# naver/must3r

Measured on AMD Instinct MI355X. Metric: views/sec (whole node) MUSt3R_512 20-view 512x384; pointmap max-abs-err vs ref, higher is better.
Workload: dtype fp16 (split weights in the attention-side Linears, plain in the Mlp Linears); 1 GPU; MUSt3R_512 20-view 384x512 scenes, S=28 independent scenes IN FLIGHT per GPU (560 views/step); one at a time: value_single_scene; scenes_in_flight_per_gpu=28, H=384, W=512, parallelism=single GPU

## Files before the change

### include/must3r_hip.h

```cpp
#ifndef MUST3R_HIP_H
#define MUST3R_HIP_H

#include <stdint.h>
#include <stddef.h>

#ifdef __cplusplus
extern "C" {
#endif

#define MUST3R_HIP_ABI_VERSION 21

typedef struct must3r_hip_ctx must3r_hip_ctx;

enum { MUST3R_BF16 = 0, MUST3R_F16 = 1, MUST3R_F16_W2 = 2, MUST3R_F16_WA = 3 };
#define MUST3R_ATTN_FP8 0x100
int must3r_hip_has_fp8_attention(void);

enum { MUST3R_MEM_KV = 0, MUST3R_MEM_NORM_Y = 1, MUST3R_MEM_RAW = 2 };

typedef struct must3r_hip_config {
    int32_t img_size, patch_size;
    int32_t enc_dim, enc_depth, enc_heads;
    int32_t dec_dim, dec_depth, dec_heads;
    int32_t mlp_ratio;
    float rope_freq;
    float rope_f0;
} must3r_hip_config;

int must3r_hip_abi_version(void);
const char* must3r_hip_last_error(void);
int must3r_hip_set_option(const char* name, long long value);

int must3r_hip_create(const must3r_hip_config* cfg, int device, must3r_hip_ctx** out);
void must3r_hip_destroy(must3r_hip_ctx* ctx);

int must3r_hip_load_weight(must3r_hip_ctx* ctx, const char* name, const float* data, int is_device,
                           int ndim, const int64_t* shape);
enum { MUST3R_PART_ENCODER = 1, MUST3R_PART_DECODER = 2 };
int must3r_hip_finalize_weights(must3r_hip_ctx* ctx, int parts);

int must3r_hip_encode(must3r_hip_ctx* ctx, int dtype, const float* img, int n_views, int H, int W,
                      float* out_tokens, int64_t* out_pos, void* stream);

typedef struct must3r_hip_group {
    const float* tokens;
    const int64_t* pos;
    int32_t n_views, n_tokens, H, W;
    float* pointmaps;
    int64_t pointmaps_scene_stride;
} must3r_hip_group;

typedef int (*must3r_hip_cp_exchange_fn)(void* user, int layer, void* slots, size_t slot_bytes, int n_slots, int my_slot, void* stream);
typedef struct must3r_hip_cp {
    int32_t world, rank;
    int32_t n_mem_total;
    int32_t partial16;
    void* slots;
    size_t slot_bytes;
    must3r_hip_cp_exchange_fn exchange;
    void* user;
} must3r_hip_cp;

typedef struct must3r_hip_decode_args {
    int32_t dtype;
    int32_t mem_mode;
    int32_t render;
    int32_t first_call;
    int32_t n_groups;
    const must3r_hip_group* groups;
    int32_t n_mem;
    void* const* mem;
    float* feats;
    int32_t mem_capacity;
    int32_t n_scenes;
    int64_t mem_scene_stride;
    const must3r_hip_cp* cp;
    int32_t causal;
} must3r_hip_decode_args;

size_t must3r_hip_cp_slot_bytes(const must3r_hip_ctx* ctx, int rows);
size_t must3r_hip_cp_slot_bytes16(const must3r_hip_ctx* ctx, int rows);

int must3r_hip_decode(must3r_hip_ctx* ctx, const must3r_hip_decode_args* args, void* stream);

int must3r_hip_postprocess(const float* pointmaps, float* pts3d, float* pts3d_local, float* conf, size_t npix,
                           void* stream);
enum { MUST3R_ACT_NORM_EXP = 0, MUST3R_ACT_LINEAR = 1 };
int must3r_hip_postprocess_act(const float* pointmaps, int activation, float* pts3d, float* pts3d_local, float* conf, size_t npix,
                               void* stream);
int must3r_hip_postprocess_act_grad(const float* pointmaps, int activation, const float* grad_pts3d, const float* grad_pts3d_local,
                                    const float* grad_conf, float* grad_pointmaps, size_t npix, void* stream);

size_t must3r_hip_postprocess_cam_scratch_bytes(int n_views, int H, int W);
int must3r_hip_postprocess_cam(const float* pointmaps, int n_views, int H, int W, float* pts3d, float* pts3d_local,
                               float* conf, float* focal, float* c2w, void* scratch, size_t scratch_bytes, void* stream);
int must3r_hip_postprocess_cam_act(const float* pointmaps, int activation, int n_views, int H, int W, float* pts3d, float* pts3d_local,
                                   float* conf, float* focal, float* c2w, void* scratch, size_t scratch_bytes, void* stream);

int must3r_hip_affine(int is_double, const float* A, const void* sub, const void* B, int b_transposed, const void* bias,
                      const float* resid, float* out, int M, int N, int K, void* stream);
int must3r_hip_row_norm(const float* x, int M, int C, float* out, void* stream);
int must3r_hip_l2_normalize(const float* x, int64_t outer, int L, int64_t inner, float* out, void* stream);
int must3r_hip_layernorm_act_f32(const float* x, const float* gamma, const float* beta, float eps, int M, int C, int gelu,
                                 float* out, void* stream);
int must3r_hip_topk_gather(const float* feat, const float* attn, int n_images, int N, int C, int k, float* out_feat,
                           float* out_attn, int64_t* out_idx, void* stream);
int must3r_hip_weighted_spoc(const float* feat, const float* attn, int n_images, int N, int C, float* out, void* stream);

int must3r_hip_asmk_centroid_sqnorm(const float* centroids, int K, int D, float* out, void* stream);
size_t must3r_hip_asmk_quantize_scratch_bytes(int M, int K, int k);
int must3r_hip_asmk_quantize(const float* feat, int M, const float* centroids, const float* c_sqnorm, int K, int D, int k, int32_t* ids,
                             void* scratch, size_t scratch_bytes, void* stream);
int must3r_hip_asmk_aggregate(const float* feat, const float* centroids, int K, int D, const int32_t* ids, int k_ids, int k_use,
                              const int32_t* offsets_dev, int n_images, int max_rows, int32_t* words, uint32_t* bits, int32_t* counts,
                              void* stream);
int must3r_hip_asmk_scores(const int32_t* words_q, const uint32_t* bits_q, const int32_t* counts_q, const int32_t* offsets_q, int k_q, int n_q,
                           const int32_t* words_d, const uint32_t* bits_d, const int32_t* counts_d, const int32_t* offsets_d, int k_d, int n_d,
                           int D, float alpha, float threshold, int normalize, double* out, void* stream);

int must3r_hip_nn_query(const float* db_xyz, int64_t n_db, const float* q_xyz, int64_t n_q, float* out_dist, void* stream);
int must3r_hip_quadrant_ids(const float* pts_xyz, int64_t n, const float* cam_center_host3, int divider, int32_t* out, void* stream);

size_t must3r_hip_nn_index_bytes(int64_t n, int divider);
size_t must3r_hip_nn_index_scratch_bytes(int64_t n);
int must3r_hip_nn_index_build(const float* xyz, const int32_t* quadrant_ids, int64_t n, int divider, void* index, void* scratch, void* stream);
int must3r_hip_nn_index_query(const void* index, const float* q_xyz, int64_t n_q, const float* cam_center_host3, int divider, float* out_dist,
                              void* stream);

#define MUST3R_EXPORT_MAX_THR 8
#define MUST3R_EXPORT_BLOCK 1024
#define MUST3R_EXPORT_GLB 0
#define MUST3R_EXPORT_PLY 1
typedef struct must3r_hip_export_view {
    const float* conf;
    const float* pts;
    const float* rgb;
    int32_t H, W;
    double M[12];
} must3r_hip_export_view;
size_t must3r_hip_export_scratch_bytes(const must3r_hip_export_view* views_host, int n_views, int n_thr, int mesh);
int must3r_hip_export_count(const must3r_hip_export_view* views_host, int n_views, const float* thr_host, int n_thr, int mesh,
                            void* scratch, size_t scratch_bytes, int64_t* totals_host, void* stream);
int must3r_hip_export_scatter_points(const must3r_hip_export_view* views_host, int n_views, const float* thr_host, int n_thr, int k,
                                     int layout, const void* scratch, void* out_pos, void* out_col, float* minmax, void* stream);
int must3r_hip_export_vertices(const must3r_hip_export_view* views_host, int n_views, int n_thr, void* scratch, float* out_pos,
                               void* out_col, float* minmax, void* stream);
int must3r_hip_export_scatter_faces(const must3r_hip_export_view* views_host, int n_views, const float* thr_host, int n_thr, int k,
                                    const void* scratch, uint32_t* out_faces, void* stream);

#define MUST3R_NORM_AVG_DIS 0
#define MUST3R_NORM_AVG_LOG1P 1
#define MUST3R_NORM_SQRT_DIS 2
#define MUST3R_NORM_MEDIAN_DIS 3
typedef struct must3r_hip_metrics_loss_args {
    int32_t n_scenes, n_views, H, W;
    const float* gt_pts;
    const float* in_camera0;
    const float* w2c;
    const float* pr_pts;
    const float* pr_local;
    const float* conf;
    const uint8_t* valid;
    const uint8_t* sky;
    const float* gt_scale;
    const float* pr_scale;
    const uint8_t* pr_warp;
    int32_t gt_warp, has_dist_clip, loss_in_log;
    float dist_clip, sky_loss_value, alpha;
    int64_t* counts;
    double* sums;
    float* pix_g; float* pix_l; uint8_t* msk_g; uint8_t* msk_l;
} must3r_hip_metrics_loss_args;
size_t must3r_hip_metrics_loss_scratch_bytes(int n_scenes, int n_views, int H, int W);
int must3r_hip_metrics_loss(const must3r_hip_metrics_loss_args* args, void* scratch, size_t scratch_bytes, void* stream);
size_t must3r_hip_metrics_factor_scratch_bytes(int n_scenes, int n_views, int H, int W, int mode);
int must3r_hip_metrics_factor(const float* pts, const float* trf, const uint8_t* valid, int n_scenes, int n_views, int H, int W, int mode,
                              float* factor, float* dist, void* scratch, size_t scratch_bytes, void* stream);

enum { MUST3R_LOSS_W_SCALAR = 0, MUST3R_LOSS_W_MEAN = 1, MUST3R_LOSS_W_CONF = 2, MUST3R_LOSS_W_PIXEL = 3 };
typedef struct must3r_hip_metrics_loss_grad_args {
    const float* w_g;
    const float* w_l;
    int32_t weighting;
    int32_t factor_mode;
    int32_t n_own;
    int32_t reserved;
    const int64_t* counts;
    const uint8_t* own_factor;
    const int64_t* n_valid;
    float* grad_pts;
    float* grad_local;
    float* grad_conf;
} must3r_hip_metrics_loss_grad_args;
size_t must3r_hip_metrics_loss_grad_scratch_bytes(int n_scenes, int n_views, int H, int W);
int must3r_hip_metrics_loss_grad(const must3r_hip_metrics_loss_args* args, const must3r_hip_metrics_loss_grad_args* grad, void* scratch,
                                 size_t scratch_bytes, void* stream);

enum { MUST3R_RESAMPLE_AA_BILINEAR = 0, MUST3R_RESAMPLE_PIL_LANCZOS = 1, MUST3R_RESAMPLE_PIL_BICUBIC = 2, MUST3R_RESAMPLE_NEAREST_EXACT = 3 };
enum { MUST3R_IMG_U8_HWC = 0, MUST3R_IMG_F32_CHW = 1 };

int must3r_hip_resample_coeffs(int mode, int in_size, int out_size, int* ksize, int32_t* bounds, void* weights);

typedef struct must3r_hip_image_desc {
    const void* src;
    int32_t src_format;
    int32_t channels;
    int32_t H, W;
    int64_t row_stride;
    int64_t plane_stride;
    int32_t crop_y, crop_x, crop_h, crop_w;
    int32_t resize_h, resize_w;
    int32_t out_y, out_x, out_h, out_w;
    int64_t out_offset;
} must3r_hip_image_desc;

size_t must3r_hip_image_scratch_bytes(int mode, const must3r_hip_image_desc* descs, int n_images);
int must3r_hip_resample(int mode, const must3r_hip_image_desc* descs, int n_images, float* out, void* scratch, size_t scratch_bytes,
                        void* stream);

enum { MUST3R_EPI_STORE16 = 0, MUST3R_EPI_STORE16_GELU = 1, MUST3R_EPI_QKV_ROPE = 2, MUST3R_EPI_RESID_F32 = 3,
       MUST3R_EPI_F32 = 4, MUST3R_EPI_HEAD = 5 };

int must3r_hip_op_gemm(int dtype, int epi, const void* A, const void* W, const float* bias, void* out,
                       int M, int N, int K, int lda, int ldc,
                       const int64_t* pos, const float* rope_tab, int rope_cols, int rope_npos,
                       const float* bias2, int row_start2, int accumulate,
                       int ntok, int gw, int H, int W_img,
                       int wsplit,
                       void* stream);
int must3r_hip_op_sparse24_pack(const float* w, int rows, int K, void* vals, void* idx, void* stream);
int must3r_hip_op_gemm_sp(int epi, const void* A, const void* W2, const void* Wlo_sp, const void* Widx_sp, const float* bias, void* out,
// ... 365 lines not shown
```

### must3r_amd/_lib.py

```python
import ctypes as C
import os

_HERE = os.path.dirname(os.path.abspath(__file__))
LIB_PATH = os.path.join(_HERE, "libmust3r_hip.so")

BF16, F16, F16_W2, F16_WA = 0, 1, 2, 3
ATTN_FP8 = 0x100
MEM_KV, MEM_NORM_Y, MEM_RAW = 0, 1, 2
PART_ENCODER, PART_DECODER = 1, 2
EPI_STORE16, EPI_STORE16_GELU, EPI_QKV_ROPE, EPI_RESID_F32, EPI_F32, EPI_HEAD = range(6)
ABI_VERSION = 21
ACT_NORM_EXP, ACT_LINEAR = 0, 1
EXPORT_MAX_THR, EXPORT_GLB, EXPORT_PLY = 8, 0, 1
NORM_AVG_DIS, NORM_AVG_LOG1P, NORM_SQRT_DIS, NORM_MEDIAN_DIS = range(4)
LOSS_W_SCALAR, LOSS_W_MEAN, LOSS_W_CONF, LOSS_W_PIXEL = range(4)
RESAMPLE_AA_BILINEAR, RESAMPLE_PIL_LANCZOS, RESAMPLE_PIL_BICUBIC, RESAMPLE_NEAREST_EXACT = range(4)
IMG_U8_HWC, IMG_F32_CHW = 0, 1
LIN_BIAS, LIN_BIAS_RES, LIN_BIAS_GELU = range(3)
TRAIN_LINEAR_F32, TRAIN_LINEAR_BF16 = 0, 1
TRAIN_ATTENTION_F32, TRAIN_ATTENTION_BF16 = 0, 1

class Config(C.Structure):
    _fields_ = [("img_size", C.c_int32), ("patch_size", C.c_int32),
                ("enc_dim", C.c_int32), ("enc_depth", C.c_int32), ("enc_heads", C.c_int32),
                ("dec_dim", C.c_int32), ("dec_depth", C.c_int32), ("dec_heads", C.c_int32),
                ("mlp_ratio", C.c_int32), ("rope_freq", C.c_float), ("rope_f0", C.c_float)]


class Group(C.Structure):
    _fields_ = [("tokens", C.c_void_p), ("pos", C.c_void_p),
                ("n_views", C.c_int32), ("n_tokens", C.c_int32), ("H", C.c_int32), ("W", C.c_int32),
                ("pointmaps", C.c_void_p), ("pointmaps_scene_stride", C.c_int64)]


CpExchangeFn = C.CFUNCTYPE(C.c_int, C.c_void_p, C.c_int, C.c_void_p, C.c_size_t, C.c_int, C.c_int, C.c_void_p)


class Cp(C.Structure):
    _fields_ = [("world", C.c_int32), ("rank", C.c_int32), ("n_mem_total", C.c_int32), ("partial16", C.c_int32),
                ("slots", C.c_void_p), ("slot_bytes", C.c_size_t), ("exchange", CpExchangeFn), ("user", C.c_void_p)]


class DecodeArgs(C.Structure):
    _fields_ = [("dtype", C.c_int32), ("mem_mode", C.c_int32), ("render", C.c_int32), ("first_call", C.c_int32),
                ("n_groups", C.c_int32), ("groups", C.POINTER(Group)), ("n_mem", C.c_int32),
                ("mem", C.POINTER(C.c_void_p)), ("feats", C.c_void_p),
                ("mem_capacity", C.c_int32), ("n_scenes", C.c_int32), ("mem_scene_stride", C.c_int64),
                ("cp", C.POINTER(Cp)), ("causal", C.c_int32)]


class ImageDesc(C.Structure):
    _fields_ = [("src", C.c_void_p), ("src_format", C.c_int32), ("channels", C.c_int32), ("H", C.c_int32), ("W", C.c_int32),
                ("row_stride", C.c_int64), ("plane_stride", C.c_int64),
                ("crop_y", C.c_int32), ("crop_x", C.c_int32), ("crop_h", C.c_int32), ("crop_w", C.c_int32),
                ("resize_h", C.c_int32), ("resize_w", C.c_int32),
                ("out_y", C.c_int32), ("out_x", C.c_int32), ("out_h", C.c_int32), ("out_w", C.c_int32), ("out_offset", C.c_int64)]


class AttnOp(C.Structure):
    _fields_ = [("dtype", C.c_int32), ("Q", C.c_void_p), ("K", C.c_void_p), ("V", C.c_void_p), ("O", C.c_void_p),
                ("ldq", C.c_int32), ("ldk", C.c_int32), ("ldv", C.c_int32), ("ldo", C.c_int32), ("heads", C.c_int32),
                ("views_dev", C.c_void_p), ("n_views", C.c_int32), ("view0_inline", C.c_int32), ("view0", C.c_int32 * 6),
                ("max_nq", C.c_int32), ("max_nk", C.c_int32), ("q_prescaled", C.c_int32),
                ("nsplit", C.c_int32), ("scratch", C.c_void_p), ("total_q_rows", C.c_int32), ("dense_rows", C.c_int32),
                ("stage", C.c_int32), ("slot_o", C.c_void_p), ("slot_ml", C.c_void_p), ("p16", C.c_int32), ("nslots", C.c_int32),
                ("stride_o", C.c_int64), ("stride_ml", C.c_int64), ("picked", C.POINTER(C.c_char_p))]


class LnOp(C.Structure):
    _fields_ = [("dtype", C.c_int32), ("x", C.c_void_p), ("x16", C.c_void_p), ("add", C.c_void_p), ("w", C.c_void_p), ("b", C.c_void_p),
                ("out16", C.c_void_p), ("out16_lo", C.c_void_p), ("out16_dup", C.c_void_p), ("ld16", C.c_int32),
                ("out32", C.c_void_p), ("copy32", C.c_void_p), ("raw16", C.c_void_p), ("M", C.c_int32), ("C", C.c_int32), ("eps", C.c_float),
                ("rows_per_group", C.c_int32), ("add_groups", C.c_int32), ("picked", C.POINTER(C.c_char_p)), ("mean_out", C.c_void_p)]


class GemmOp(C.Structure):
    _fields_ = [("dtype", C.c_int32), ("epi", C.c_int32), ("A", C.c_void_p), ("W", C.c_void_p), ("bias", C.c_void_p), ("out", C.c_void_p),
                ("M", C.c_int32), ("N", C.c_int32), ("K", C.c_int32), ("lda", C.c_int32), ("ldc", C.c_int32), ("wsplit", C.c_int32),
                ("Wlo_sp", C.c_void_p), ("Widx_sp", C.c_void_p), ("wsp_rows", C.c_int32), ("out_scale", C.c_float), ("scale_cols", C.c_int32),
                ("batch", C.c_int32), ("strideA", C.c_int64), ("strideW", C.c_int64), ("strideB", C.c_int64), ("out_table", C.c_void_p), ("wdiv", C.c_int32),
                ("pos", C.c_void_p), ("rope_tab", C.c_void_p), ("rope_cols", C.c_int32), ("rope_npos", C.c_int32),
                ("bias2", C.c_void_p), ("row_start2", C.c_int32), ("row_period2", C.c_int32), ("accumulate", C.c_int32),
                ("ntok", C.c_int32), ("gw", C.c_int32), ("H", C.c_int32), ("Wimg", C.c_int32), ("head_views", C.c_int32), ("head_scene_skip", C.c_int64),
                ("picked", C.POINTER(C.c_char_p))]


class LnFoldOp(C.Structure):
    _fields_ = [("dtype", C.c_int32), ("epi", C.c_int32), ("A", C.c_void_p), ("W", C.c_void_p), ("bias", C.c_void_p), ("out", C.c_void_p),
                ("M", C.c_int32), ("N", C.c_int32), ("K", C.c_int32), ("lda", C.c_int32), ("ldc", C.c_int32), ("wsplit", C.c_int32),
                ("x16_out", C.c_void_p), ("copy32_out", C.c_void_p), ("stats_out", C.c_void_p),
                ("ln_stats", C.c_void_p), ("ln_s", C.c_void_p), ("ln_eps", C.c_float), ("ln_shift", C.c_void_p), ("ln_shift_init", C.c_int32),
                ("pos", C.c_void_p), ("rope_tab", C.c_void_p), ("rope_cols", C.c_int32), ("rope_npos", C.c_int32),
                ("out_scale", C.c_float), ("scale_cols", C.c_int32), ("bias2", C.c_void_p), ("row_start2", C.c_int32),
                ("picked", C.POINTER(C.c_char_p))]


class ExportView(C.Structure):
    _fields_ = [("conf", C.c_void_p), ("pts", C.c_void_p), ("rgb", C.c_void_p), ("H", C.c_int32), ("W", C.c_int32), ("M", C.c_double * 12)]


class MetricsLossArgs(C.Structure):
    _fields_ = [("n_scenes", C.c_int32), ("n_views", C.c_int32), ("H", C.c_int32), ("W", C.c_int32),
                ("gt_pts", C.c_void_p), ("in_camera0", C.c_void_p), ("w2c", C.c_void_p), ("pr_pts", C.c_void_p), ("pr_local", C.c_void_p),
                ("conf", C.c_void_p), ("valid", C.c_void_p), ("sky", C.c_void_p), ("gt_scale", C.c_void_p), ("pr_scale", C.c_void_p),
                ("pr_warp", C.c_void_p), ("gt_warp", C.c_int32), ("has_dist_clip", C.c_int32), ("loss_in_log", C.c_int32),
                ("dist_clip", C.c_float), ("sky_loss_value", C.c_float), ("alpha", C.c_float),
                ("counts", C.c_void_p), ("sums", C.c_void_p),
                ("pix_g", C.c_void_p), ("pix_l", C.c_void_p), ("msk_g", C.c_void_p), ("msk_l", C.c_void_p)]


class MetricsLossGradArgs(C.Structure):
    _fields_ = [("w_g", C.c_void_p), ("w_l", C.c_void_p), ("weighting", C.c_int32), ("factor_mode", C.c_int32), ("n_own", C.c_int32),
                ("reserved", C.c_int32), ("counts", C.c_void_p), ("own_factor", C.c_void_p), ("n_valid", C.c_void_p),
                ("grad_pts", C.c_void_p), ("grad_local", C.c_void_p), ("grad_conf", C.c_void_p)]


class HeadGradArgs(C.Structure):
    _fields_ = [("x", C.c_void_p), ("gamma", C.c_void_p), ("beta", C.c_void_p), ("W", C.c_void_p), ("G", C.c_void_p),
                ("n_views", C.c_int32), ("H", C.c_int32), ("Wimg", C.c_int32), ("D", C.c_int32), ("eps", C.c_float), ("reserved", C.c_int32),
                ("dx", C.c_void_p), ("dgamma", C.c_void_p), ("dbeta", C.c_void_p), ("dW", C.c_void_p), ("db", C.c_void_p)]


class HeadForwardArArgs(C.Structure):
    _fields_ = [("x", C.c_void_p), ("gamma", C.c_void_p), ("beta", C.c_void_p), ("W", C.c_void_p), ("b", C.c_void_p),
                ("dtype", C.c_int32), ("n_views", C.c_int32), ("H", C.c_int32), ("Wimg", C.c_int32), ("D", C.c_int32), ("eps", C.c_float),
                ("pointmaps", C.c_void_p), ("transposed", C.c_void_p), ("stream", C.c_void_p)]


class HeadGradArArgs(C.Structure):
    _fields_ = [("g", HeadGradArgs), ("transposed", C.c_void_p), ("stream", C.c_void_p)]


class AttnTrainArgs(C.Structure):
    _fields_ = [("q", C.c_void_p), ("k", C.c_void_p), ("v", C.c_void_p), ("dO", C.c_void_p),
                ("ldq", C.c_int32), ("ldk", C.c_int32), ("ldv", C.c_int32), ("lddo", C.c_int32), ("heads", C.c_int32), ("n_views", C.c_int32),
                ("views", C.c_void_p), ("O", C.c_void_p), ("lse", C.c_void_p), ("dQ", C.c_void_p), ("dK", C.c_void_p), ("dV", C.c_void_p),
                ("ldo", C.c_int32), ("lddq", C.c_int32), ("lddk", C.c_int32), ("lddv", C.c_int32)]


class AttnMaskedArgs(C.Structure):
    _fields_ = [("core", AttnTrainArgs), ("mask_bits", C.c_void_p), ("view_mask", C.c_void_p), ("mask_rows", C.c_int32), ("mask_ld", C.c_int32),
                ("stream", C.c_void_p)]


class MlpSublayerArgs(C.Structure):
    _fields_ = [("x", C.c_void_p), ("gamma", C.c_void_p), ("beta", C.c_void_p), ("W1", C.c_void_p), ("b1", C.c_void_p), ("W2", C.c_void_p), ("b2", C.c_void_p),
                ("dy", C.c_void_p), ("M", C.c_int32), ("D", C.c_int32), ("hidden", C.c_int32), ("eps", C.c_float), ("out", C.c_void_p),
                ("dx", C.c_void_p), ("dgamma", C.c_void_p), ("dbeta", C.c_void_p), ("dW1", C.c_void_p), ("db1", C.c_void_p), ("dW2", C.c_void_p),
                ("db2", C.c_void_p)]


class AttnSublayerArgs(C.Structure):
    _fields_ = [("x", C.c_void_p), ("gamma", C.c_void_p), ("beta", C.c_void_p), ("Wqkv", C.c_void_p), ("bqkv", C.c_void_p), ("Wproj", C.c_void_p),
                ("bproj", C.c_void_p), ("dy", C.c_void_p), ("pos", C.c_void_p), ("rope_tab", C.c_void_p), ("views", C.c_void_p),
                ("M", C.c_int32), ("D", C.c_int32), ("n_views", C.c_int32), ("rope_npos", C.c_int32), ("eps", C.c_float), ("reserved", C.c_int32),
                ("out", C.c_void_p), ("dx", C.c_void_p), ("dgamma", C.c_void_p), ("dbeta", C.c_void_p), ("dWqkv", C.c_void_p), ("dbqkv", C.c_void_p),
                ("dWproj", C.c_void_p), ("dbproj", C.c_void_p)]


class CrossSublayerArgs(C.Structure):
    _fields_ = [("x", C.c_void_p), ("mem", C.c_void_p), ("gamma", C.c_void_p), ("beta", C.c_void_p), ("Wq", C.c_void_p), ("bq", C.c_void_p),
                ("Wk", C.c_void_p), ("bk", C.c_void_p), ("Wv", C.c_void_p), ("bv", C.c_void_p), ("Wproj", C.c_void_p), ("bproj", C.c_void_p),
                ("dy", C.c_void_p), ("views", C.c_void_p), ("out", C.c_void_p),
                ("dx", C.c_void_p), ("dmem", C.c_void_p), ("dgamma", C.c_void_p), ("dbeta", C.c_void_p), ("dWq", C.c_void_p), ("dbq", C.c_void_p),
                ("dWk", C.c_void_p), ("dbk", C.c_void_p), ("dWv", C.c_void_p), ("dbv", C.c_void_p), ("dWproj", C.c_void_p), ("dbproj", C.c_void_p),
                ("M", C.c_int32), ("Rm", C.c_int32), ("D", C.c_int32), ("n_views", C.c_int32), ("ldmem", C.c_int32), ("lddmem", C.c_int32),
                ("eps", C.c_float), ("reserved", C.c_int32), ("stream", C.c_void_p)]


class CrossSublayerMaskedArgs(C.Structure):
    _fields_ = [("core", CrossSublayerArgs), ("mask_bits", C.c_void_p), ("view_mask", C.c_void_p), ("mask_rows", C.c_int32), ("mask_ld", C.c_int32)]


FEEDBACK_MAX_LAYERS = 32


class FeedbackPrepareArgs(C.Structure):
    _fields_ = [(n, C.c_void_p * FEEDBACK_MAX_LAYERS) for n in ("x", "gamma", "beta", "dy", "y", "dx", "dgamma", "dbeta")] + [
        ("offset", C.c_void_p), ("doffset", C.c_void_p), ("L", C.c_int32), ("R", C.c_int32), ("D", C.c_int32), ("add_layers", C.c_int32),
        ("eps", C.c_float), ("reserved", C.c_int32), ("stream", C.c_void_p)]


OPTIM_CHUNK = 32768


class OptimTensor(C.Structure):
    _fields_ = [("p", C.c_void_p), ("g", C.c_void_p), ("m", C.c_void_p), ("v", C.c_void_p), ("step", C.c_void_p), ("n", C.c_int64),
                ("group", C.c_int32), ("reserved", C.c_int32)]


class OptimGroup(C.Structure):
    _fields_ = [("lr", C.c_double), ("weight_decay", C.c_double), ("beta1", C.c_double), ("beta2", C.c_double), ("eps", C.c_double)]


class OptimControl(C.Structure):
    _fields_ = [("norm", C.c_float), ("coef", C.c_float), ("found_inf", C.c_int32), ("reserved", C.c_int32)]


class OptimArgs(C.Structure):
    _fields_ = [("tensors", C.POINTER(OptimTensor)), ("groups", C.POINTER(OptimGroup)), ("n_tensors", C.c_int32), ("n_groups", C.c_int32),
                ("control", C.c_void_p), ("scale", C.c_void_p), ("growth_tracker", C.c_void_p),
                ("max_norm", C.c_float), ("growth_factor", C.c_float), ("backoff_factor", C.c_float), ("growth_interval", C.c_int32),
                ("stream", C.c_void_p)]


class PatchRowsArgs(C.Structure):
    _fields_ = [("img", C.c_void_p), ("transposed", C.c_void_p), ("rows", C.c_void_p), ("pos", C.c_void_p),
                ("V", C.c_int32), ("H", C.c_int32), ("W", C.c_int32), ("reserved", C.c_int32), ("stream", C.c_void_p)]


GT_VIEW_BLOCKS = 32


class GtArgs(C.Structure):
    _fields_ = [("depth", C.c_void_p), ("depth_scale", C.c_void_p), ("K", C.c_void_p), ("c2w", C.c_void_p), ("transposed", C.c_void_p),
                ("pts3d", C.c_void_p), ("valid", C.c_void_p), ("sky", C.c_void_p), ("n_valid", C.c_void_p),
                ("scratch", C.c_void_p), ("scratch_bytes", C.c_size_t),
                ("V", C.c_int32), ("Hs", C.c_int32), ("Ws", C.c_int32), ("depth_u16", C.c_int32), ("stream", C.c_void_p)]


AUG_BRIGHTNESS, AUG_CONTRAST, AUG_SATURATION, AUG_HUE = range(4)
AUG_TILE = 64


class AugmentColorView(C.Structure):
    _fields_ = [("src_offset", C.c_int64), ("h", C.c_int32), ("w", C.c_int32), ("portrait", C.c_int32), ("order", C.c_int32 * 4),
                ("apply", C.c_int32 * 4), ("factor", C.c_float * 4), ("reserved", C.c_int32)]


class AugmentColorArgs(C.Structure):
    _fields_ = [("src", C.c_void_p), ("src_elems", C.c_int64), ("views", C.POINTER(AugmentColorView)), ("out", C.c_void_p),
                ("scratch", C.c_void_p), ("scratch_bytes", C.c_size_t),
                ("V", C.c_int32), ("Hs", C.c_int32), ("Ws", C.c_int32), ("reserved", C.c_int32), ("stream", C.c_void_p)]


class AugmentDepthView(C.Structure):
    _fields_ = [("src", C.c_void_p), ("row_stride", C.c_int64), ("H", C.c_int32), ("W", C.c_int32),
                ("crop_x", C.c_int32), ("crop_y", C.c_int32), ("crop_w", C.c_int32), ("crop_h", C.c_int32),
                ("resize_w", C.c_int32), ("resize_h", C.c_int32),
                ("win_x", C.c_int32), ("win_y", C.c_int32), ("out_w", C.c_int32), ("out_h", C.c_int32), ("portrait", C.c_int32), ("reserved", C.c_int32)]


class AugmentDepthArgs(C.Structure):
    _fields_ = [("views", C.POINTER(AugmentDepthView)), ("out", C.c_void_p), ("scratch", C.c_void_p), ("scratch_bytes", C.c_size_t),
                ("V", C.c_int32), ("Hs", C.c_int32), ("Ws", C.c_int32), ("depth_u16", C.c_int32), ("stream", C.c_void_p)]


class ProfRecord(C.Structure):
    _fields_ = [("name", C.c_char * 32), ("ms", C.c_double), ("flops", C.c_double), ("calls", C.c_int64)]


vp, i32, i64, fp, sz, cstr, P = C.c_void_p, C.c_int, C.c_int64, C.c_float, C.c_size_t, C.c_char_p, C.POINTER
PROTOTYPES = {
    "must3r_hip_last_error": (cstr, []),
    "must3r_hip_has_fp8_attention": (i32, []),
    "must3r_hip_abi_version": (i32, []),
    "must3r_hip_set_option": (i32, [cstr, i64]),
    "must3r_hip_create": (i32, [P(Config), i32, P(vp)]),
    "must3r_hip_destroy": (None, [vp]),
    "must3r_hip_load_weight": (i32, [vp, cstr, vp, i32, i32, P(i64)]),
    "must3r_hip_finalize_weights": (i32, [vp, i32]),
    "must3r_hip_encode": (i32, [vp, i32, vp, i32, i32, i32, vp, vp, vp]),
    "must3r_hip_cp_slot_bytes": (sz, [vp, i32]),
    "must3r_hip_cp_slot_bytes16": (sz, [vp, i32]),
    "must3r_hip_decode": (i32, [vp, P(DecodeArgs), vp]),
    "must3r_hip_postprocess": (i32, [vp, vp, vp, vp, sz, vp]),
    "must3r_hip_postprocess_act": (i32, [vp, i32, vp, vp, vp, sz, vp]),
    "must3r_hip_postprocess_act_grad": (i32, [vp, i32, vp, vp, vp, vp, sz, vp]),
    "must3r_hip_postprocess_cam_scratch_bytes": (sz, [i32, i32, i32]),
    "must3r_hip_postprocess_cam": (i32, [vp, i32, i32, i32, vp, vp, vp, vp, vp, vp, sz, vp]),
    "must3r_hip_postprocess_cam_act": (i32, [vp, i32, i32, i32, i32, vp, vp, vp, vp, vp, vp, sz, vp]),
    "must3r_hip_affine": (i32, [i32, vp, vp, vp, i32, vp, vp, vp, i32, i32, i32, vp]),
    "must3r_hip_row_norm": (i32, [vp, i32, i32, vp, vp]),
    "must3r_hip_l2_normalize": (i32, [vp, i64, i32, i64, vp, vp]),
    "must3r_hip_layernorm_act_f32": (i32, [vp, vp, vp, fp, i32, i32, i32, vp, vp]),
    "must3r_hip_topk_gather": (i32, [vp, vp, i32, i32, i32, i32, vp, vp, vp, vp]),
    "must3r_hip_weighted_spoc": (i32, [vp, vp, i32, i32, i32, vp, vp]),
    "must3r_hip_asmk_quantize_scratch_bytes": (sz, [i32, i32, i32]),
    "must3r_hip_asmk_centroid_sqnorm": (i32, [vp, i32, i32, vp, vp]),
    "must3r_hip_asmk_quantize": (i32, [vp, i32, vp, vp, i32, i32, i32, vp, vp, sz, vp]),
    "must3r_hip_asmk_aggregate": (i32, [vp, vp, i32, i32, vp, i32, i32, vp, i32, i32, vp, vp, vp, vp]),
    "must3r_hip_asmk_scores": (i32, [vp, vp, vp, vp, i32, i32, vp, vp, vp, vp, i32, i32, i32, fp, fp, i32, vp, vp]),
    "must3r_hip_nn_query": (i32, [vp, i64, vp, i64, vp, vp]),
    "must3r_hip_quadrant_ids": (i32, [vp, i64, P(fp), i32, vp, vp]),
    "must3r_hip_nn_index_bytes": (sz, [i64, i32]),
    "must3r_hip_nn_index_scratch_bytes": (sz, [i64]),
    "must3r_hip_nn_index_build": (i32, [vp, vp, i64, i32, vp, vp, vp]),
    "must3r_hip_nn_index_query": (i32, [vp, vp, i64, P(fp), i32, vp, vp]),
    "must3r_hip_export_scratch_bytes": (sz, [P(ExportView), i32, i32, i32]),
    "must3r_hip_export_count": (i32, [P(ExportView), i32, P(fp), i32, i32, vp, sz, P(i64), vp]),
    "must3r_hip_export_scatter_points": (i32, [P(ExportView), i32, P(fp), i32, i32, i32, vp, vp, vp, vp, vp]),
    "must3r_hip_export_vertices": (i32, [P(ExportView), i32, i32, vp, vp, vp, vp, vp]),
    "must3r_hip_export_scatter_faces": (i32, [P(ExportView), i32, P(fp), i32, i32, vp, vp, vp]),
    "must3r_hip_metrics_loss_scratch_bytes": (sz, [i32, i32, i32, i32]),
    "must3r_hip_metrics_loss": (i32, [P(MetricsLossArgs), vp, sz, vp]),
    "must3r_hip_metrics_factor_scratch_bytes": (sz, [i32, i32, i32, i32, i32]),
    "must3r_hip_metrics_factor": (i32, [vp, vp, vp, i32, i32, i32, i32, i32, vp, vp, vp, sz, vp]),
    "must3r_hip_metrics_loss_grad_scratch_bytes": (sz, [i32, i32, i32, i32]),
    "must3r_hip_metrics_loss_grad": (i32, [P(MetricsLossArgs), P(MetricsLossGradArgs), vp, sz, vp]),
    "must3r_hip_resample_coeffs": (i32, [i32, i32, i32, P(i32), vp, vp]),
    "must3r_hip_image_scratch_bytes": (sz, [i32, P(ImageDesc), i32]),
    "must3r_hip_resample": (i32, [i32, P(ImageDesc), i32, vp, vp, sz, vp]),
    "must3r_hip_op_gemm": (i32, [i32, i32, vp, vp, vp, vp, i32, i32, i32, i32, i32, vp, vp, i32, i32, vp, i32, i32, i32, i32, i32, i32, i32, vp]),
    "must3r_hip_op_sparse24_pack": (i32, [vp, i32, i32, vp, vp, vp]),
    "must3r_hip_op_gemm_sp": (i32, [i32, vp, vp, vp, vp, vp, vp, i32, i32, i32, i32, i32, vp, vp, i32, i32, vp]),
    "must3r_hip_op_gemm_lnfold": (i32, [i32, i32, vp, vp, vp, vp, i32, i32, i32, i32, i32, vp, vp, vp, vp, vp, fp, vp, i32, vp, vp, i32, i32, fp, i32, vp]),
    "must3r_hip_op_gemm_lnfold_ex": (i32, [P(LnFoldOp), vp]),
    "must3r_hip_op_gemm_fold256": (i32, [i32, i32, vp, vp, vp, vp, vp, vp, i32, i32, i32, i32, i32, vp, vp, vp, vp, vp, fp, vp, vp, vp, i32, i32, fp, i32, vp]),
    "must3r_hip_op_gemm_ex": (i32, [P(GemmOp), vp]),
    "must3r_hip_rope_table": (i32, [fp, fp, i32, vp]),
    "must3r_hip_attention_scratch_bytes": (sz, [i32, i32, i32]),
    "must3r_hip_op_attention": (i32, [i32, vp, vp, vp, vp, i32, i32, i32, i32, i32, vp, i32, i32, i32, vp, i32, vp]),
    "must3r_hip_op_attention_ex": (i32, [P(AttnOp), vp]),
    "must3r_hip_op_layernorm": (i32, [i32, vp, vp, vp, vp, vp, vp, vp, vp, i32, i32, fp, vp]),
    "must3r_hip_op_layernorm_ex": (i32, [P(LnOp), vp]),
    "must3r_hip_op_im2col": (i32, [i32, vp, vp, i32, i32, i32, vp]),
    "must3r_hip_op_cast": (i32, [i32, vp, vp, vp, sz, vp]),
    "must3r_hip_head_grad_splits": (i32, [i32]),
    "must3r_hip_head_forward_scratch_bytes": (sz, [i32, i32, i32, i32]),
    "must3r_hip_head_forward": (i32, [i32, vp, vp, vp, vp, vp, i32, i32, i32, i32, fp, vp, vp, sz, vp]),
    "must3r_hip_op_head_linear": (i32, [i32, vp, vp, vp, i32, i32, i32, i32, vp, vp, sz, vp]),
    "must3r_hip_head_grad_scratch_bytes": (sz, [i32, i32, i32, i32]),
    "must3r_hip_head_grad": (i32, [P(HeadGradArgs), vp, sz, vp]),
    "must3r_hip_head_forward_many_ar_scratch_bytes": (sz, [i32, i32, i32, i32]),
    "must3r_hip_head_forward_many_ar": (i32, [P(HeadForwardArArgs), vp, sz]),
    "must3r_hip_head_grad_many_ar_scratch_bytes": (sz, [i32, i32, i32, i32]),
    "must3r_hip_head_grad_many_ar": (i32, [P(HeadGradArArgs), vp, sz]),
    "must3r_hip_op_linear_dgrad_f32": (i32, [vp, i32, vp, vp, i32, i32, i32, vp]),
    "must3r_hip_op_linear_wgrad_scratch_bytes": (sz, [i32, i32, i32]),
    "must3r_hip_op_linear_wgrad_f32": (i32, [vp, i32, vp, i32, vp, vp, i32, i32, i32, vp, sz, vp]),
    "must3r_hip_op_layernorm_grad_scratch_bytes": (sz, [i32, i32]),
    "must3r_hip_op_layernorm_grad": (i32, [vp, vp, vp, vp, vp, vp, i32, i32, fp, vp, sz, vp]),
    "must3r_hip_attn_train_scratch_bytes": (sz, [i32, i32, i32, i32]),
    "must3r_hip_attn_train_groups": (i32, [vp, i32]),
    "must3r_hip_attn_forward_f32": (i32, [P(AttnTrainArgs), vp, sz, vp]),
    "must3r_hip_attn_grad": (i32, [P(AttnTrainArgs), vp, sz, vp]),
    "must3r_hip_attn_masked_scratch_bytes": (sz, [i32, i32, i32, i32]),
    "must3r_hip_attn_masked_forward": (i32, [P(AttnMaskedArgs), vp, sz]),
    "must3r_hip_attn_masked_grad": (i32, [P(AttnMaskedArgs), vp, sz]),
    "must3r_hip_op_linear_f32": (i32, [i32, vp, i32, vp, vp, vp, i32, vp, i32, vp, i32, i32, i32, i32, vp]),
    "must3r_hip_op_layernorm_f32": (i32, [vp, vp, vp, vp, i32, i32, fp, vp]),
    "must3r_hip_op_gelu_f32": (i32, [vp, vp, vp, C.c_longlong, vp]),
    "must3r_hip_op_gelu_grad_f32": (i32, [vp, i32, vp, i32, vp, i32, i32, i32, vp]),
    "must3r_hip_op_rope_f32": (i32, [vp, i32, vp, vp, i32, i32, i32, i32, vp]),
    "must3r_hip_op_layernorm_grad_add": (i32, [vp, vp, vp, vp, vp, vp, vp, i32, i32, fp, vp, sz, vp]),
    "must3r_hip_mlp_sublayer_scratch_bytes": (sz, [i32, i32, i32]),
    "must3r_hip_mlp_sublayer_forward": (i32, [P(MlpSublayerArgs), vp, sz, vp]),
    "must3r_hip_mlp_sublayer_grad": (i32, [P(MlpSublayerArgs), vp, sz, vp]),
    "must3r_hip_attn_sublayer_scratch_bytes": (sz, [i32, i32, i32]),
    "must3r_hip_attn_sublayer_forward": (i32, [P(AttnSublayerArgs), vp, sz, vp]),
    "must3r_hip_attn_sublayer_grad": (i32, [P(AttnSublayerArgs), vp, sz, vp]),
    "must3r_hip_cross_sublayer_scratch_bytes": (sz, [i32, i32, i32, i32, i32]),
    "must3r_hip_cross_sublayer_forward": (i32, [P(CrossSublayerArgs), vp, sz]),
    "must3r_hip_cross_sublayer_grad": (i32, [P(CrossSublayerArgs), vp, sz]),
    "must3r_hip_cross_sublayer_masked_scratch_bytes": (sz, [i32, i32, i32, i32, i32]),
    "must3r_hip_cross_sublayer_masked_forward": (i32, [P(CrossSublayerMaskedArgs), vp, sz]),
    "must3r_hip_cross_sublayer_masked_grad": (i32, [P(CrossSublayerMaskedArgs), vp, sz]),
    "must3r_hip_feedback_prepare_scratch_bytes": (sz, [i32, i32, i32]),
    "must3r_hip_feedback_prepare_forward": (i32, [P(FeedbackPrepareArgs), vp, sz]),
    "must3r_hip_feedback_prepare_grad": (i32, [P(FeedbackPrepareArgs), vp, sz]),
    "must3r_hip_optim_scratch_bytes": (sz, [i64, i64]),
    "must3r_hip_optim_norm": (i32, [P(OptimArgs), vp, sz]),
    "must3r_hip_optim_adamw": (i32, [P(OptimArgs), vp, sz]),
    "must3r_hip_train_linear_mode": (i32, [i32]),
    "must3r_hip_train_attention_mode": (i32, [i32]),
    "must3r_hip_patch_rows": (i32, [P(PatchRowsArgs)]),
    "must3r_hip_gt_from_depth": (i32, [P(GtArgs)]),
    "must3r_hip_augment_color_scratch_bytes": (sz, [i32, i32, i32]),
    "must3r_hip_augment_color": (i32, [P(AugmentColorArgs)]),
    "must3r_hip_augment_depth_scratch_bytes": (sz, [i32]),
    "must3r_hip_augment_depth": (i32, [P(AugmentDepthArgs)]),
    "must3r_hip_debug_tr_probe": (i32, [vp, vp]),
    "must3r_hip_set_profiling": (i32, [vp, i32]),
    "must3r_hip_get_profile": (i32, [vp, P(ProfRecord), i32, i32]),
}
EXPORTS = tuple(PROTOTYPES)


class HipError(RuntimeError):
    pass


_lib = None


def load():
    global _lib
    if _lib is not None:
        return _lib
    if not os.path.exists(LIB_PATH):
        raise ImportError(
            f"{LIB_PATH} not found: build it with `python -c 'import __graft_entry__ as g; g.build()'` "
            "(make -C must3r_amd/csrc). must3r_amd has no CPU fallback.")
    lib = C.CDLL(LIB_PATH)
    for name, (restype, argtypes) in PROTOTYPES.items():
        fn = getattr(lib, name)
        fn.restype, fn.argtypes = restype, argtypes
    if lib.must3r_hip_abi_version() != ABI_VERSION:
        raise ImportError(f"{LIB_PATH}: ABI version {lib.must3r_hip_abi_version()} != {ABI_VERSION}; rebuild")
    _lib = lib
    return lib


def stream_ptr(device):
    import torch
    return torch.cuda.current_stream(device).cuda_stream


def check(rc):
    if rc != 0:
        raise HipError(load().must3r_hip_last_error().decode("utf-8", "replace"))


def has_fp8_attention():
    return bool(load().must3r_hip_has_fp8_attention())
# ... 52 lines not shown
```

### must3r_amd/csrc/kernels.hpp

```cpp
#pragma once
#include <hip/hip_runtime.h>
#include <stdint.h>

struct must3r_hip_ctx;

namespace m3r {

enum DType { DT_BF16 = 0, DT_F16 = 1 };

enum Epi {
    EPI_STORE16 = 0,
    EPI_STORE16_GELU,
    EPI_QKV_ROPE,
    EPI_RESID_F32,
    EPI_F32,
    EPI_HEAD,
    EPI_COUNT
};

#ifdef M3R_ATTN_FP8
constexpr bool kAttnFp8Built = true;
#else
constexpr bool kAttnFp8Built = false;
#endif

struct GemmArgs {
    const void* A;
    const void* W;
    const float* bias;
    void* out;
    int M, N, K, lda, ldc;
    int wsplit;
    const void* Wlo_sp;
    const void* Widx_sp;
    int wsp_rows;
    float out_scale;
    int scale_cols;
    int batch;
    long long strideA, strideW, strideB;
    void* const* out_table;
    int wdiv;
    const int64_t* pos;
    const float* rope_tab;
    int rope_cols;
    int rope_npos;
    const float* bias2;
    int row_start2;
    int row_period2;
    int accumulate;
    int ntok, gw, H, Wimg;
    int head_views;
    long long head_scene_skip;
    void* x16_out;
    float* copy32_out;
    float* stats_out;
    const float* ln_stats;
    const float* ln_s;
    float ln_eps;
    float* ln_shift;
    int ln_shift_init;
    int fold256;
    int gm;
#ifdef GEMM_TRACE
    int trace_block;
#endif
};

int launch_gemm(DType dt, Epi epi, const GemmArgs& a, hipStream_t s, const char** err);
const char* gemm_last_kernel();
bool gemm_fold256_shape_ok(int M, int N, int K, bool split);

struct AttnView {
    int q_row0;
    int nq;
    int kv_row0;
    int nk;
    int skip_lo;
    int skip_hi;
};

struct AttnArgs {
    const void* Q; const void* K; const void* V; void* O;
    int ldq, ldk, ldv, ldo;
    int heads;
    const AttnView* views;
    int nviews;
    int view0_inline;
    AttnView view0;
    int max_nq;
    float scale;
    int q_prescaled;
    int nsplit;
    float* part_o;
    float* part_ml;
    int total_q_rows;
    int dense_rows;
    int part16;
    int fp8;
    int max_nk;
    long long part_stride_o, part_stride_ml;
};
int launch_attention_partial_merge(DType dt, const AttnArgs& a, float* out_o, float* out_ml, int p16, hipStream_t s, const char** err);
int launch_attention_partial_empty(float* out_o, float* out_ml, int rows, int heads, int p16, hipStream_t s, const char** err);
int launch_attention_partial_final(DType dt, const AttnArgs& a, const float* slots_o, const float* slots_ml, long long stride_o, long long stride_ml, int nslots,
                                   int p16, hipStream_t s, const char** err);
size_t attention_split_scratch_bytes(int nsplit, int total_q_rows, int heads);
int attention_pick_split(int nviews, int heads, int max_nq, int max_nk);
int launch_attention(DType dt, const AttnArgs& a, hipStream_t s, const char** err);
bool attention_is_small(int nviews, int heads, int max_nq, int nsplit);
int launch_attention_phase(DType dt, const AttnArgs& a, int phase, hipStream_t s, const char** err);
const char* attention_last_kernel();

struct LnArgs {
    const float* x;
    const void* x16;
    void* raw16;
    const float* add;
    const float* w; const float* b;
    void* out16;
    void* out16_lo;
    void* out16_dup;
    int ld16;
    float* out32;
    float* copy32;
    float* mean_out;
    int M, C;
    float eps;
    int rows_per_group;
    int add_groups;
};
int launch_layernorm(DType dt, const LnArgs& a, hipStream_t s, const char** err);
const char* layernorm_last_kernel();

int launch_im2col(DType dt, const float* img, void* out16, int V, int H, int W, hipStream_t s, const char** err);
int launch_cast(DType dt, const float* in, void* out16, void* out16_lo, size_t n, hipStream_t s, const char** err);
int launch_quant8(DType dt, const void* in16, int ld_in, void* out8, int ld_out, void* const* out_table, int rows_per_group,
                  size_t rows, int cols, int tail_cols, hipStream_t s, const char** err);
int launch_fill_pos(int64_t* pos, int V, int gh, int gw, hipStream_t s, const char** err);
int launch_split16(DType dt, const float* in, void* hi, void* lo, size_t n, hipStream_t s, const char** err);
int launch_sparse24_pack(const float* w, int rows, int K, void* vals, void* idx, hipStream_t s, const char** err);

int head_layernorm(must3r_hip_ctx* c, DType dt, const float* x, const float* gamma, const float* beta, void* hcat, float* y32, int R, int D, float eps,
                   hipStream_t s);
int head_linear(must3r_hip_ctx* c, DType dt, const void* hcat, const void* wcat, const float* bias_ps, float* pointmaps, int rows, int D, int OUT, int ntok,
                int gw, int H, int Wimg, int head_views, long long head_scene_skip, hipStream_t s);

int launch_dgrad_seg_f32(const float* dZ, int ldz, const float* W0, const float* W1, int O0, float* out, int ldo, int M, int O, int K, hipStream_t s);

struct LinArgs;
bool train_linear_bf16();
int launch_linear_bf16(const char* who, int epi, const LinArgs& p, hipStream_t s);
int launch_dgrad_bf16(const char* who, const float* dZ, int ldz, const float* W0, const float* W1, int O0, float* out, int ldo, int M, int O, int K, hipStream_t s);
int launch_wgrad_parts_bf16(const float* dZ, int ldz, const float* A, int lda, int M, int O, int K, int rows_per_split, int S, int want_dw, float* part,
                            float* pdb, hipStream_t s);

int launch_tr_probe(short* out, hipStream_t s);

}
```

### must3r_amd/csrc/misc.hip

```cpp
#include "abi.hpp"
#include "common.hpp"
#include "kernels.hpp"
#include "options.hpp"
#include <cstring>
#include <cstdio>
#include <cstdlib>

namespace m3r {
namespace {
struct OptRow { const char* name; long long def, lo, hi; };
const OptRow kOpts[OPT_COUNT] = {
    {"PERSIST", 0, 0, 1}, {"GEMM256", 1, 0, 2}, {"G256K", 1, 0, 2}, {"G256P", 1, 0, 1}, {"G256P_SPLIT", 1, 0, 2}, {"SPARSE_256", 1, 0, 1},
    {"SPARSE_LO", 1, 0, 1}, {"BK128", 1, 0, 1}, {"LN_ROWS", 1, 0, 1}, {"LNFOLD", 1, 0, 2}, {"ENC_CHUNK_ROWS", 32768, 256, 1 << 22}, {"ATTN_LZ", 1, 0, 2},
    {"LNFOLD256", 0, 0, 1}, {"G256_GM", 4, 1, 64}, {"NN_LEAF_LOG2", 5, 4, 6}, {"NN_QUERY_LANES_LOG2", 3, 0, 4},
};
long long g_opt_val[OPT_COUNT];
bool g_opt_init[OPT_COUNT];
}

int opt(Opt o) {
    if (!g_opt_init[o]) {
        const OptRow& r = kOpts[o];
        long long v = r.def;
        char env[48];
        snprintf(env, sizeof(env), "M3R_%s", r.name);
        if (const char* e = getenv(env)) {
            char* end = nullptr;
            const long long x = strtoll(e, &end, 10);
            if (end == e || *end != 0 || x < r.lo || x > r.hi)
                fprintf(stderr, "libmust3r_hip: %s=%s ignored (an integer in [%lld, %lld] is expected); using %lld\n", env, e, r.lo, r.hi, r.def);
            else v = x;
        }
        g_opt_val[o] = v;
        g_opt_init[o] = true;
    }
    return (int)g_opt_val[o];
}

int opt_set(const char* name, long long value, const char** err) {
    static thread_local char msg[128];
    for (int o = 0; o < OPT_COUNT; ++o) {
        if (name == nullptr || strcmp(name, kOpts[o].name) != 0) continue;
        if (value < kOpts[o].lo || value > kOpts[o].hi) {
            snprintf(msg, sizeof(msg), "set_option: %s = %lld is outside [%lld, %lld]", name, value, kOpts[o].lo, kOpts[o].hi);
            *err = msg;
            return 1;
        }
        g_opt_val[o] = value;
        g_opt_init[o] = true;
        return 0;
    }
    snprintf(msg, sizeof(msg), "set_option: unknown option '%s'", name ? name : "(null)");
    *err = msg;
    return 1;
}


template <class T, bool MEAN = false>
__global__ void __launch_bounds__(256) ln_kernel(const LnArgs p) {
    typedef typename Vec<T>::v4 v4;
    const int lane = threadIdx.x & 63;
    const int row = blockIdx.x * 4 + (threadIdx.x >> 6);
    if (row >= p.M) return;
    const float* wp = p.w;
    const float* bp = p.b;
    const float* addp = p.add ? p.add + (size_t)row * p.C : nullptr;
    if (p.rows_per_group > 0) {
        const int g = row / p.rows_per_group;
        wp += (size_t)g * p.C;
        bp += (size_t)g * p.C;
        addp = (p.add && g < p.add_groups) ? p.add + (size_t)(row - g * p.rows_per_group) * p.C : nullptr;
    }
    f32x4 v[4];
    float s = 0.f;
#pragma unroll
    for (int i = 0; i < 4; ++i) {
        const int c = (i * 64 + lane) * 4;
        v[i] = f32x4{0.f, 0.f, 0.f, 0.f};
        if (c < p.C) {
            if (p.x) v[i] = *reinterpret_cast<const f32x4*>(p.x + (size_t)row * p.C + c);
            else v[i] = __builtin_convertvector(*reinterpret_cast<const v4*>(reinterpret_cast<const T*>(p.x16) + (size_t)row * p.C + c), f32x4);
            if (addp) v[i] += *reinterpret_cast<const f32x4*>(addp + c);
            if (p.copy32) *reinterpret_cast<f32x4*>(p.copy32 + (size_t)row * p.C + c) = v[i];
            if (p.raw16) *reinterpret_cast<v4*>(reinterpret_cast<T*>(p.raw16) + (size_t)row * p.C + c) = cvt4_sat<T>(v[i]);
            s += v[i][0] + v[i][1] + v[i][2] + v[i][3];
        }
    }
    const float mean = wave_sum_dpp(s) / (float)p.C;
    if constexpr (MEAN) {
        if (lane == 0) p.mean_out[row] = mean;
    }
    float q = 0.f;
#pragma unroll
    for (int i = 0; i < 4; ++i) {
        const int c = (i * 64 + lane) * 4;
        if (c < p.C) {
            v[i] -= mean;
            q += v[i][0] * v[i][0] + v[i][1] * v[i][1] + v[i][2] * v[i][2] + v[i][3] * v[i][3];
        }
    }
    const float rstd = rsqrtf(wave_sum_dpp(q) / (float)p.C + p.eps);
#pragma unroll
    for (int i = 0; i < 4; ++i) {
        const int c = (i * 64 + lane) * 4;
        if (c < p.C) {
            const f32x4 w = *reinterpret_cast<const f32x4*>(wp + c);
            const f32x4 b = *reinterpret_cast<const f32x4*>(bp + c);
            const f32x4 y = v[i] * rstd * w + b;
            if (p.out32) *reinterpret_cast<f32x4*>(p.out32 + (size_t)row * p.C + c) = y;
            if (p.out16) {
                const size_t ld = p.ld16 ? (size_t)p.ld16 : (size_t)p.C;
                const v4 h = cvt4<T>(y);
                *reinterpret_cast<v4*>(reinterpret_cast<T*>(p.out16) + row * ld + c) = h;
                if (p.out16_dup) *reinterpret_cast<v4*>(reinterpret_cast<T*>(p.out16_dup) + row * ld + c) = h;
                if (p.out16_lo) {
                    const f32x4 hf = __builtin_convertvector(h, f32x4);
                    *reinterpret_cast<v4*>(reinterpret_cast<T*>(p.out16_lo) + row * ld + c) = cvt4<T>(y - hf);
                }
            }
        }
    }
}

template <class T, int NV>
__global__ void __launch_bounds__(256) ln_rows_kernel(const LnArgs p) {
    typedef typename Vec<T>::v4 v4;
    const int lane = threadIdx.x & 63;
    const int nwaves = gridDim.x * 4;
    int row = blockIdx.x * 4 + (threadIdx.x >> 6);
    if (row >= p.M) return;
    const bool grouped = p.rows_per_group > 0;
    bool act[NV];
    f32x4 w[NV], b[NV];
#pragma unroll
    for (int i = 0; i < NV; ++i) {
        act[i] = (i * 64 + lane) * 4 < p.C;
        w[i] = b[i] = f32x4{0.f, 0.f, 0.f, 0.f};
        if (act[i] && !grouped) {
            w[i] = *reinterpret_cast<const f32x4*>(p.w + (i * 64 + lane) * 4);
            b[i] = *reinterpret_cast<const f32x4*>(p.b + (i * 64 + lane) * 4);
        }
    }
    auto load = [&](int r, f32x4 (&v)[NV]) {
#pragma unroll
        for (int i = 0; i < NV; ++i) {
            const int c = (i * 64 + lane) * 4;
            v[i] = f32x4{0.f, 0.f, 0.f, 0.f};
            if (act[i]) {
                if (p.x) v[i] = *reinterpret_cast<const f32x4*>(p.x + (size_t)r * p.C + c);
                else v[i] = __builtin_convertvector(*reinterpret_cast<const v4*>(reinterpret_cast<const T*>(p.x16) + (size_t)r * p.C + c), f32x4);
            }
        }
    };
    f32x4 v[NV], nx[NV];
    load(row, v);
    for (; row < p.M; row += nwaves) {
        const int nr = row + nwaves;
        if (nr < p.M) load(nr, nx);
        const float* addp = p.add ? p.add + (size_t)row * p.C : nullptr;
        if (grouped) {
            const int g = row / p.rows_per_group;
            addp = (p.add && g < p.add_groups) ? p.add + (size_t)(row - g * p.rows_per_group) * p.C : nullptr;
#pragma unroll
            for (int i = 0; i < NV; ++i)
                if (act[i]) {
                    w[i] = *reinterpret_cast<const f32x4*>(p.w + (size_t)g * p.C + (i * 64 + lane) * 4);
                    b[i] = *reinterpret_cast<const f32x4*>(p.b + (size_t)g * p.C + (i * 64 + lane) * 4);
                }
        }
        float s = 0.f;
#pragma unroll
        for (int i = 0; i < NV; ++i) {
            const int c = (i * 64 + lane) * 4;
            if (act[i]) {
                if (addp) v[i] += *reinterpret_cast<const f32x4*>(addp + c);
                if (p.copy32) *reinterpret_cast<f32x4*>(p.copy32 + (size_t)row * p.C + c) = v[i];
                if (p.raw16) *reinterpret_cast<v4*>(reinterpret_cast<T*>(p.raw16) + (size_t)row * p.C + c) = cvt4_sat<T>(v[i]);
                s += v[i][0] + v[i][1] + v[i][2] + v[i][3];
            }
        }
        const float mean = wave_sum_dpp(s) / (float)p.C;
        float q = 0.f;
#pragma unroll
        for (int i = 0; i < NV; ++i)
            if (act[i]) {
                v[i] -= mean;
                q += v[i][0] * v[i][0] + v[i][1] * v[i][1] + v[i][2] * v[i][2] + v[i][3] * v[i][3];
            }
        const float rstd = rsqrtf(wave_sum_dpp(q) / (float)p.C + p.eps);
#pragma unroll
        for (int i = 0; i < NV; ++i) {
            const int c = (i * 64 + lane) * 4;
            if (act[i]) {
                const f32x4 y = v[i] * rstd * w[i] + b[i];
                if (p.out32) *reinterpret_cast<f32x4*>(p.out32 + (size_t)row * p.C + c) = y;
                if (p.out16) {
                    const size_t ld = p.ld16 ? (size_t)p.ld16 : (size_t)p.C;
                    const v4 h = cvt4<T>(y);
                    *reinterpret_cast<v4*>(reinterpret_cast<T*>(p.out16) + row * ld + c) = h;
                    if (p.out16_dup) *reinterpret_cast<v4*>(reinterpret_cast<T*>(p.out16_dup) + row * ld + c) = h;
                    if (p.out16_lo) {
                        const f32x4 hf = __builtin_convertvector(h, f32x4);
                        *reinterpret_cast<v4*>(reinterpret_cast<T*>(p.out16_lo) + row * ld + c) = cvt4<T>(y - hf);
                    }
                }
            }
        }
#pragma unroll
        for (int i = 0; i < NV; ++i) v[i] = nx[i];
    }
}

static int ln_rows_mode() { return opt(OPT_LN_ROWS); }
static thread_local const char* g_ln_pick = "";
const char* layernorm_last_kernel() { return g_ln_pick; }
template <class T>
static void launch_ln_t(const LnArgs& a, hipStream_t s) {
    const int grid_one = (a.M + 3) / 4;
    if (a.mean_out != nullptr) {
        g_ln_pick = "ln";
        hipLaunchKernelGGL((ln_kernel<T, true>), dim3(grid_one), dim3(256), 0, s, a);
        return;
    }
    if (ln_rows_mode() == 0 || a.M < 65536) {
        g_ln_pick = "ln";
        hipLaunchKernelGGL(ln_kernel<T>, dim3(grid_one), dim3(256), 0, s, a);
        return;
    }
    const int grid = 256 * 8;
    g_ln_pick = a.C <= 768 ? "ln_rows/3" : "ln_rows/4";
    if (a.C <= 768) hipLaunchKernelGGL((ln_rows_kernel<T, 3>), dim3(grid), dim3(256), 0, s, a);
    else hipLaunchKernelGGL((ln_rows_kernel<T, 4>), dim3(grid), dim3(256), 0, s, a);
}

int launch_layernorm(DType dt, const LnArgs& a, hipStream_t s, const char** err) {
    if (a.M <= 0) return 0;
    if (a.C > 1024 || a.C % 4) { *err = "layernorm: C must be <= 1024 and a multiple of 4"; return 1; }
    if (dt == DT_BF16) launch_ln_t<bf16_t>(a, s);
    else launch_ln_t<f16_t>(a, s);
    if (hipGetLastError() != hipSuccess) { *err = "layernorm: launch failed"; return 1; }
    return 0;
}

template <class T>
__global__ void im2col_kernel(const float* __restrict__ img, T* __restrict__ out, int V, int H, int W) {
    typedef typename Vec<T>::v8 v8;
    const int gh = H / 16, gw = W / 16;
    const size_t total = (size_t)V * gh * gw * 96;
    for (size_t idx = (size_t)blockIdx.x * blockDim.x + threadIdx.x; idx < total; idx += (size_t)gridDim.x * blockDim.x) {
        const int ch = (int)(idx % 96);
        const size_t tok = idx / 96;
        const int t = (int)(tok % (gh * gw));
        const int v = (int)(tok / (gh * gw));
        const int gy = t / gw, gx = t - gy * gw;
        const int c = ch / 32, rem = ch - c * 32;
        const int i = rem >> 1, j0 = (rem & 1) * 8;
        const float* src = img + (((size_t)v * 3 + c) * H + gy * 16 + i) * W + gx * 16 + j0;
        const f32x4 a = *reinterpret_cast<const f32x4*>(src);
        const f32x4 b = *reinterpret_cast<const f32x4*>(src + 4);
        const f32x8 f = __builtin_shufflevector(a, b, 0, 1, 2, 3, 4, 5, 6, 7);
        *reinterpret_cast<v8*>(out + tok * 768 + ch * 8) = cvt8<T>(f);
    }
}

int launch_im2col(DType dt, const float* img, void* out16, int V, int H, int W, hipStream_t s, const char** err) {
    if (H % 16 || W % 16) { *err = "im2col: H and W must be multiples of 16"; return 1; }
    const size_t total = (size_t)V * (H / 16) * (W / 16) * 96;
    if (!total) return 0;
    const int grid = (int)((total + 255) / 256 < 4096 ? (total + 255) / 256 : 4096);
    if (dt == DT_BF16) hipLaunchKernelGGL(im2col_kernel<bf16_t>, dim3(grid), dim3(256), 0, s, img, (bf16_t*)out16, V, H, W);
    else hipLaunchKernelGGL(im2col_kernel<f16_t>, dim3(grid), dim3(256), 0, s, img, (f16_t*)out16, V, H, W);
    if (hipGetLastError() != hipSuccess) { *err = "im2col: launch failed"; return 1; }
    return 0;
}

template <class T>
__global__ void cast_kernel(const float* __restrict__ in, T* __restrict__ hi, T* __restrict__ lo, size_t n4) {
    typedef typename Vec<T>::v4 v4;
    for (size_t i = (size_t)blockIdx.x * blockDim.x + threadIdx.x; i < n4; i += (size_t)gridDim.x * blockDim.x) {
        const f32x4 x = reinterpret_cast<const f32x4*>(in)[i];
        const v4 h = cvt4<T>(x);
        reinterpret_cast<v4*>(hi)[i] = h;
        if (lo) reinterpret_cast<v4*>(lo)[i] = cvt4<T>(x - __builtin_convertvector(h, f32x4));
    }
}

int launch_split16(DType dt, const float* in, void* hi, void* lo, size_t n, hipStream_t s, const char** err) {
    if (n % 4) { *err = "cast: element count must be a multiple of 4"; return 1; }
    if (!n) return 0;
    const size_t n4 = n / 4;
    const int grid = (int)((n4 + 255) / 256 < 8192 ? (n4 + 255) / 256 : 8192);
    if (dt == DT_BF16) hipLaunchKernelGGL(cast_kernel<bf16_t>, dim3(grid), dim3(256), 0, s, in, (bf16_t*)hi, (bf16_t*)lo, n4);
    else hipLaunchKernelGGL(cast_kernel<f16_t>, dim3(grid), dim3(256), 0, s, in, (f16_t*)hi, (f16_t*)lo, n4);
    if (hipGetLastError() != hipSuccess) { *err = "cast: launch failed"; return 1; }
    return 0;
}

int launch_cast(DType dt, const float* in, void* out16, void* out16_lo, size_t n, hipStream_t s, const char** err) {
    return launch_split16(dt, in, out16, out16_lo, n, s, err);
}

__global__ void sparse24_pack_kernel(const float* __restrict__ w, int rows, int K, f16_t* __restrict__ vals, unsigned short* __restrict__ idx) {
    const size_t total = (size_t)(K / 64) * rows * 4;
    for (size_t u = (size_t)blockIdx.x * blockDim.x + threadIdx.x; u < total; u += (size_t)gridDim.x * blockDim.x) {
        const int g = (int)(u & 3);
        const size_t tn = u >> 2;
        const int n = (int)(tn % rows), t = (int)(tn / rows);
        const float* src = w + (size_t)n * K + t * 64 + g * 16;
        unsigned bits = 0;
        f16_t out[8];
#pragma unroll
        for (int q = 0; q < 4; ++q) {
            float lo[4], mag[4];
#pragma unroll
            for (int e = 0; e < 4; ++e) {
                const float x = src[q * 4 + e];
                const f16_t hi = (f16_t)x;
                lo[e] = (float)(f16_t)(x - (float)hi);
                mag[e] = fabsf(lo[e]);
            }
            int p0 = 0;
#pragma unroll
            for (int e = 1; e < 4; ++e) if (mag[e] > mag[p0]) p0 = e;
            int p1 = p0 == 0 ? 1 : 0;
#pragma unroll
            for (int e = 0; e < 4; ++e) if (e != p0 && mag[e] > mag[p1]) p1 = e;
            const int a = p0 < p1 ? p0 : p1, b = p0 < p1 ? p1 : p0;
            out[q * 2] = (f16_t)lo[a];
            out[q * 2 + 1] = (f16_t)lo[b];
            bits |= (unsigned)(a | (b << 2)) << (4 * q);
        }
        f16_t* dv = vals + ((size_t)t * rows + n) * 32 + g * 8;
#pragma unroll
        for (int e = 0; e < 8; ++e) dv[e] = out[e];
        idx[(((size_t)t * (rows / 32) + n / 32) * 64 + (n % 16) + 16 * g) * 2 + ((n % 32) / 16)] = (unsigned short)bits;
    }
}

int launch_sparse24_pack(const float* w, int rows, int K, void* vals, void* idx, hipStream_t s, const char** err) {
    if (rows <= 0 || K <= 0 || rows % 32 || K % 64) { *err = "sparse24_pack: rows % 32 and K % 64 must be 0"; return 1; }
    const size_t total = (size_t)(K / 64) * rows * 4;
    const int grid = (int)((total + 255) / 256 < 8192 ? (total + 255) / 256 : 8192);
    hipLaunchKernelGGL(sparse24_pack_kernel, dim3(grid), dim3(256), 0, s, w, rows, K, (f16_t*)vals, (unsigned short*)idx);
    if (hipGetLastError() != hipSuccess) { *err = "sparse24_pack: launch failed"; return 1; }
    return 0;
}

#ifdef M3R_ATTN_FP8
template <class T>
__global__ void quant8_kernel(const T* __restrict__ in, int ld_in, unsigned char* __restrict__ out, int ld_out, void* const* out_table,
                              int rows_per_group, size_t rows, int cols, int tail_cols) {
    typedef typename Vec<T>::v8 v8;
    const int cpr = (cols + tail_cols) / 8;
    const size_t total = rows * (size_t)cpr;
    for (size_t idx = (size_t)blockIdx.x * blockDim.x + threadIdx.x; idx < total; idx += (size_t)gridDim.x * blockDim.x) {
        const size_t r = idx / cpr;
        const int c = (int)(idx - r * cpr) * 8;
        const v8 raw = *reinterpret_cast<const v8*>(in + r * ld_in + c);
        unsigned char* dst = out;
        size_t rr = r;
        if (out_table) {
            const size_t g = r / rows_per_group;
            dst = reinterpret_cast<unsigned char*>(out_table[g]);
            rr = r - g * rows_per_group;
        }
        if (c >= cols) {
            *reinterpret_cast<v8*>(dst + rr * ld_out + cols + (size_t)(c - cols) * 2) = raw;
            continue;
        }
        const f32x8 x = __builtin_convertvector(raw, f32x8);
        float y[8];
#pragma unroll
        for (int e = 0; e < 8; ++e) y[e] = __builtin_amdgcn_fmed3f(x[e], -448.0f, 448.0f);
        int lo = 0, hi = 0;
        lo = __builtin_amdgcn_cvt_pk_fp8_f32(y[0], y[1], lo, false);
        lo = __builtin_amdgcn_cvt_pk_fp8_f32(y[2], y[3], lo, true);
        hi = __builtin_amdgcn_cvt_pk_fp8_f32(y[4], y[5], hi, false);
        hi = __builtin_amdgcn_cvt_pk_fp8_f32(y[6], y[7], hi, true);
        *reinterpret_cast<u32x2*>(dst + rr * ld_out + c) = u32x2{(unsigned)lo, (unsigned)hi};
    }
}

int launch_quant8(DType dt, const void* in16, int ld_in, void* out8, int ld_out, void* const* out_table, int rows_per_group,
                  size_t rows, int cols, int tail_cols, hipStream_t s, const char** err) {
    if (!rows || !(cols + tail_cols)) return 0;
    if (cols % 16 || tail_cols % 8 || ld_in % 8 || ld_out % 16) { *err = "quant8: cols % 16, tail_cols % 8, ld_in % 8, ld_out % 16"; return 1; }
    const size_t total = rows * (size_t)((cols + tail_cols) / 8);
    const int grid = (int)((total + 255) / 256 < 8192 ? (total + 255) / 256 : 8192);
    if (dt == DT_BF16) hipLaunchKernelGGL(quant8_kernel<bf16_t>, dim3(grid), dim3(256), 0, s, (const bf16_t*)in16, ld_in, (unsigned char*)out8, ld_out, out_table, rows_per_group, rows, cols, tail_cols);
    else hipLaunchKernelGGL(quant8_kernel<f16_t>, dim3(grid), dim3(256), 0, s, (const f16_t*)in16, ld_in, (unsigned char*)out8, ld_out, out_table, rows_per_group, rows, cols, tail_cols);
    if (hipGetLastError() != hipSuccess) { *err = "quant8: launch failed"; return 1; }
    return 0;
}
#endif

__global__ void fill_pos_kernel(int64_t* pos, int V, int gh, int gw) {
    const size_t total = (size_t)V * gh * gw;
    for (size_t i = (size_t)blockIdx.x * blockDim.x + threadIdx.x; i < total; i += (size_t)gridDim.x * blockDim.x) {
        const int t = (int)(i % (gh * gw));
        pos[i * 2 + 0] = t / gw;
        pos[i * 2 + 1] = t % gw;
    }
}

int launch_fill_pos(int64_t* pos, int V, int gh, int gw, hipStream_t s, const char** err) {
    const size_t total = (size_t)V * gh * gw;
    if (!total) return 0;
    const int grid = (int)((total + 255) / 256 < 2048 ? (total + 255) / 256 : 2048);
    hipLaunchKernelGGL(fill_pos_kernel, dim3(grid), dim3(256), 0, s, pos, V, gh, gw);
    if (hipGetLastError() != hipSuccess) { *err = "fill_pos: launch failed"; return 1; }
    return 0;
}

__device__ __forceinline__ void norm_exp3(const float* v, float* o) {
    const float d = sqrtf(v[0] * v[0] + v[1] * v[1] + v[2] * v[2]);
    const float sc = expm1f(d) / fmaxf(d, 1e-8f);
    o[0] = v[0] * sc;
    o[1] = v[1] * sc;
    o[2] = v[2] * sc;
}

template <bool LINEAR>
__global__ void postprocess_kernel(const float* __restrict__ pm, float* __restrict__ p3, float* __restrict__ pl,
                                   float* __restrict__ cf, size_t npix) {
    for (size_t i = (size_t)blockIdx.x * blockDim.x + threadIdx.x; i < npix; i += (size_t)gridDim.x * blockDim.x) {
        float v[7];
#pragma unroll
        for (int k = 0; k < 7; ++k) v[k] = pm[i * 7 + k];
        float a[3], b[3];
        if constexpr (LINEAR) {
#pragma unroll
            for (int k = 0; k < 3; ++k) { a[k] = v[k]; b[k] = v[3 + k]; }
        } else {
            norm_exp3(v, a);
            norm_exp3(v + 3, b);
        }
#pragma unroll
        for (int k = 0; k < 3; ++k) {
            p3[i * 3 + k] = a[k];
            pl[i * 3 + k] = b[k];
        }
        cf[i] = 1.0f + expf(v[6]);
    }
}

__device__ __forceinline__ void norm_exp3_grad(const float* v, const float* g, float* o) {
    const float d = sqrtf(v[0] * v[0] + v[1] * v[1] + v[2] * v[2]);
    if (d == 0.f) { o[0] = o[1] = o[2] = 0.f; return; }
    const float c = fmaxf(d, 1e-8f);
    const float h = expm1f(d) / c;
    const float b = d >= 1e-8f ? expf(d) - h : expf(d) * d / c;
    const float s = (v[0] * g[0] + v[1] * g[1] + v[2] * g[2]) / d * b;
    o[0] = h * g[0] + s * (v[0] / d);
    o[1] = h * g[1] + s * (v[1] / d);
// ... 82 lines not shown
```

### must3r_amd/csrc/model.hip

```cpp
#include <hip/hip_runtime.h>
#include <cmath>
#include <cstdarg>
#include <cstdio>
#include <cstring>
#include <map>
#include <string>
#include <vector>

#include "abi.hpp"
#include "kernels.hpp"
#include "options.hpp"

using namespace m3r;

static thread_local char g_err[512] = "";
int m3r::fail(const char* fmt, ...) {
    va_list ap;
    va_start(ap, fmt);
    vsnprintf(g_err, sizeof(g_err), fmt, ap);
    va_end(ap);
    return 1;
}
#define HIP_OK(expr)                                                                              \
    do {                                                                                          \
// ... 623 lines not shown
struct Fold {
    uint16_t* x16 = nullptr;
    float* stats = nullptr;
    float* shift = nullptr;
    bool f256 = false;
    bool fresh = true;
    bool on() const { return x16 != nullptr; }
    void in(GemmArgs& g, const Param* s, const Param* c) {
        g.A = x16; g.ln_stats = stats; g.ln_s = s->d; g.bias = c->d; g.ln_eps = 1e-6f;
        g.ln_shift = shift; g.ln_shift_init = (fresh && !f256) ? 1 : 0; g.fold256 = f256 ? 1 : 0;
        fresh = false;
    }
    void out(GemmArgs& g, float* copy32) const { g.x16_out = x16; g.stats_out = stats; g.copy32_out = copy32; g.ln_shift = shift; g.fold256 = f256 ? 1 : 0; }
};

struct BlockRows {
    int R, C, heads, F;
    float* x; uint16_t *h16, *qkv, *a16, *g16;
    uint8_t* q8;
    const int64_t* pos;
};
struct SelfViews { const AttnView* dev; int n, max_n; double flops; const AttnView* inline0; };

static int self_attention_sublayer(must3r_hip_ctx* c, DType dt, const std::vector<Param*>& LP, const BlockRows& b, const SelfViews& v, Fold& fold, bool fold_n1,
                                   float* copy32, float* mean_out, hipStream_t s) {
    const int R = b.R, C = b.C;
    const bool a8 = kAttnFp8Built && c->attn8 != 0;
    const void* w;
    if (!fold_n1) {
        LnArgs la = lnargs(b.x, nullptr, LP[LF_N1W]->d, LP[LF_N1B]->d, b.h16, nullptr, nullptr, copy32, R, C, 1e-6f);
        if (mean_out) { la.mean_out = mean_out; fold.fresh = false; }
        M3R_OK(layernorm_a(c, dt, la, s));
    }
    M3R_OK(w16p(c, *LP[fold_n1 ? LF_QKVLN_W : LF_QKVW], dt, &w, s));
    GemmArgs ga = gargs(b.h16, w, LP[LF_QKVB]->d, b.qkv, R, 3 * C, C, C, 3 * C);
    if (fold_n1) fold.in(ga, LP[LF_QKVLN_S], LP[LF_QKVLN_C]);
    ga.pos = b.pos; ga.rope_tab = c->rope_tab; ga.rope_cols = 2 * C; ga.rope_npos = c->rope_npos;
    ga.out_scale = kQScale; ga.scale_cols = C;
    M3R_OK(gemm(c, dt, EPI_QKV_ROPE, ga, s));
    AttnArgs aa;
    memset(&aa, 0, sizeof(aa));
    aa.Q = b.qkv; aa.K = b.qkv + C; aa.V = b.qkv + 2 * C; aa.O = b.a16;
    aa.ldq = aa.ldk = aa.ldv = 3 * C; aa.ldo = C; aa.heads = b.heads;
    aa.views = v.dev; aa.nviews = v.n; aa.max_nq = v.max_n; aa.scale = 0.125f; aa.q_prescaled = 1;
    if (v.inline0) { aa.view0_inline = 1; aa.view0 = *v.inline0; }
    if (a8 && !attention_is_small(v.n, b.heads, v.max_n, 1)) {
        M3R_OK(quant8(c, dt, b.qkv, 3 * C, b.q8, 2 * C, nullptr, 0, (size_t)R, 2 * C, 0, s));
        aa.Q = b.q8; aa.K = b.q8 + C; aa.ldq = aa.ldk = 2 * C; aa.fp8 = 1;
    }
    aa.max_nk = v.max_n;
    M3R_OK(attention(c, dt, aa, v.flops, PC_ATTN_SA, s));
    M3R_OK(w16p(c, *LP[LF_PROJW], dt, &w, s));
    GemmArgs gp = gargs(b.a16, w, LP[LF_PROJB]->d, b.x, R, C, C, C, C);
    if (fold.on()) fold.out(gp, nullptr);
    return gemm(c, dt, EPI_RESID_F32, gp, s);
}

static int mlp_sublayer(must3r_hip_ctx* c, DType dt, const std::vector<Param*>& LP, int norm_w, const BlockRows& b, Fold& fold, bool leave_rows, float* copy32,
                        hipStream_t s) {
    const int R = b.R, C = b.C, F = b.F;
    const bool folded = fold.on();
    const void* w;
    int ws;
    if (!folded) M3R_OK(layernorm_a(c, dt, lnargs(b.x, nullptr, LP[norm_w]->d, LP[norm_w + 1]->d, b.h16, nullptr, nullptr, nullptr, R, C, 1e-6f), s));
    M3R_OK(wmlp(c, *LP[folded ? LF_FC1LN_W : LF_FC1W], dt, &w, &ws, s));
    GemmArgs g1 = gargs(b.h16, w, LP[LF_FC1B]->d, b.g16, R, F, C, C, F);
    if (folded) fold.in(g1, LP[LF_FC1LN_S], LP[LF_FC1LN_C]);
    M3R_OK(gemm(c, dt, EPI_STORE16_GELU, g1, s, ws));
    M3R_OK(wmlp(c, *LP[LF_FC2W], dt, &w, &ws, s));
    GemmArgs g2 = gargs(b.g16, w, LP[LF_FC2B]->d, b.x, R, C, F, F, C);
    if (leave_rows) fold.out(g2, copy32);
    return gemm(c, dt, EPI_RESID_F32, g2, s, ws);
}

static int encode_chunk(must3r_hip_ctx* c, DType dt, const float* img, int V, int H, int W, float* out_tokens,
                        int64_t* out_pos, hipStream_t s) {
    const must3r_hip_config& g = c->cfg;
    const int C = g.enc_dim, gh = H / 16, gw = W / 16, N = gh * gw, R = V * N, F = g.mlp_ratio * C;
    const char* err = "";
    const bool a8 = kAttnFp8Built && c->attn8 != 0;
    if (c->enc_tab.empty()) build_layer_tables(c, false);
    const bool f256 = opt(OPT_LNFOLD256) != 0 && dt == DT_F16 && c->wsplit == 2 && c->mlp_plain && !a8 && (C == 768 || C == 1024) &&
                      c->enc_tab[0][LF_QKVLN_W] && c->enc_tab[0][LF_FC1LN_W] &&
                      gemm_fold256_shape_ok(R, 3 * C, C, true) && gemm_fold256_shape_ok(R, C, C, true) &&
                      gemm_fold256_shape_ok(R, F, C, false) && gemm_fold256_shape_ok(R, C, F, false);
    Workspace ws; uint16_t* P16;
    BlockRows b{R, C, g.enc_heads, F, nullptr, nullptr, nullptr, nullptr, nullptr, nullptr, out_pos};
    Fold fold; fold.f256 = f256;
    ws.want(P16, (size_t)R * 768);
    ws.want(b.x, (size_t)R * C);
    ws.want(b.h16, (size_t)R * C);
    ws.want(b.qkv, (size_t)R * 3 * C);
    ws.want(b.a16, (size_t)R * C);
    ws.want(b.g16, (size_t)R * F);
    ws.want(b.q8, a8 ? (size_t)R * 2 * C : 0);
    ws.want(fold.x16, f256 ? (size_t)R * C : 0);
    ws.want(fold.stats, f256 ? (size_t)R * (C / 64) * 2 : 0);
    ws.want(fold.shift, f256 ? (size_t)R : 0);
    M3R_OK(ws.commit(c, s));
    if (f256) HIP_OK(hipMemsetAsync(fold.shift, 0, (size_t)R * sizeof(float), s));

    {
        ProfScope ps(c, s, PC_MISC, 0.0);
        if (launch_fill_pos(out_pos, V, gh, gw, s, &err)) return fail("%s", err);
        if (launch_im2col(dt, img, P16, V, H, W, s, &err)) return fail("%s", err);
    }
    std::vector<AttnView> views(V);
    for (int v = 0; v < V; ++v) views[v] = AttnView{v * N, N, v * N, N, 0, 0};
    void* views_dev = nullptr;
    M3R_OK(upload_table(c, views.data(), sizeof(AttnView) * V, &views_dev, s));
    const SelfViews sv{reinterpret_cast<const AttnView*>(views_dev), V, N, 4.0 * V * (double)N * N * C, nullptr};

    const void* w;
    M3R_OK(w16(c, "encoder.patch_embed.proj.weight", dt, &w, s));
    M3R_OK(gemm(c, dt, EPI_F32, gargs(P16, w, p32(c, "encoder.patch_embed.proj.bias"), b.x, R, C, 768, 768, C), s));
    for (int l = 0; l < g.enc_depth; ++l) {
        const std::vector<Param*>& LP = c->enc_tab[l];
        M3R_OK(self_attention_sublayer(c, dt, LP, b, sv, fold, f256 && l > 0, nullptr, nullptr, s));
        M3R_OK(mlp_sublayer(c, dt, LP, LF_N2W, b, fold, f256 && l + 1 < g.enc_depth, nullptr, s));
    }
    return layernorm_a(c, dt, lnargs(b.x, nullptr, p32(c, "encoder.norm_enc.weight"), p32(c, "encoder.norm_enc.bias"), nullptr, nullptr,
                     out_tokens, nullptr, R, C, 1e-6f), s);
}

extern "C" int must3r_hip_encode(must3r_hip_ctx* c, int dtype, const float* img, int n_views, int H, int W,
                                 float* out_tokens, int64_t* out_pos, void* stream) {
    if (!c || !img || !out_tokens || !out_pos) return fail("encode: null argument");
    if (!c->fin_enc) return fail("encode: encoder weights not finalized");
    if ((dtype & MUST3R_ATTN_FP8) && !kAttnFp8Built) return fail("encode: MUST3R_ATTN_FP8 is an experiment build (make EXTRA=-DM3R_ATTN_FP8): measured outside the 1e-3 target for +0.4 %%");
    if (!set_mode(c, dtype)) return fail("encode: bad dtype %d", dtype & ~MUST3R_ATTN_FP8);
    if (n_views <= 0) return 0;
    if (H <= 0 || W <= 0 || H % 16 || W % 16) return fail("encode: H=%d W=%d must be positive multiples of 16", H, W);
    if (H / 16 > c->rope_npos || W / 16 > c->rope_npos) return fail("encode: image too large for the RoPE table");
    DeviceGuard dev_guard(c->device);
    hipStream_t s = reinterpret_cast<hipStream_t>(stream);
    const int N = (H / 16) * (W / 16);
    const int chunk_rows = opt(OPT_ENC_CHUNK_ROWS);
    int per = chunk_rows / N;
    if (per < 1) per = 1;
    {
        const int nch = (n_views + per - 1) / per;
        per = (n_views + nch - 1) / nch;
    }
    for (int v0 = 0; v0 < n_views; v0 += per) {
        const int nv = (n_views - v0 < per) ? n_views - v0 : per;
        M3R_OK(encode_chunk(c, c->dt, img +(size_t)v0 * 3 * H * W, nv, H, W, out_tokens + (size_t)v0 * N * c->cfg.enc_dim,
                            out_pos + (size_t)v0 * N * 2, s));
    }
    return 0;
}

struct Decode {
    must3r_hip_ctx* c; const must3r_hip_decode_args* A; void* stream; hipStream_t s; DType dt; bool a8;
    int C, D, Hh, F, L, Nm, mode;
    int S, Rs, R, total_views, max_n; long long mem_stride; std::vector<int> grow0; bool one_block;
    bool update, use_mask, lone_view, need_pre_kv, lnf, lnf_all, f256;
    const must3r_hip_cp* cp;
    int max_nk_ca, ca_split, memD; size_t split_bytes, memRB, kvs_rows1, kvs_rows, kv16_rows;
    BlockRows b; Fold fold;
    uint16_t *t16, *hcat, *q16, *yall, *kvs, *ytmp, *kv16; float *newmem, *off32; char* split_ws; uint8_t* kvs8;
    std::vector<AttnView> tab; SelfViews sv; const AttnView* ca_views; double ca_flops; void* const* kvout;
};

static void decode_plan(Decode& d) {
    must3r_hip_ctx* c = d.c; const must3r_hip_decode_args* A = d.A;
    const must3r_hip_config& g = c->cfg;
    d.dt = c->dt;
    d.a8 = kAttnFp8Built && c->attn8 != 0;
    d.C = g.enc_dim; d.D = g.dec_dim; d.Hh = g.dec_heads; d.F = g.mlp_ratio * g.dec_dim; d.L = g.dec_depth; d.Nm = A->n_mem; d.mode = A->mem_mode;
    const int D = d.D, F = d.F, Nm = d.Nm;
    const int S = d.S = A->n_scenes > 1 ? A->n_scenes : 1;
    d.mem_stride = S > 1 ? A->mem_scene_stride : 0;
    int Rs = 0, views_s = 0;
    d.max_n = 0;
    d.grow0.resize(A->n_groups);
    for (int gi = 0; gi < A->n_groups; ++gi) {
        const must3r_hip_group& G = A->groups[gi];
        d.grow0[gi] = Rs;
        Rs += G.n_views * G.n_tokens;
        views_s += G.n_views;
        if (G.n_tokens > d.max_n) d.max_n = G.n_tokens;
    }
    const int R = S * Rs;
    d.Rs = Rs; d.R = R; d.total_views = S * views_s;
    d.one_block = A->n_groups == 1;
    const bool update = d.update = !A->render;
    d.cp = A->cp;
    const int Nm_global = d.cp ? d.cp->n_mem_total : Nm;
    d.use_mask = update && (Nm_global > 0 || views_s > 1);
    d.lone_view = update && views_s == 1 && Nm_global > 0;
    d.need_pre_kv = update && !d.lone_view;
    d.lnf = opt(OPT_LNFOLD) != 0 && update && !d.need_pre_kv && c->wsplit == 2 && d.dt == DT_F16 && !d.a8 && !A->feats && A->n_groups == 1 &&
            S == 1 && D == 768 && F % 96 == 0;
    d.f256 = !d.lnf && opt(OPT_LNFOLD256) != 0 && c->wsplit == 2 && c->mlp_plain && d.dt == DT_F16 && !d.a8 && !A->feats && !A->cp && (D == 768 || D == 1024) &&
             gemm_fold256_shape_ok(R, 3 * D, D, true) && gemm_fold256_shape_ok(R, D, D, true) &&
             gemm_fold256_shape_ok(R, F, D, false) && gemm_fold256_shape_ok(R, D, F, false);
    d.lnf_all = d.lnf && opt(OPT_LNFOLD) == 2;
    d.max_nk_ca = A->render ? Nm : Nm + (d.lone_view ? 0 : Rs);
    d.ca_split = attention_pick_split(d.total_views, d.Hh, d.max_n, d.max_nk_ca);
    if (d.cp) d.ca_split = Nm > 0 ? (d.ca_split > 2 ? d.ca_split : 2) : 0;
    d.split_bytes = attention_split_scratch_bytes(d.ca_split, R, d.Hh);
    d.memD = d.mode == MUST3R_MEM_KV ? 2 * D : D;
    d.memRB = (d.a8 && d.mode == MUST3R_MEM_KV) ? (size_t)3 * D : (size_t)d.memD * 2;
    d.kvs_rows1 = d.mode == MUST3R_MEM_KV ? 0 : (size_t)d.max_nk_ca;
    d.kvs_rows = d.kvs_rows1 * S;
    d.kv16_rows = (d.a8 && d.mode == MUST3R_MEM_KV && update) ? (size_t)d.L * R : 0;
}

static int decode_workspace(Decode& d) {
    const size_t R = d.R, D = d.D, L = d.L;
    const bool update = d.update, lnF = d.lnf || d.f256, a8 = d.a8;
    d.b = BlockRows{d.R, d.D, d.Hh, d.F, nullptr, nullptr, nullptr, nullptr, nullptr, nullptr, d.A->groups[0].pos};
    d.fold.f256 = d.f256;
    Workspace ws;
    ws.want(d.t16, R * d.C);
    ws.want(d.b.x, R * D);
    ws.want(d.b.h16, R * D);
    ws.want(d.hcat, R * 3 * D);
    ws.want(d.b.qkv, R * 3 * D);
    ws.want(d.q16, R * D);
    ws.want(d.b.a16, R * D);
    ws.want(d.b.g16, R * d.F);
    ws.want(d.newmem, update ? L * R * D : 0);
    ws.want(d.off32, update ? R * D : 0);
    ws.want(d.yall, update ? L * R * D : 0);
    ws.want(d.fold.x16, lnF ? R * D : 0);
    ws.want(d.fold.stats, lnF ? R * (D / 16) * 2 : 0);
    ws.want(d.fold.shift, lnF ? R : 0);
    ws.want(d.split_ws, d.split_bytes);
    ws.want(d.kvs, d.kvs_rows * 2 * D);
    ws.want(d.ytmp, d.mode == MUST3R_MEM_RAW ? d.kvs_rows * D : 0);
    ws.want(d.b.q8, a8 ? R * 2 * D : 0);
    ws.want(d.kv16, d.kv16_rows * 2 * D);
    ws.want(d.kvs8, a8 ? d.kvs_rows * D : 0);
    M3R_OK(ws.commit(d.c, d.s));
    if (d.f256) HIP_OK(hipMemsetAsync(d.fold.shift, 0, R * sizeof(float), d.s));
    return 0;
}

static int decode_tables(Decode& d) {
    const must3r_hip_decode_args* A = d.A;
    const int S = d.S, Rs = d.Rs, Nm = d.Nm, D = d.D, L = d.L, total_views = d.total_views;
    d.tab.resize(2 * (size_t)total_views);
    double sa_flops = 0;
    d.ca_flops = 0;
    const long long kv_stride = d.mode == MUST3R_MEM_KV ? d.mem_stride : (long long)d.kvs_rows1;
    int vi = 0;
    for (int b = 0; b < S; ++b)
        for (int gi = 0; gi < A->n_groups; ++gi) {
            const must3r_hip_group& G = A->groups[gi];
            for (int j = 0; j < G.n_views; ++j, ++vi) {
                const int rl = d.grow0[gi] + j * G.n_tokens, n = G.n_tokens;
                const int r0 = b * Rs + rl;
                d.tab[vi] = AttnView{r0, n, r0, n, 0, 0};
                AttnView cv{r0, n, (int)(b * kv_stride), Nm, 0, 0};
                if (d.update) {
                    if (d.lone_view) { cv.nk = Nm; }
                    else if (d.use_mask && A->causal) {
                        if (Nm == 0 && j == 0) { cv.nk = 2 * n; cv.skip_lo = 0; cv.skip_hi = n; }
                        else { cv.nk = Nm + rl; }
                    }
                    else if (d.use_mask) { cv.nk = Nm + Rs; cv.skip_lo = Nm + rl; cv.skip_hi = Nm + rl + n; }
                    else { cv.nk = Nm + Rs; }
                }
                d.tab[total_views + vi] = cv;
                sa_flops += 4.0 * n * (double)n * D;
                d.ca_flops += 4.0 * n * (double)(cv.nk - (cv.skip_hi - cv.skip_lo)) * D;
            }
        }
    void* tab_dev = nullptr;
    M3R_OK(upload_table(d.c, d.tab.data(), sizeof(AttnView) * d.tab.size(), &tab_dev, d.s));
    const AttnView* sa_views = reinterpret_cast<const AttnView*>(tab_dev);
    d.ca_views = sa_views + total_views;
    d.sv = SelfViews{sa_views, total_views, d.max_n, sa_flops, total_views == 1 ? &d.tab[0] : nullptr};

    void* kvout_dev = nullptr;
    if (d.update && d.mode == MUST3R_MEM_KV) {
        std::vector<void*> outs(2 * (size_t)L * S);
        for (int l = 0; l < L; ++l)
            for (int b = 0; b < S; ++b) {
                void* memrow = reinterpret_cast<char*>(A->mem[l]) + ((size_t)b * d.mem_stride + Nm) * d.memRB;
                outs[(size_t)l * S + b] = d.a8 ? static_cast<void*>(d.kv16 + ((size_t)l * S + b) * Rs * 2 * D) : memrow;
                outs[(size_t)L * S + (size_t)l * S + b] = memrow;
            }
        M3R_OK(upload_table(d.c, outs.data(), sizeof(void*) * outs.size(), &kvout_dev, d.s));
    }
    d.kvout = reinterpret_cast<void* const*>(kvout_dev);
    return 0;
}

static int decode_embed(Decode& d) {
    must3r_hip_ctx* c = d.c; const must3r_hip_decode_args* A = d.A; hipStream_t s = d.s;
    const int S = d.S, Rs = d.Rs, C = d.C, D = d.D;
    const char* err = "";
    for (int b = 0; b < (d.one_block ? 1 : S); ++b)
        for (int gi = 0; gi < A->n_groups; ++gi) {
            const must3r_hip_group& G = A->groups[gi];
            const size_t rg = (size_t)G.n_views * G.n_tokens;
            ProfScope ps(c, s, PC_MISC, 0.0);
            if (launch_cast(d.dt, G.tokens + (size_t)b * rg * C, d.t16 + ((size_t)b * Rs + d.grow0[gi]) * C, nullptr, (d.one_block ? S : 1) * rg * C, s, &err))
                return fail("%s", err);
        }
    const void* w;
    M3R_OK(w16(c, "decoder.feat_embed_enc_to_dec.weight", d.dt, &w, s));
    GemmArgs ga = gargs(d.t16, w, p32(c, "decoder.feat_embed_enc_to_dec.bias"), d.b.x, d.R, D, C, C, D);
    ga.bias2 = p32(c, "decoder.image2_embed");
    ga.row_start2 = A->first_call ? A->groups[0].n_tokens : 0;
    ga.row_period2 = S > 1 ? Rs : 0;
    if (d.lnf_all) { ga.x16_out = d.fold.x16; ga.stats_out = d.fold.stats; ga.copy32_out = d.newmem; }
    M3R_OK(gemm(c, d.dt, EPI_F32, ga, s));
    if (!d.one_block) {
        int64_t* pos_ws = reinterpret_cast<int64_t*>(d.t16);
        for (int b = 0; b < S; ++b)
            for (int gi = 0; gi < A->n_groups; ++gi) {
                const must3r_hip_group& G = A->groups[gi];
                const size_t rg = (size_t)G.n_views * G.n_tokens;
                HIP_OK(hipMemcpyAsync(pos_ws + ((size_t)b * Rs + d.grow0[gi]) * 2, G.pos + (size_t)b * rg * 2, rg * 16, hipMemcpyDeviceToDevice, s));
            }
        d.b.pos = pos_ws;
    }
    return 0;
}

static int kv_project(Decode& d, int l, const float* src, const float* add, float* copy) {
    must3r_hip_ctx* c = d.c; const must3r_hip_decode_args* A = d.A; hipStream_t s = d.s;
    const int S = d.S, Rs = d.Rs, R = d.R, D = d.D, Nm = d.Nm;
    const std::vector<Param*>& LP = c->dec_tab[l];
    if (d.mode != MUST3R_MEM_KV) {
        for (int b = 0; b < S; ++b) {
            uint16_t* dst = reinterpret_cast<uint16_t*>(A->mem[l]) + ((size_t)b * d.mem_stride + Nm) * d.memD;
            const size_t o = (size_t)b * Rs * D;
            LnArgs la = lnargs(src + o, add ? add + o : nullptr, LP[LF_NYW]->d, LP[LF_NYB]->d, nullptr, nullptr, nullptr, copy ? copy + o : nullptr, Rs, D, 1e-6f);
            if (d.mode == MUST3R_MEM_NORM_Y) la.out16 = dst; else la.raw16 = dst;
            M3R_OK(layernorm_a(c, d.dt, la, s));
        }
        return 0;
    }
    M3R_OK(layernorm_a(c, d.dt, lnargs(src, add, LP[LF_NYW]->d, LP[LF_NYB]->d, d.b.h16, nullptr, nullptr, copy, R, D, 1e-6f), s));
    const void* wk;
    M3R_OK(w16p(c, *LP[LF_PKVW], d.dt, &wk, s));
    GemmArgs gk = gargs(d.b.h16, wk, LP[LF_PKVB]->d, nullptr, Rs, 2 * D, D, D, 2 * D);
    gk.batch = S; gk.strideA = (long long)Rs * D; gk.out_table = d.kvout + (size_t)l * S;
    if (S == 1) { gk.batch = 0; gk.out_table = nullptr; gk.out = d.a8 ? static_cast<void*>(d.kv16) : reinterpret_cast<char*>(A->mem[l]) + (size_t)Nm * d.memRB; }
    M3R_OK(gemm(c, d.dt, EPI_STORE16, gk, s));
    if (!d.a8) return 0;
    return quant8(c, d.dt, d.kv16 + (size_t)l * S * Rs * 2 * D * (S > 1 ? 1 : 0), 2 * D, S == 1 ? reinterpret_cast<char*>(A->mem[l]) + (size_t)Nm * d.memRB : nullptr,
                  3 * D, S > 1 ? d.kvout + (size_t)d.L * S + (size_t)l * S : nullptr, Rs, (size_t)R, D, D, s);
}
static int kv_source(Decode& d, int l, const void** kptr) {
    must3r_hip_ctx* c = d.c; hipStream_t s = d.s;
    const int D = d.D, rows = (int)d.kvs_rows1;
    if (d.mode == MUST3R_MEM_KV) { *kptr = d.A->mem[l]; return 0; }
    const std::vector<Param*>& LP = c->dec_tab[l];
    const void* wk;
    M3R_OK(w16p(c, *LP[LF_PKVW], d.dt, &wk, s));
    for (int b = 0; b < d.S; ++b) {
        const uint16_t* src = reinterpret_cast<const uint16_t*>(d.A->mem[l]) + (size_t)b * d.mem_stride * D;
        if (d.mode == MUST3R_MEM_RAW) {
            LnArgs la = lnargs(nullptr, nullptr, LP[LF_NYW]->d, LP[LF_NYB]->d, d.ytmp, nullptr, nullptr, nullptr, rows, D, 1e-6f);
            la.x16 = src;
            M3R_OK(layernorm_a(c, d.dt, la, s));
            src = d.ytmp;
        }
        M3R_OK(gemm(c, d.dt, EPI_STORE16, gargs(src, wk, LP[LF_PKVB]->d, d.kvs + (size_t)b * rows * 2 * D, rows, 2 * D, D, D, 2 * D), s));
    }
    *kptr = d.kvs;
    if (d.a8) M3R_OK(quant8(c, d.dt, d.kvs, 2 * D, d.kvs8, D, nullptr, 0, (size_t)d.kvs_rows, D, 0, s));
    return 0;
}

static int cross_attention_cp(Decode& d, int l, AttnArgs& aa) {
    must3r_hip_ctx* c = d.c; hipStream_t s = d.s; const must3r_hip_cp* cp = d.cp;
    const int R = d.R, p16 = cp->partial16 ? 1 : 0;
    const char* err = "";
    char* const slot0 = reinterpret_cast<char*>(cp->slots);
    const size_t o_bytes = (size_t)R * d.D * (p16 ? 2 : 4);
    float* const my_o = reinterpret_cast<float*>(slot0 + (size_t)cp->rank * cp->slot_bytes);
    float* const my_ml = reinterpret_cast<float*>(slot0 + (size_t)cp->rank * cp->slot_bytes + o_bytes);
    if (d.Nm > 0) {
        {
            ProfScope ps(c, s, PC_ATTN_CA, d.ca_flops);
            if (launch_attention_phase(d.dt, aa, 1, s, &err)) return fail("%s", err);
            ps.kernel(attention_last_kernel(), "/cross");
        }
        ProfScope ps(c, s, PC_ATTN_COMBINE, 0.0);
        aa.total_q_rows = R;
        if (launch_attention_partial_merge(d.dt, aa, my_o, my_ml, p16, s, &err)) return fail("%s", err);
    } else {
        ProfScope ps(c, s, PC_ATTN_COMBINE, 0.0);
        if (launch_attention_partial_empty(my_o, my_ml, R, d.Hh, p16, s, &err)) return fail("%s", err);
    }
    if (cp->exchange(cp->user, l, cp->slots, cp->slot_bytes, cp->world, cp->rank, d.stream))
        return fail("decode: the context-parallel exchange of layer %d failed", l);
    ProfScope ps(c, s, PC_ATTN_COMBINE, 0.0);
    aa.total_q_rows = R;
    if (launch_attention_partial_final(d.dt, aa, reinterpret_cast<const float*>(slot0), reinterpret_cast<const float*>(slot0 + o_bytes),
                                       (long long)(cp->slot_bytes / (p16 ? 2 : 4)), (long long)(cp->slot_bytes / 4), cp->world, p16, s, &err)) return fail("%s", err);
    return 0;
}

static int cross_attention_sublayer(Decode& d, int l) {
    must3r_hip_ctx* c = d.c; hipStream_t s = d.s; const DType dt = d.dt;
    const BlockRows& b = d.b;
    const std::vector<Param*>& LP = c->dec_tab[l];
    const int R = d.R, D = d.D;
    const bool folded = d.fold.on();
    const void* w;
    if (!folded) M3R_OK(layernorm_a(c, dt, lnargs(b.x, nullptr, LP[LF_N2W]->d, LP[LF_N2B]->d, b.h16, nullptr, nullptr, nullptr, R, D, 1e-6f), s));
    M3R_OK(w16p(c, *LP[folded ? LF_PQLN_W : LF_PQW], dt, &w, s));
    GemmArgs gq = gargs(b.h16, w, LP[LF_PQB]->d, d.q16, R, D, D, D, D);
    if (folded) d.fold.in(gq, LP[LF_PQLN_S], LP[LF_PQLN_C]);
    gq.out_scale = kQScale; gq.scale_cols = D;
    M3R_OK(gemm(c, dt, EPI_STORE16, gq, s));
    const void* mk = nullptr;
    M3R_OK(kv_source(d, l, &mk));
    AttnArgs aa;
    memset(&aa, 0, sizeof(aa));
    aa.Q = d.q16; aa.K = mk; aa.V = reinterpret_cast<const uint16_t*>(mk) + D; aa.O = b.a16;
    aa.ldq = D; aa.ldk = aa.ldv = 2 * D; aa.ldo = D; aa.heads = d.Hh;
    if (d.a8) {
        M3R_OK(quant8(c, dt, d.q16, D, b.q8, D, nullptr, 0, (size_t)R, D, 0, s));
        aa.Q = b.q8; aa.fp8 = 1;
        if (d.mode == MUST3R_MEM_KV) { aa.ldk = 3 * D; aa.ldv = 3 * D / 2; aa.V = reinterpret_cast<const char*>(mk) + D; }
        else { aa.K = d.kvs8; aa.ldk = D; }
    }
    aa.max_nk = d.max_nk_ca;
    aa.views = d.ca_views; aa.nviews = d.total_views; aa.max_nq = d.max_n; aa.scale = 0.125f; aa.q_prescaled = 1;
    if (d.total_views == 1) { aa.view0_inline = 1; aa.view0 = d.tab[d.total_views]; }
    if (d.ca_split > 1) {
        aa.nsplit = d.ca_split; aa.total_q_rows = R; aa.dense_rows = 1;
        aa.part_o = reinterpret_cast<float*>(d.split_ws);
        aa.part_ml = aa.part_o + (size_t)d.ca_split * R * D;
    }
    if (d.cp) M3R_OK(cross_attention_cp(d, l, aa));
    else M3R_OK(attention(c, dt, aa, d.ca_flops, PC_ATTN_CA, s));
    M3R_OK(w16p(c, *LP[LF_CPW], dt, &w, s));
    GemmArgs gp = gargs(b.a16, w, LP[LF_CPB]->d, b.x, R, D, D, D, D);
    if (folded) d.fold.out(gp, nullptr);
    return gemm(c, dt, EPI_RESID_F32, gp, s);
}

static int decode_head(Decode& d) {
    must3r_hip_ctx* c = d.c; const must3r_hip_decode_args* A = d.A;
    const int S = d.S, R = d.R, D = d.D, OUT = c->cfg.patch_size * c->cfg.patch_size * 7;
    M3R_OK(head_layernorm(c, d.dt, d.b.x, p32(c, "decoder.norm_dec.weight"), p32(c, "decoder.norm_dec.bias"), d.hcat,
                          A->feats ? A->feats + (size_t)(d.L - 1) * R * D : nullptr, R, D, 1e-6f, d.s));
    const void* wcat;
    M3R_OK(w3(c, "decoder.head_dec.proj_ps.weight", d.dt, &wcat, d.s));
    for (int b = 0; b < (d.one_block ? 1 : S); ++b)
        for (int gi = 0; gi < A->n_groups; ++gi) {
            const must3r_hip_group& G = A->groups[gi];
            const int rg = G.n_views * G.n_tokens;
            const int Rg = d.one_block ? S * rg : rg;
            const size_t scene_elems = (size_t)G.n_views * G.H * G.W * 7;
            const size_t scene_stride = G.pointmaps_scene_stride > 0 ? (size_t)G.pointmaps_scene_stride : scene_elems;
            const bool skip = d.one_block && scene_stride != scene_elems;
            M3R_OK(head_linear(c, d.dt, d.hcat + ((size_t)b * d.Rs + d.grow0[gi]) * 3 * D, wcat, p32(c, "decoder.head_dec.proj_ps.bias"),
                               G.pointmaps + (size_t)b * scene_stride, Rg, D, OUT, G.n_tokens, G.W / 16, G.H, G.W, skip ? G.n_views : 0,
                               skip ? (long long)(scene_stride - scene_elems) : 0, d.s));
        }
    return 0;
}

static int decode_feedback_memory(Decode& d) {
    must3r_hip_ctx* c = d.c; hipStream_t s = d.s; const DType dt = d.dt;
    const int S = d.S, Rs = d.Rs, R = d.R, D = d.D, L = d.L;
    uint16_t* const h16 = d.b.h16;
    const void* w;
    const bool fb_mlp = is_loaded(c, "decoder.feedback_layer.fc1.weight");
    const bool fb_lin = !fb_mlp && is_loaded(c, "decoder.feedback_layer.weight");
    float* const off32 = (fb_mlp || fb_lin) ? d.off32 : nullptr;
    if (fb_mlp || fb_lin)
        M3R_OK(layernorm_a(c, dt, lnargs(d.newmem + (size_t)(L - 1) * R * D, nullptr, p32(c, "decoder.feedback_norm.weight"),
                         p32(c, "decoder.feedback_norm.bias"), h16, nullptr, nullptr, nullptr, R, D, 1e-5f), s));
    if (fb_mlp) {
        int ws_fb;
        M3R_OK(wmlp(c, c->params.at("decoder.feedback_layer.fc1.weight"), dt, &w, &ws_fb, s));
        M3R_OK(gemm(c, dt, EPI_STORE16_GELU, gargs(h16, w, p32(c, "decoder.feedback_layer.fc1.bias"), d.b.g16, R, 4 * D, D, D, 4 * D), s, ws_fb));
        M3R_OK(wmlp(c, c->params.at("decoder.feedback_layer.fc2.weight"), dt, &w, &ws_fb, s));
        M3R_OK(gemm(c, dt, EPI_F32, gargs(d.b.g16, w, p32(c, "decoder.feedback_layer.fc2.bias"), off32, R, D, 4 * D, 4 * D, D), s, ws_fb));
    } else if (fb_lin) {
        M3R_OK(w16(c, "decoder.feedback_layer.weight", dt, &w, s));
        M3R_OK(gemm(c, dt, EPI_F32, gargs(h16, w, p32(c, "decoder.feedback_layer.bias"), off32, R, D, D, D, D), s));
    }
    if (d.mode != MUST3R_MEM_KV) {
        for (int l = 0; l < L; ++l)
            M3R_OK(kv_project(d, l, d.newmem + (size_t)l * R * D, l < L - 1 ? off32 : nullptr, nullptr));
        return 0;
    }
    LnArgs la = lnargs(d.newmem, off32, p32(c, "decoder.norm_y_all.weight"), p32(c, "decoder.norm_y_all.bias"), d.yall, nullptr,
                       nullptr, nullptr, L * R, D, 1e-6f);
    la.rows_per_group = R; la.add_groups = L - 1;
    M3R_OK(layernorm_a(c, dt, la, s));
    const void* wk;
    M3R_OK(w16(c, "decoder.projkv_all.weight", dt, &wk, s));
    GemmArgs gk = gargs(d.yall, wk, p32(c, "decoder.projkv_all.bias"), nullptr, Rs, 2 * D, D, D, 2 * D);
    gk.batch = L * S; gk.wdiv = S; gk.strideA = (long long)Rs * D; gk.strideW = (long long)2 * D * D * (c->wsplit == 2 ? 2 : 1);
    gk.strideB = 2 * D; gk.out_table = d.kvout;
    M3R_OK(gemm(c, dt, EPI_STORE16, gk, s));
    if (d.a8) M3R_OK(quant8(c, dt, d.kv16, 2 * D, nullptr, 3 * D, d.kvout + (size_t)L * S, Rs, (size_t)L * R, D, D, s));
    return 0;
}

static int decode_impl(must3r_hip_ctx* c, const must3r_hip_decode_args* A, void* stream) {
    DeviceGuard dev_guard(c->device);
    if (c->dec_tab.empty()) build_layer_tables(c, true);
    Decode d; d.c = c; d.A = A; d.stream = stream; d.s = reinterpret_cast<hipStream_t>(stream);
    decode_plan(d);
    M3R_OK(decode_workspace(d));
    M3R_OK(decode_tables(d));
    M3R_OK(decode_embed(d));
    const size_t RD = (size_t)d.R * d.D;
    for (int l = 0; l < d.L; ++l) {
        const std::vector<Param*>& LP = c->dec_tab[l];
        if (d.need_pre_kv) M3R_OK(kv_project(d, l, d.b.x, nullptr, nullptr));
        const bool fq = d.lnf_all || (d.fold.on() && l > 0);
        M3R_OK(self_attention_sublayer(c, d.dt, LP, d.b, d.sv, d.fold, fq, d.update ? d.newmem + l * RD : nullptr, d.lnf ? d.fold.shift : nullptr, d.s));
        M3R_OK(cross_attention_sublayer(d, l));
        M3R_OK(mlp_sublayer(c, d.dt, LP, LF_N3W, d.b, d.fold, d.fold.on() && l + 1 < d.L, d.update ? d.newmem + (l + 1) * RD : nullptr, d.s));
        if (A->feats && l < d.L - 1)
            HIP_OK(hipMemcpyAsync(A->feats + l * RD, d.b.x, RD * sizeof(float), hipMemcpyDeviceToDevice, d.s));
    }
    M3R_OK(decode_head(d));
    return d.update ? decode_feedback_memory(d) : 0;
}

extern "C" int must3r_hip_has_fp8_attention(void) { return kAttnFp8Built ? 1 : 0; }

static size_t cp_slot_bytes(const must3r_hip_ctx* c, int rows, int partial16) {
    return align_up((size_t)rows * ((size_t)c->cfg.dec_dim * (partial16 ? 2 : 4) + 2 * (size_t)c->cfg.dec_heads * sizeof(float)), 256);
}
extern "C" size_t must3r_hip_cp_slot_bytes(const must3r_hip_ctx* c, int rows) {
    if (!c || rows <= 0) return 0;
    return cp_slot_bytes(c, rows, 0);
}
extern "C" size_t must3r_hip_cp_slot_bytes16(const must3r_hip_ctx* c, int rows) {
    if (!c || rows <= 0) return 0;
    return cp_slot_bytes(c, rows, 1);
}

extern "C" int must3r_hip_decode(must3r_hip_ctx* c, const must3r_hip_decode_args* A, void* stream) {
    if (!c || !A || !A->groups || !A->mem) return fail("decode: null argument");
    if (!c->fin_dec) return fail("decode: decoder weights not finalized");
    if (!set_mode(c, A->dtype)) return fail("decode: bad dtype %d", A->dtype);
    if ((A->dtype & MUST3R_ATTN_FP8) && !kAttnFp8Built) return fail("decode: MUST3R_ATTN_FP8 is an experiment build (make EXTRA=-DM3R_ATTN_FP8): measured outside the 1e-3 target for +0.4 %%");
    if (A->mem_mode != MUST3R_MEM_KV && A->mem_mode != MUST3R_MEM_NORM_Y && A->mem_mode != MUST3R_MEM_RAW)
        return fail("decode: bad mem_mode %d", A->mem_mode);
    if (A->n_groups <= 0) return fail("decode: no input group");
    if (A->n_mem < 0) return fail("decode: negative n_mem");
    if (A->render && (A->first_call || A->n_mem <= 0)) return fail("decode: render needs a memory (decoder.py:278)");
    if (A->first_call && A->n_mem != 0) return fail("decode: first_call with a non-empty memory");
    if (A->n_scenes < 0) return fail("decode: negative n_scenes");
    const int S = A->n_scenes > 1 ? A->n_scenes : 1;
    if (A->causal != 0 && A->causal != 1) return fail("decode: causal must be 0 or 1");
    if (A->causal && (A->n_groups != 1 || A->cp)) return fail("decode: the causal forward takes ONE group of views (CausalMUSt3R has no list dispatch) and no context parallelism");
    if (A->cp) {
        const must3r_hip_cp& P = *A->cp;
        if (P.world < 1 || P.rank < 0 || P.rank >= P.world) return fail("decode: context parallel: bad rank %d of %d", P.rank, P.world);
        if (A->render || A->first_call || S != 1 || A->n_groups != 1 || A->groups[0].n_views != 1)
            return fail("decode: context parallel is for memory-update calls of ONE view on ONE scene against an existing memory");
        if (A->mem_mode != MUST3R_MEM_KV || (A->dtype & MUST3R_ATTN_FP8)) return fail("decode: context parallel needs memory_mode 'kv' and 16-bit attention operands");
        if (P.n_mem_total <= 0 || A->n_mem > P.n_mem_total) return fail("decode: context parallel: n_mem_total %d with %d local rows", P.n_mem_total, A->n_mem);
        if (P.partial16 != 0 && P.partial16 != 1) return fail("decode: context parallel: partial16 must be 0 or 1");
        if (!P.exchange || !P.slots || (reinterpret_cast<uintptr_t>(P.slots) & 15) || (P.slot_bytes & 15) ||
            P.slot_bytes < cp_slot_bytes(c, A->groups[0].n_tokens, P.partial16))
            return fail("decode: context parallel: slots must be 16-byte aligned, world x slot_bytes with slot_bytes >= %zu, and an exchange function given",
                        cp_slot_bytes(c, A->groups[0].n_tokens, P.partial16));
    }
    long long Rs = 0, views_s = 0;
    for (int gi = 0; gi < A->n_groups; ++gi) {
        const must3r_hip_group& G = A->groups[gi];
        if (!G.tokens || !G.pos || !G.pointmaps) return fail("decode: null buffer in group %d", gi);
        if (G.n_views <= 0 || G.n_tokens <= 0) return fail("decode: empty group %d", gi);
        if (G.pointmaps_scene_stride != 0 && G.pointmaps_scene_stride < (long long)G.n_views * G.H * G.W * 7)
            return fail("decode: group %d: pointmaps_scene_stride %lld is smaller than one scene's pointmaps", gi, (long long)G.pointmaps_scene_stride);
        if (G.pointmaps_scene_stride % 4 != 0 || (reinterpret_cast<uintptr_t>(G.pointmaps) & 15) != 0)
            return fail("decode: group %d: pointmaps must be 16-byte aligned and pointmaps_scene_stride (%lld) a multiple of 4 floats", gi, (long long)G.pointmaps_scene_stride);
        if (G.H % 16 || G.W % 16 || (G.H / 16) * (G.W / 16) != G.n_tokens)
            return fail("decode: group %d: %dx%d does not give %d tokens", gi, G.H, G.W, G.n_tokens);
        if (G.H / 16 > c->rope_npos || G.W / 16 > c->rope_npos) return fail("decode: group %d: image too large for the RoPE table", gi);
        Rs += (long long)G.n_views * G.n_tokens;
        views_s += G.n_views;
    }
    for (int l = 0; l < c->cfg.dec_depth; ++l)
        if (!A->mem[l]) return fail("decode: null memory buffer for layer %d", l);
    const long long rows_needed = (long long)A->n_mem + (A->render ? 0 : Rs);
    if (A->mem_capacity <= 0) return fail("decode: mem_capacity must be given (rows each scene's memory buffer can hold)");
    if (rows_needed > A->mem_capacity)
        return fail("decode: memory buffers hold %d rows, this call needs %lld (n_mem %d + %lld new)", A->mem_capacity, rows_needed, A->n_mem,
                    A->render ? 0LL : Rs);
    if (S > 1 && A->mem_scene_stride < A->mem_capacity)
        return fail("decode: mem_scene_stride %lld < mem_capacity %d", (long long)A->mem_scene_stride, A->mem_capacity);
    if ((S - 1) * (S > 1 ? (long long)A->mem_scene_stride : 0) + rows_needed > 0x7fffffffLL || (long long)S * Rs > (1LL << 24))
        return fail("decode: call too large (row indices are 32-bit)");
    {
        const long long memD = A->mem_mode == MUST3R_MEM_KV ? 2LL * c->cfg.dec_dim : 1LL * c->cfg.dec_dim;
        if (rows_needed * 2LL * c->cfg.dec_dim * 2 >= 0x7fffffffLL || rows_needed * memD * 2 >= 0x7fffffffLL)
            return fail("decode: a scene memory of %lld rows exceeds the 2 GiB the attention staging can address per layer", rows_needed);
    }
    const long long max_views = (long long)(must3r_hip_ctx::kSlotBytes / (2 * sizeof(AttnView)));
    if (!A->render && A->mem_mode == MUST3R_MEM_KV && (size_t)2 * c->cfg.dec_depth * S * sizeof(void*) > must3r_hip_ctx::kSlotBytes)
        return fail("decode: %d scenes in one memory update (limit %zu at decoder depth %d)", S,
                    must3r_hip_ctx::kSlotBytes / (2 * sizeof(void*) * c->cfg.dec_depth), c->cfg.dec_depth);
    if (S * views_s <= max_views) return decode_impl(c, A, stream);
    if (!A->render) return fail("decode: %lld views in one memory update (limit %lld)", S * views_s, max_views);
    if (A->feats) return fail("decode: return_feats with %lld rendered views in one call (limit %lld)", S * views_s, max_views);
    must3r_hip_decode_args sub = *A;
    if (S > 1) {
        const int per = views_s <= max_views ? (int)(max_views / views_s) : 1;
        std::vector<must3r_hip_group> gs(A->n_groups);
        std::vector<void*> mems(c->cfg.dec_depth);
        const long long memRB = ((A->dtype & MUST3R_ATTN_FP8) && A->mem_mode == MUST3R_MEM_KV) ? 3LL * c->cfg.dec_dim
                                : (A->mem_mode == MUST3R_MEM_KV ? 4LL : 2LL) * c->cfg.dec_dim;
        for (int b0 = 0; b0 < S; b0 += per) {
            const int nb = S - b0 < per ? S - b0 : per;
            for (int gi = 0; gi < A->n_groups; ++gi) {
                gs[gi] = A->groups[gi];
                const size_t rg = (size_t)gs[gi].n_views * gs[gi].n_tokens;
                gs[gi].tokens += (size_t)b0 * rg * c->cfg.enc_dim;
                gs[gi].pos += (size_t)b0 * rg * 2;
                gs[gi].pointmaps += (size_t)b0 * (gs[gi].pointmaps_scene_stride > 0 ? (size_t)gs[gi].pointmaps_scene_stride
                                                                                       : (size_t)gs[gi].n_views * gs[gi].H * gs[gi].W * 7);
            }
            for (int l = 0; l < c->cfg.dec_depth; ++l)
                mems[l] = reinterpret_cast<char*>(A->mem[l]) + (size_t)b0 * A->mem_scene_stride * memRB;
            sub.groups = gs.data(); sub.mem = mems.data(); sub.n_scenes = nb;
            M3R_OK(must3r_hip_decode(c, &sub, stream));
        }
        return 0;
    }
    for (int gi = 0; gi < A->n_groups; ++gi) {
        const must3r_hip_group& G = A->groups[gi];
        for (long long v0 = 0; v0 < G.n_views; v0 += max_views) {
            must3r_hip_group g1 = G;
            g1.n_views = (int)(G.n_views - v0 < max_views ? G.n_views - v0 : max_views);
            g1.tokens += (size_t)v0 * G.n_tokens * c->cfg.enc_dim;
            g1.pos += (size_t)v0 * G.n_tokens * 2;
            g1.pointmaps += (size_t)v0 * G.H * G.W * 7;
            sub.groups = &g1; sub.n_groups = 1;
            M3R_OK(decode_impl(c, &sub, stream));
        }
    }
    return 0;
}

extern "C" int must3r_hip_op_gemm(int dtype, int epi, const void* A, const void* W, const float* bias, void* out, int M, int N,
                                  int K, int lda, int ldc, const int64_t* pos, const float* rope_tab, int rope_cols,
                                  int rope_npos, const float* bias2, int row_start2, int accumulate, int ntok, int gw, int H,
                                  int W_img, int wsplit, void* stream) {
    if (dtype != MUST3R_BF16 && dtype != MUST3R_F16) return fail("op_gemm: bad dtype");
    if (epi < 0 || epi >= EPI_COUNT) return fail("op_gemm: bad epilogue");
    GemmArgs a = gargs(A, W, bias, out, M, N, K, lda, ldc);
    a.pos = pos; a.rope_tab = rope_tab; a.rope_cols = rope_cols; a.rope_npos = rope_npos;
    a.bias2 = bias2; a.row_start2 = row_start2; a.accumulate = accumulate;
    a.ntok = ntok; a.gw = gw; a.H = H; a.Wimg = W_img; a.wsplit = wsplit;
    const char* err = "";
    if (launch_gemm((DType)dtype, (Epi)epi, a, reinterpret_cast<hipStream_t>(stream), &err)) return fail("%s", err);
    return 0;
}

extern "C" int must3r_hip_op_sparse24_pack(const float* w, int rows, int K, void* vals, void* idx, void* stream) {
    const char* err = "";
    if (launch_sparse24_pack(w, rows, K, vals, idx, reinterpret_cast<hipStream_t>(stream), &err)) return fail("%s", err);
    return 0;
}
extern "C" int must3r_hip_op_gemm_fold256(int epi, int wsplit, const void* A, const void* W, const void* Wlo_sp, const void* Widx_sp, const float* bias, void* out,
                                          int M, int N, int K, int lda, int ldc, void* x16_out, float* copy32_out, float* stats_out, const float* ln_stats,
                                          const float* ln_s, float ln_eps, float* ln_shift, const int64_t* pos, const float* rope_tab, int rope_cols, int rope_npos,
                                          float out_scale, int scale_cols, void* stream) {
    if (epi < 0 || epi >= EPI_COUNT) return fail("op_gemm_fold256: bad epilogue");
    GemmArgs a = gargs(A, W, bias, out, M, N, K, lda, ldc);
    a.wsplit = wsplit == 2 ? 2 : 0; a.Wlo_sp = Wlo_sp; a.Widx_sp = Widx_sp; a.wsp_rows = N;
    a.x16_out = x16_out; a.copy32_out = copy32_out; a.stats_out = stats_out;
    a.ln_stats = ln_stats; a.ln_s = ln_s; a.ln_eps = ln_eps; a.ln_shift = ln_shift; a.fold256 = 1;
    a.pos = pos; a.rope_tab = rope_tab; a.rope_cols = rope_cols; a.rope_npos = rope_npos;
    a.out_scale = out_scale; a.scale_cols = scale_cols;
    const char* err = "";
    if (launch_gemm(DT_F16, (Epi)epi, a, reinterpret_cast<hipStream_t>(stream), &err)) return fail("%s", err);
    return 0;
}
extern "C" int must3r_hip_op_gemm_sp(int epi, const void* A, const void* W2, const void* Wlo_sp, const void* Widx_sp, const float* bias, void* out, int M,
                                     int N, int K, int lda, int ldc, const int64_t* pos, const float* rope_tab, int rope_cols, int rope_npos, void* stream) {
    if (epi < 0 || epi >= EPI_COUNT) return fail("op_gemm_sp: bad epilogue");
    GemmArgs a = gargs(A, W2, bias, out, M, N, K, lda, ldc);
    a.wsplit = 2; a.Wlo_sp = Wlo_sp; a.Widx_sp = Widx_sp; a.wsp_rows = N;
    a.pos = pos; a.rope_tab = rope_tab; a.rope_cols = rope_cols; a.rope_npos = rope_npos;
    const char* err = "";
    if (launch_gemm(DT_F16, (Epi)epi, a, reinterpret_cast<hipStream_t>(stream), &err)) return fail("%s", err);
    return 0;
}

extern "C" int must3r_hip_op_gemm_lnfold(int dtype, int epi, const void* A, const void* W2, const float* bias, void* out, int M, int N, int K,
                                         int lda, int ldc, void* x16_out, float* copy32_out, float* stats_out, const float* ln_stats,
                                         const float* ln_s, float ln_eps, float* ln_shift, int ln_shift_init, const int64_t* pos,
                                         const float* rope_tab, int rope_cols, int rope_npos, float out_scale, int scale_cols, void* stream) {
    if (dtype != MUST3R_F16) return fail("op_gemm_lnfold: fp16 operands with split weights only");
    if (epi < 0 || epi >= EPI_COUNT) return fail("op_gemm_lnfold: bad epilogue");
    GemmArgs a = gargs(A, W2, bias, out, M, N, K, lda, ldc);
    a.wsplit = 2;
    a.x16_out = x16_out; a.copy32_out = copy32_out; a.stats_out = stats_out;
    a.ln_stats = ln_stats; a.ln_s = ln_s; a.ln_eps = ln_eps; a.ln_shift = ln_shift; a.ln_shift_init = ln_shift_init;
    a.pos = pos; a.rope_tab = rope_tab; a.rope_cols = rope_cols; a.rope_npos = rope_npos;
    a.out_scale = out_scale; a.scale_cols = scale_cols;
    const char* err = "";
    if (launch_gemm(DT_F16, (Epi)epi, a, reinterpret_cast<hipStream_t>(stream), &err)) return fail("%s", err);
    return 0;
}

extern "C" int must3r_hip_op_gemm_lnfold_ex(const must3r_hip_lnfold_op* d, void* stream) {
    if (!d) return fail("op_gemm_lnfold_ex: null descriptor");
    if (d->dtype != MUST3R_F16) return fail("op_gemm_lnfold_ex: the fold is built for fp16 operands (dtype)");
    if (d->epi < 0 || d->epi >= EPI_COUNT) return fail("op_gemm_lnfold_ex: bad epilogue");
    if (d->wsplit != 0 && d->wsplit != 2) return fail("op_gemm_lnfold_ex: wsplit = %d (0: plain weights, 2: split weights)", d->wsplit);
    if (!d->A || !d->W || !d->out) return fail("op_gemm_lnfold_ex: A, W and out are needed");
    if (d->M < 0 || d->N <= 0 || d->K <= 0) return fail("op_gemm_lnfold_ex: M >= 0, N > 0 and K > 0 are needed");
    const bool cons = d->ln_stats != nullptr, prod = d->x16_out || d->copy32_out || d->stats_out;
    if (cons && prod) return fail("op_gemm_lnfold_ex: ln_stats (consumer) and x16_out / copy32_out / stats_out (producer) exclude each other");
    if (cons) {
        if (d->epi != EPI_STORE16 && d->epi != EPI_STORE16_GELU && d->epi != EPI_QKV_ROPE) return fail("op_gemm_lnfold_ex: a consumer has a 16-bit-store epilogue");
        if (!d->ln_s || !d->bias || !d->ln_shift) return fail("op_gemm_lnfold_ex: a consumer needs ln_s, bias and ln_shift");
        if (d->K != 768) return fail("op_gemm_lnfold_ex: a consumer reads 48 fragment sums per row (K = 768), not K = %d", d->K);
    }
    if (prod) {
        if (d->epi != EPI_RESID_F32 && d->epi != EPI_F32) return fail("op_gemm_lnfold_ex: producer outputs belong to the RESID_F32 / F32 epilogues");
        if (d->stats_out && !d->x16_out) return fail("op_gemm_lnfold_ex: stats_out comes with x16_out");
        if (d->stats_out && d->N != 768) return fail("op_gemm_lnfold_ex: stats_out needs N = 768, not N = %d", d->N);
        if (d->ldc != d->N) return fail("op_gemm_lnfold_ex: producer outputs are addressed with out's stride: ldc = %d must equal N = %d", d->ldc, d->N);
    }
    if (d->bias2 && d->epi != EPI_F32) return fail("op_gemm_lnfold_ex: bias2 belongs to EPI_F32");
    if (d->row_start2 < 0) return fail("op_gemm_lnfold_ex: row_start2 must not be negative");
    if (d->out_scale != 0.f && d->epi != EPI_STORE16 && d->epi != EPI_QKV_ROPE) return fail("op_gemm_lnfold_ex: out_scale belongs to the STORE16 / QKV_ROPE epilogues");
    if (d->out_scale != 0.f && (d->scale_cols < 0 || d->scale_cols % 64 != 0)) return fail("op_gemm_lnfold_ex: scale_cols = %d must be a multiple of 64", d->scale_cols);
    GemmArgs a = gargs(d->A, d->W, d->bias, d->out, d->M, d->N, d->K, d->lda, d->ldc);
    a.wsplit = d->wsplit;
    a.x16_out = d->x16_out; a.copy32_out = d->copy32_out; a.stats_out = d->stats_out;
    a.ln_stats = d->ln_stats; a.ln_s = d->ln_s; a.ln_eps = d->ln_eps; a.ln_shift = d->ln_shift; a.ln_shift_init = d->ln_shift_init;
    a.pos = d->pos; a.rope_tab = d->rope_tab; a.rope_cols = d->rope_cols; a.rope_npos = d->rope_npos;
    a.out_scale = d->out_scale; a.scale_cols = d->scale_cols;
    a.bias2 = d->bias2; a.row_start2 = d->row_start2;
    const char* err = "";
    if (launch_gemm(DT_F16, (Epi)d->epi, a, reinterpret_cast<hipStream_t>(stream), &err)) return fail("%s", err);
    if (d->picked && d->M > 0) *d->picked = gemm_last_kernel();
    return 0;
}

extern "C" int must3r_hip_op_gemm_ex(const must3r_hip_gemm_op* d, void* stream) {
    if (!d) return fail("op_gemm_ex: null descriptor");
    if (d->dtype != MUST3R_BF16 && d->dtype != MUST3R_F16) return fail("op_gemm_ex: bad dtype");
    if (d->epi < 0 || d->epi >= EPI_COUNT) return fail("op_gemm_ex: bad epilogue");
    if (!d->A || !d->W) return fail("op_gemm_ex: A and W are needed");
    if (d->M < 0 || d->N <= 0 || d->K <= 0) return fail("op_gemm_ex: M >= 0, N > 0 and K > 0 are needed");
    if (d->batch < 0 || d->wdiv < 0 || d->strideA < 0 || d->strideW < 0 || d->strideB < 0) return fail("op_gemm_ex: batch, wdiv and the strides must not be negative");
    if (d->batch > 1 && !d->out_table) return fail("op_gemm_ex: batch = %d needs out_table", d->batch);
    if (d->batch <= 1 && !d->out) return fail("op_gemm_ex: out is needed");
    if (d->wdiv > 1 && (d->batch <= 1 || d->batch % d->wdiv != 0)) return fail("op_gemm_ex: wdiv = %d must divide batch = %d", d->wdiv, d->batch);
    if (d->out_scale != 0.f && d->epi != EPI_STORE16 && d->epi != EPI_QKV_ROPE) return fail("op_gemm_ex: out_scale belongs to the STORE16 / QKV_ROPE epilogues");
    if (d->out_scale != 0.f && (d->scale_cols < 0 || d->scale_cols % 64 != 0)) return fail("op_gemm_ex: scale_cols = %d must be a multiple of 64", d->scale_cols);
    if (d->row_start2 < 0 || d->row_period2 < 0) return fail("op_gemm_ex: row_start2 and row_period2 must not be negative");
    if (d->row_period2 > 0 && !d->bias2) return fail("op_gemm_ex: row_period2 = %d needs bias2", d->row_period2);
    if ((d->head_views != 0 || d->head_scene_skip != 0) && d->epi != EPI_HEAD) return fail("op_gemm_ex: head_views / head_scene_skip belong to EPI_HEAD");
    if (d->head_views < 0 || d->head_scene_skip < 0) return fail("op_gemm_ex: head_views and head_scene_skip must not be negative");
    if (d->head_scene_skip % 4 != 0) return fail("op_gemm_ex: head_scene_skip = %lld must be a multiple of 4 floats", (long long)d->head_scene_skip);
    if ((d->Wlo_sp != nullptr) != (d->Widx_sp != nullptr)) return fail("op_gemm_ex: Wlo_sp and Widx_sp come together");
    if (d->Wlo_sp) {
        if (d->wsplit != 2 || d->dtype != MUST3R_F16) return fail("op_gemm_ex: the sparse low part belongs to fp16 split weights (wsplit = 2)");
        const long long ngroups = d->batch > 1 ? (d->wdiv > 1 ? d->batch / d->wdiv : d->batch) : 1;
        const long long need = (ngroups - 1) * (d->strideW / (2 * (long long)d->K)) + d->N;
        if (d->wsp_rows < need || d->wsp_rows % 32 != 0)
            return fail("op_gemm_ex: wsp_rows = %d, but the %lld weight groups index %lld rows of the packed low part (a multiple of 32)", d->wsp_rows, ngroups, need);
    }
    GemmArgs a = gargs(d->A, d->W, d->bias, d->out, d->M, d->N, d->K, d->lda, d->ldc);
    a.wsplit = d->wsplit == 2 ? 2 : 0; a.Wlo_sp = d->Wlo_sp; a.Widx_sp = d->Widx_sp; a.wsp_rows = d->wsp_rows;
    a.out_scale = d->out_scale; a.scale_cols = d->scale_cols;
    a.batch = d->batch; a.strideA = d->strideA; a.strideW = d->strideW; a.strideB = d->strideB; a.out_table = d->out_table; a.wdiv = d->wdiv;
    a.pos = d->pos; a.rope_tab = d->rope_tab; a.rope_cols = d->rope_cols; a.rope_npos = d->rope_npos;
    a.bias2 = d->bias2; a.row_start2 = d->row_start2; a.row_period2 = d->row_period2; a.accumulate = d->accumulate;
    a.ntok = d->ntok; a.gw = d->gw; a.H = d->H; a.Wimg = d->Wimg; a.head_views = d->head_views; a.head_scene_skip = d->head_scene_skip;
    const char* err = "";
    if (launch_gemm((DType)d->dtype, (Epi)d->epi, a, reinterpret_cast<hipStream_t>(stream), &err)) return fail("%s", err);
    if (d->picked && d->M > 0) *d->picked = gemm_last_kernel();
    return 0;
}

extern "C" size_t must3r_hip_attention_scratch_bytes(int nsplit, int total_q_rows, int heads) {
    return attention_split_scratch_bytes(nsplit, total_q_rows, heads);
}

extern "C" int must3r_hip_op_attention(int dtype, const void* Q, const void* K, const void* V, void* O, int ldq, int ldk, int ldv,
                                       int ldo, int heads, const int32_t* views_dev, int n_views, int max_nq, int nsplit,
                                       void* scratch, int total_q_rows, void* stream) {
    const int fp8 = (dtype & MUST3R_ATTN_FP8) ? 1 : 0;
    if (fp8 && !kAttnFp8Built) return fail("op_attention: MUST3R_ATTN_FP8 is an experiment build (make EXTRA=-DM3R_ATTN_FP8)");
    dtype &= ~MUST3R_ATTN_FP8;
    if (dtype != MUST3R_BF16 && dtype != MUST3R_F16) return fail("op_attention: bad dtype");
    AttnArgs a;
    memset(&a, 0, sizeof(a));
    a.fp8 = fp8;
    a.Q = Q; a.K = K; a.V = V; a.O = O; a.ldq = ldq; a.ldk = ldk; a.ldv = ldv; a.ldo = ldo; a.heads = heads;
// ... 121 lines not shown
```

### must3r_amd/csrc/options.hpp

```cpp
#pragma once

namespace m3r {

enum Opt {
    OPT_PERSIST = 0,
    OPT_GEMM256,
    OPT_G256K,
    OPT_G256P,
    OPT_G256P_SPLIT,
    OPT_SPARSE_256,
    OPT_SPARSE_LO,
    OPT_BK128,
    OPT_LN_ROWS,
    OPT_LNFOLD,
    OPT_ENC_CHUNK_ROWS,
    OPT_ATTN_LZ,
    OPT_LNFOLD256,
    OPT_G256_GM,
    OPT_NN_LEAF_LOG2,
    OPT_NN_QUERY_LANES_LOG2,
    OPT_COUNT
};

int opt(Opt o);
int opt_set(const char* name, long long value, const char** err);

}
```

### must3r_amd/engine.py

```python
import torch

from . import _lib
from .model import ActivationType


@torch.no_grad()
def postprocess(pointmaps, pointmaps_activation=ActivationType.NORM_EXP, compute_cam=False):
    if isinstance(pointmaps_activation, str):
        pointmaps_activation = ActivationType(pointmaps_activation)
    if pointmaps_activation not in (ActivationType.NORM_EXP, ActivationType.LINEAR):
        raise ValueError(f"Unknown activation: {pointmaps_activation}")
    if pointmaps.shape[-1] != 7:
        raise NotImplementedError("fused postprocess handles the 7-channel (pts3d, pts3d_local, conf) layout of the released models")
    act = _lib.ACT_LINEAR if pointmaps_activation == ActivationType.LINEAR else _lib.ACT_NORM_EXP
    if not pointmaps.is_cuda:
        raise RuntimeError("must3r_amd.postprocess: input is on CPU; the HIP path has no CPU fallback")
    pm = pointmaps.float().contiguous()
    lead = pm.shape[:-1]
    npix = pm.numel() // 7
    p3 = torch.empty((*lead, 3), dtype=torch.float32, device=pm.device)
    pl = torch.empty((*lead, 3), dtype=torch.float32, device=pm.device)
    cf = torch.empty(lead, dtype=torch.float32, device=pm.device)
    lib = _lib.load()
    stream = _lib.stream_ptr(pm.device)
    out = {"pts3d": p3, "pts3d_local": pl, "conf": cf}
    if not compute_cam:
        with torch.cuda.device(pm.device):
            _lib.check(lib.must3r_hip_postprocess_act(pm.data_ptr(), act, p3.data_ptr(), pl.data_ptr(), cf.data_ptr(), npix, stream))
        return out
    if pm.dim() < 3:
        raise ValueError("compute_cam needs pointmaps of shape [..., H, W, 7]")
    batch_dims = tuple(pm.shape[:-3])
    H, W = int(pm.shape[-3]), int(pm.shape[-2])
    n = npix // (H * W) if H * W else 0
    focal = torch.empty(batch_dims, dtype=torch.float32, device=pm.device)
    c2w = torch.empty((*batch_dims, 4, 4), dtype=torch.float32, device=pm.device)
    if n:
        with torch.cuda.device(pm.device):
            nbytes = lib.must3r_hip_postprocess_cam_scratch_bytes(n, H, W)
            scratch = torch.empty(nbytes, dtype=torch.uint8, device=pm.device)
            _lib.check(lib.must3r_hip_postprocess_cam_act(pm.data_ptr(), act, n, H, W, p3.data_ptr(), pl.data_ptr(), cf.data_ptr(),
                                                      focal.data_ptr(), c2w.data_ptr(), scratch.data_ptr(), nbytes, stream))
    out["focal"] = focal
    out["c2w"] = c2w
    return out


def demo_mem_batches(n_views, init_num_images=2, batch_num_views=1):
    if n_views <= init_num_images:
        return [n_views]
    rest = n_views - init_num_images
    out = [init_num_images] + [batch_num_views] * (rest // batch_num_views)
    if rest % batch_num_views:
        out.append(rest % batch_num_views)
    return out


@torch.no_grad()
def run_scene(encoder, decoder, imgs, true_shape, mem_batches=None, render_bs=None, activate=True, encoder_tokens=None):
    V = imgs.shape[0]
    if mem_batches is None:
        mem_batches = demo_mem_batches(V)
    true_shape = true_shape.cpu() if true_shape.is_cuda else true_shape
    x, pos = encoder_tokens if encoder_tokens is not None else encoder(imgs, true_shape)
    mem = None
    upd = []
    i = 0
    if imgs.is_cuda and hasattr(decoder, "reserve_memory_tokens"):
        decoder.reserve_memory_tokens = sum(mem_batches) * ((imgs.shape[-2] // 16) * (imgs.shape[-1] // 16))
    for nb in mem_batches:
        mem, pm = decoder(x[i:i + nb].unsqueeze(0), pos[i:i + nb].unsqueeze(0), true_shape[i:i + nb].unsqueeze(0), mem)
        upd.append(pm[0])
        i += nb
    ren = []
    bs = render_bs or V
    for v0 in range(0, V, bs):
        _, pm = decoder(x[v0:v0 + bs].unsqueeze(0), pos[v0:v0 + bs].unsqueeze(0), true_shape[v0:v0 + bs].unsqueeze(0), mem,
                        render=True)
        ren.append(pm[0])
    out = {"update": torch.cat(upd, dim=0), "render": torch.cat(ren, dim=0), "mem": mem, "x": x, "pos": pos}
    if activate:
        out.update(postprocess(out["render"]))
    return out


@torch.no_grad()
def run_scenes(encoder, decoder, imgs, true_shape, mem_batches=None, activate=True, encoder_tokens=None):
    S, V = int(imgs.shape[0]), int(imgs.shape[1])
    if mem_batches is None:
        mem_batches = demo_mem_batches(V)
    true_shape = true_shape.cpu() if true_shape.is_cuda else true_shape
    if encoder_tokens is not None:
        x, pos = encoder_tokens
    else:
        x, pos = encoder(imgs.reshape(S * V, *imgs.shape[2:]), true_shape.repeat(S, 1))
    x = x.view(S, V, *x.shape[1:])
    pos = pos.view(S, V, *pos.shape[1:])
    ts = true_shape.unsqueeze(0).expand(S, -1, -1)
    if hasattr(decoder, "reserve_memory_tokens"):
        decoder.reserve_memory_tokens = sum(mem_batches) * ((imgs.shape[-2] // 16) * (imgs.shape[-1] // 16))
    strided = bool(getattr(decoder, "_ctx", "x") != "x") and imgs.is_cuda
    H, W = int(imgs.shape[-2]), int(imgs.shape[-1])
    upd_all = torch.empty((S, sum(mem_batches), H, W, 7), dtype=torch.float32, device=imgs.device) if strided else None
    mem, upd, i = None, [], 0
    for nb in mem_batches:
        if strided:
            mem, pm = decoder(x[:, i:i + nb], pos[:, i:i + nb], ts[:, i:i + nb], mem, pointmaps_out=upd_all[:, i:i + nb])
        else:
            mem, pm = decoder(x[:, i:i + nb], pos[:, i:i + nb], ts[:, i:i + nb], mem)
            upd.append(pm)
        i += nb
    _, ren = decoder(x, pos, ts, mem, render=True)
    out = {"update": upd_all if strided else torch.cat(upd, dim=1), "render": ren, "mem": mem, "x": x, "pos": pos}
    if activate:
        out.update(postprocess(out["render"]))
    return out


@torch.no_grad()
def run_scene_mixed(encoder, decoder, img_groups, mem_batches=None, activate=True):
    dev = img_groups[0].device
    enc = []
    for g in img_groups:
        n, _, H, W = g.shape
        ts = torch.tensor([[H, W]] * n, dtype=torch.int64)
        x, pos = encoder(g, ts)
        enc.append((x, pos, ts))
    owner = [(gi, j) for gi, g in enumerate(img_groups) for j in range(g.shape[0])]
    V = len(owner)
    if mem_batches is None:
        mem_batches = demo_mem_batches(V)
    if hasattr(decoder, "reserve_memory_tokens"):
        decoder.reserve_memory_tokens = sum(int(enc[gi][0].shape[1]) for gi, _ in owner[:sum(mem_batches)])
    mem, upd, i = None, [], 0
    for nb in mem_batches:
        batch = owner[i:i + nb]
        gids = sorted({gi for gi, _ in batch})
        xs, ps, tss = [], [], []
        for gi in gids:
            js = [j for g2, j in batch if g2 == gi]
            x, pos, ts = enc[gi]
            xs.append(x[js[0]:js[-1] + 1].unsqueeze(0))
            ps.append(pos[js[0]:js[-1] + 1].unsqueeze(0))
            tss.append(ts[js[0]:js[-1] + 1].unsqueeze(0))
        if len(gids) == 1:
            mem, pm = decoder(xs[0], ps[0], tss[0], mem)
            pms = [pm]
        else:
            mem, pms = decoder(xs, ps, tss, mem)
        for pm in pms:
            upd += [pm[0, k] for k in range(pm.shape[1])]
        i += nb
    _, ren = decoder([e[0].unsqueeze(0) for e in enc], [e[1].unsqueeze(0) for e in enc], [e[2].unsqueeze(0) for e in enc], mem,
                     render=True)
    out = {"update": upd, "render": [r[0] for r in ren], "mem": mem}
    if activate:
        pp = [postprocess(r) for r in out["render"]]
        for k in ("pts3d", "pts3d_local", "conf"):
            out[k] = [p[k] for p in pp]
    return out


@torch.no_grad()
def run_scenes_mixed(encoder, decoder, img_groups, mem_batches=None, activate=True):
    S = int(img_groups[0].shape[0])
    enc = []
    for g in img_groups:
        _, n, _, H, W = g.shape
        ts = torch.tensor([[H, W]] * n, dtype=torch.int64)
        x, pos = encoder(g.reshape(S * n, 3, H, W), ts.repeat(S, 1))
        enc.append((x.view(S, n, *x.shape[1:]), pos.view(S, n, *pos.shape[1:]), ts.unsqueeze(0).expand(S, -1, -1)))
    owner = [(gi, j) for gi, g in enumerate(img_groups) for j in range(g.shape[1])]
    V = len(owner)
    if mem_batches is None:
        mem_batches = demo_mem_batches(V)
    if hasattr(decoder, "reserve_memory_tokens"):
        decoder.reserve_memory_tokens = sum(int(enc[gi][0].shape[2]) for gi, _ in owner[:sum(mem_batches)])
    mem, upd, i = None, [], 0
    for nb in mem_batches:
        batch = owner[i:i + nb]
        gids = sorted({gi for gi, _ in batch})
        xs, ps, tss = [], [], []
        for gi in gids:
            js = [j for g2, j in batch if g2 == gi]
            x, pos, ts = enc[gi]
            xs.append(x[:, js[0]:js[-1] + 1].contiguous())
            ps.append(pos[:, js[0]:js[-1] + 1].contiguous())
            tss.append(ts[:, js[0]:js[-1] + 1])
        if len(gids) == 1:
            mem, pm = decoder(xs[0], ps[0], tss[0], mem)
            pms = [pm]
        else:
            mem, pms = decoder(xs, ps, tss, mem)
        for pm in pms:
            upd += [pm[:, k] for k in range(pm.shape[1])]
        i += nb
    _, ren = decoder([e[0] for e in enc], [e[1] for e in enc], [e[2] for e in enc], mem, render=True)
    out = {"update": upd, "render": list(ren), "mem": mem}
    if activate:
        pp = [postprocess(r) for r in out["render"]]
        for k in ("pts3d", "pts3d_local", "conf"):
            out[k] = [p[k] for p in pp]
    return out


def _label_runs(mem_labels):
    runs = getattr(mem_labels, "_m3r_runs", None)
    if runs is None or mem_labels.dim() != 2 or mem_labels.shape[0] != 1 or sum(c for _, c in runs) != mem_labels.shape[1]:
        return None
    if getattr(mem_labels, "_m3r_runs_version", None) != mem_labels._version:
        return None
    return runs


def attach_label_runs(mem_labels, runs):
    mem_labels._m3r_runs = runs
    mem_labels._m3r_runs_version = mem_labels._version
    return mem_labels


def _ranges_of(runs, idx):
    out, off = [], 0
    for lab, cnt in runs:
        if lab == idx:
            out.append((off, off + cnt))
        off += cnt
    return out


def remove_from_mem(mem_values, mem_labels, idx):
    B, Nm, D = mem_values[0].shape
    owner = getattr(mem_values[0], "_m3r_owner", None)
    in_place = (B == 1 and owner is not None and owner.valid == Nm
                and all(getattr(v, "_m3r_owner", None) is owner for v in mem_values))
    runs = _label_runs(mem_labels)
    if runs is not None:
        drop = _ranges_of(runs, idx)
        new_runs = [(lab, cnt) for lab, cnt in runs if lab != idx]
        if not drop:
            return mem_values, mem_labels
        first = drop[0][0]
        tail, off = [], 0
        for lab, cnt in runs:
            if lab != idx and off >= first:
                tail.append(torch.arange(off, off + cnt))
            off += cnt
        n = sum(c for _, c in new_runs)
        dev = mem_labels.device
        tail_idx = (torch.cat(tail) if tail else torch.zeros(0, dtype=torch.int64)).to(dev, non_blocking=True)
        if in_place:
            if n > first:
                for b in owner.bufs:
                    b[:, first:n] = b[:, tail_idx]
            owner.valid = n
            vals = owner.views(n)
        else:
            vals = [torch.cat([v[:, :first], v[:, tail_idx]], dim=1) for v in mem_values]
        labels = torch.cat([mem_labels[:, :first], mem_labels[:, tail_idx]], dim=1)
        attach_label_runs(labels, new_runs)
        return vals, labels
    keep = mem_labels != idx
    if not in_place:
        return [v[keep].view(B, -1, D) for v in mem_values], mem_labels[keep].view(B, -1)
    kept = keep[0].nonzero().flatten()
    n = int(kept.numel())
# ... 76 lines not shown
```

### must3r_amd/model/decoder.py

```python
import ctypes as C
from functools import partial

import torch
import torch.nn as nn

from .. import _lib
from ..config import ModelConfig
from .blocks import (ActivationType, DecBlockParams, LinearHeadParams, MlpParams, MEMORY_MODES, init_weights,
                     parse_pos_embed)
from ._hip_module import HipModule, operand_dtype, autocast_dtype, _DT, _TORCH_DT

_MEM_MODE = {"kv": _lib.MEM_KV, "norm_y": _lib.MEM_NORM_Y, "raw": _lib.MEM_RAW}


class _MemBuffers:

    def __init__(self, depth, cap, mem_D, dtype, device, batch=1):
        self.bufs = [torch.empty((batch, cap, mem_D), dtype=dtype, device=device) for _ in range(depth)]
        self.cap = cap
        self.batch = batch
        self.valid = 0

    def views(self, n):
        out = []
        for b in self.bufs:
            v = b[:, :n]
            v._m3r_owner = self
            out.append(v)
        return out


class MUSt3R(HipModule):
    _part = _lib.PART_DECODER
    _prefix = "decoder."

    def __init__(self, img_size=(224, 224), enc_embed_dim=1024, patch_size=16, embed_dim=768, output_dim=1792,
                 depth=12, num_heads=12, mlp_ratio=4, norm_layer=partial(nn.LayerNorm, eps=1e-6), act_layer=nn.GELU,
                 pos_embed="RoPE100", landscape_only=True, head="Linear", feedback_type=None, memory_mode="norm_y",
                 pointmaps_activation=ActivationType.NORM_EXP, block_type=None, precision="fp16wa", **kv):
        super().__init__()
        if isinstance(img_size, int):
            img_size = (img_size, img_size)
        assert memory_mode in MEMORY_MODES
        if head != "Linear":
            raise ValueError(f"invalid head {head}")
        if feedback_type not in ("single_mlp", "single_linear", None, "", False):
            raise ValueError(f"Unknown {feedback_type=}")
        assert output_dim == patch_size * patch_size * 7
        self.pointmaps_activation = pointmaps_activation
        self.depth = depth
        self.embed_dim = embed_dim
        self.memory_mode = memory_mode
        self.attn_num_heads = num_heads
        self.feedback_type = feedback_type
        self.reserve_memory_tokens = 0
        self.landscape_only = landscape_only
        self.max_seq_len = max(img_size) // patch_size
        self.grid_size = (img_size[0] // patch_size, img_size[1] // patch_size)
        freq, f0 = parse_pos_embed(pos_embed)
        self.feat_embed_enc_to_dec = nn.Linear(enc_embed_dim, embed_dim, bias=True)
        self.image2_embed = nn.Parameter(torch.zeros(1, 1, embed_dim))
        self.blocks_dec = nn.ModuleList([DecBlockParams(embed_dim, mlp_ratio, memory_mode) for _ in range(depth)])
        if feedback_type == "single_mlp":
            self.feedback_layer = MlpParams(embed_dim, 4 * embed_dim, embed_dim)
            self.feedback_norm = nn.LayerNorm(embed_dim)
        elif feedback_type == "single_linear":
            self.feedback_layer = nn.Linear(embed_dim, embed_dim)
            self.feedback_norm = nn.LayerNorm(embed_dim)
        else:
            self.feedback_layer = None
            self.feedback_norm = None
        self.norm_dec = nn.LayerNorm(embed_dim, eps=1e-6)
        self.head_dec = LinearHeadParams(embed_dim, output_dim, patch_size)
        init_weights(self)
        torch.nn.init.normal_(self.image2_embed, std=0.02)
        if feedback_type == "single_mlp":
            nn.init.constant_(self.feedback_layer.fc2.bias, 0)
            nn.init.constant_(self.feedback_layer.fc2.weight, 0)
        elif feedback_type == "single_linear":
            nn.init.constant_(self.feedback_layer.bias, 0)
            nn.init.constant_(self.feedback_layer.weight, 0)
        self._hip_init(ModelConfig(img_size=max(img_size), patch_size=patch_size, enc_dim=enc_embed_dim,
                                   enc_heads=enc_embed_dim // 64, dec_dim=embed_dim, dec_depth=depth, dec_heads=num_heads,
                                   mlp_ratio=mlp_ratio, rope_freq=freq, rope_f0=f0), precision)

    def change_memory_mode(self, memory_mode="norm_y"):
        assert memory_mode in MEMORY_MODES
        for blk in self.blocks_dec:
            blk.memory_mode = memory_mode
        self.memory_mode = memory_mode

    def from_dust3r(self, state_dict, verbose=True, load_head=False):
        state_dict = {k.replace("dec_blocks.", "blocks_dec.").replace("decoder_embed.", "feat_embed_enc_to_dec.").replace(
            "dec_norm.", "norm_dec."): v for k, v in state_dict.items()}
        if load_head:
            state_dict = {k.replace("downstream_head.proj.", "head_dec.proj."): v for k, v in state_dict.items()}
        inc = self.load_state_dict(state_dict, strict=False)
        if verbose:
            print(inc)
        return inc

    def from_croco(self, state_dict, verbose=True):
        return self.from_dust3r(state_dict, verbose=verbose)

    def _operand(self):
        ac = autocast_dtype()
        if ac == torch.bfloat16:
            return _lib.BF16
        if ac == torch.float16 and self.precision == "bf16":
            return _lib.F16
        return operand_dtype(self.precision)

    def _writable_memory(self, mem_vals, Nm, R, tdt, device, B=1, mem_D=None):
        if mem_D is None:
            mem_D = 2 * self.embed_dim if self.memory_mode == "kv" else self.embed_dim
        owner = None
        if mem_vals is not None and len(mem_vals) == self.depth:
            owner = getattr(mem_vals[0], "_m3r_owner", None)
            ok = owner is not None and owner.valid == Nm and owner.cap >= Nm + R and owner.batch == B
            if ok:
                for v, b in zip(mem_vals, owner.bufs):
                    if getattr(v, "_m3r_owner", None) is not owner or v.data_ptr() != b.data_ptr() or v.dtype != tdt \
                            or v.shape[0] != B or v.shape[1] != Nm or v.shape[2] != mem_D or v.device != b.device:
                        ok = False
                        break
            if not ok:
                owner = None
        if owner is None:
            hint = int(getattr(self, "reserve_memory_tokens", 0) or 0) if Nm == 0 else 0
            if Nm == 0:
                self.reserve_memory_tokens = 0
            cap = max(Nm + R, 2 * Nm, 1024, hint)
            owner = _MemBuffers(self.depth, cap, mem_D, tdt, device, B)
            if Nm > 0:
                for v, b in zip(mem_vals, owner.bufs):
                    b[:, :Nm].copy_(v.reshape(B, Nm, mem_D))
        return owner

    def _check_memory_rows(self, mem_vals, mem_D, fp8_rows):
        for v in mem_vals:
            if fp8_rows:
                if v.dtype != torch.uint8 or int(v.shape[2]) != mem_D:
                    raise ValueError(f"attention_fp8 with memory_mode 'kv': the memory must be the uint8 [B, Nm, {mem_D}] rows an fp8-mode "
                                     f"update returned, got {v.dtype} [.., {int(v.shape[2])}] (a memory written with attention_fp8 off cannot "
                                     "be read with it on; re-run the update in this mode)")
            elif not v.dtype.is_floating_point or int(v.shape[2]) != mem_D:
                raise ValueError(f"memory_mode {self.memory_mode!r} without attention_fp8: the memory must be floating-point [B, Nm, {mem_D}] rows, "
                                 f"got {v.dtype} [.., {int(v.shape[2])}] (a memory written with attention_fp8 on holds opaque e4m3 | 16-bit bytes "
                                 "and cannot be read with it off; re-run the update in this mode)")

    @torch.no_grad()
    def forward(self, x, pos, true_shape, current_mem=None, render=False, return_feats=False, pointmaps_out=None, cp=None):
        is_list = isinstance(x, (list, tuple))
        if is_list:
            return_feats = False
        return self._forward(x, pos, true_shape, current_mem, render, return_feats, pointmaps_out, cp)

    def _forward(self, x, pos, true_shape, current_mem, render, return_feats, pointmaps_out=None, cp=None):
        is_list = isinstance(x, (list, tuple))
        xs = list(x) if is_list else [x]
        poss = list(pos) if is_list else [pos]
        shapes = list(true_shape) if is_list else [true_shape]
        B = int(xs[0].shape[0])
        assert all(int(t.shape[0]) == B for t in xs + poss), "all groups must share the batch size"
        pouts = None if pointmaps_out is None else (list(pointmaps_out) if isinstance(pointmaps_out, (list, tuple)) else [pointmaps_out])
        out, outs, feats = self._forward_scene(xs, poss, shapes, current_mem, render, return_feats, pouts, cp)
        if return_feats:
            return out, (outs if is_list else outs[0]), (feats if is_list else feats[0])
        return out, (outs if is_list else outs[0])

    def _forward_scene(self, xs, poss, shapes, current_mem, render, return_feats, pouts=None, cp=None):
        MAXV = 1024
        B = int(xs[0].shape[0])
        if render and return_feats and B == 1 and sum(int(x.shape[1]) for x in xs) > MAXV:
            outs, feats = [], []
            for xi, pi, ti in zip(xs, poss, shapes):
                pms, fts = [], []
                tsi = ti.reshape(1, -1, 2)
                for a in range(0, int(xi.shape[1]), MAXV):
                    _, o, f = self._forward_scene([xi[:, a:a + MAXV]], [pi[:, a:a + MAXV]], [tsi[:, a:a + MAXV]], current_mem, True,
                                                  return_feats)
                    pms.append(o[0])
                    fts.append(f[0] if f is not None else None)
                outs.append(torch.cat(pms, dim=1))
                feats.append([torch.cat([f[l] for f in fts], dim=1) for l in range(len(fts[0]))] if return_feats else None)
            return current_mem, outs, (feats if return_feats else None)
        ctx = self._context()
        dev = self._ctx_dev
        device = torch.device("cuda", dev)
        odt = self._operand()
        tdt = _TORCH_DT[odt]
        fp8_rows = self.attention_fp8 and self.memory_mode == "kv"
        if fp8_rows:
            tdt = torch.uint8
        D = self.embed_dim
        assert not render or current_mem is not None

        groups = (_lib.Group * len(xs))()
        keep = []
        outs = []
        R = 0
        nimgs, Ns = [], []
        for i, (xi, pi, ti) in enumerate(zip(xs, poss, shapes)):
            _, n, N, Cenc = xi.shape
            xi = self._check_input(xi, "x", torch.float32)
            pi = self._check_input(pi, "pos", torch.int64)
            ts = ti.reshape(-1, 2)
            if ts.is_cuda:
                ts = ts.cpu()
            assert bool((ts[0:1] == ts).all()), "true_shape must be all identical"
            H, W = (int(v) for v in ts[0].tolist())
            assert (H // 16) * (W // 16) == N, (H, W, N)
            sstride = 0
            if pouts is not None:
                pm = pouts[i]
                inner = n * H * W * 7
                if (not pm.is_cuda or pm.dtype != torch.float32 or tuple(pm.shape) != (B, n, H, W, 7) or pm.device != device
                        or tuple(pm.stride()[1:]) != (H * W * 7, W * 7, 7, 1) or (B > 1 and (pm.stride(0) < inner or pm.stride(0) % 4))
                        or pm.data_ptr() % 16):
                    raise ValueError(f"pointmaps_out[{i}]: need a fp32 cuda tensor [{B}, {n}, {H}, {W}, 7] with contiguous views, got {tuple(pm.shape)} "
                                     f"{pm.dtype} strides {tuple(pm.stride())}")
                sstride = int(pm.stride(0)) if B > 1 and int(pm.stride(0)) != inner else 0
            else:
                pm = torch.empty((B, n, H, W, 7), dtype=torch.float32, device=device)
            keep += [xi, pi]
            outs.append(pm)
            groups[i] = _lib.Group(xi.data_ptr(), pi.data_ptr(), n, N, H, W, pm.data_ptr(), sstride)
            R += n * N
            nimgs.append(n)
            Ns.append(N)

        if current_mem is None:
            mem_vals, mem_labels, mem_nimgs, mem_prot_imgs, mem_prot_tok = None, torch.zeros((B, 0), dtype=torch.int64,
                                                                                            device=device), 0, 0, 0
            Nm = 0
        else:
            mem_vals, mem_labels, mem_nimgs, mem_prot_imgs, mem_prot_tok = current_mem
            Nm = int(mem_vals[0].shape[1])
            assert all(int(v.shape[0]) == B for v in mem_vals), "memory and inputs must share the batch size"

        mem_D = (3 * D if fp8_rows else 2 * D) if self.memory_mode == "kv" else D
        if current_mem is not None:
            self._check_memory_rows(mem_vals, mem_D, fp8_rows)
        if render:
            vals, stride = [], None
            for v in mem_vals:
                if not v.is_cuda or v.dtype != tdt or v.stride(2) != 1 or v.stride(1) != mem_D or (B > 1 and v.stride(0) % mem_D):
                    v = v.to(device=device, dtype=tdt).contiguous()
                vals.append(v)
            if B > 1:
                strides = {int(v.stride(0)) // mem_D for v in vals}
                if len(strides) != 1 or min(strides) < Nm:
                    vals = [v.contiguous() for v in vals]
                stride = int(vals[0].stride(0)) // mem_D
            ptrs = (C.c_void_p * self.depth)(*[v.data_ptr() for v in vals])
            keep += vals
            cap, stride = Nm, (0 if B == 1 else stride)
        else:
            owner = self._writable_memory(mem_vals, Nm, R, tdt, device, B, mem_D)
            ptrs = (C.c_void_p * self.depth)(*[b.data_ptr() for b in owner.bufs])
            cap, stride = owner.cap, owner.cap

        feats_buf = torch.empty((self.depth, B, R, D), dtype=torch.float32, device=device) if return_feats else None
        cp_struct = None
        if cp is not None:
            if render or current_mem is None or B != 1 or len(xs) != 1 or nimgs[0] != 1 or self.memory_mode != "kv" or self.attention_fp8:
                raise ValueError("context-parallel cross attention is for one-view memory updates of one scene against an existing memory, memory_mode 'kv', "
                                 "16-bit attention operands")
            cp_struct = cp.native_args(ctx, R, device)
        args = _lib.DecodeArgs(odt | (_lib.ATTN_FP8 if self.attention_fp8 else 0), _MEM_MODE[self.memory_mode],
                               1 if render else 0, 1 if current_mem is None else 0,
                               len(xs), groups, Nm, ptrs, feats_buf.data_ptr() if return_feats else None,
                               cap, B, stride, C.pointer(cp_struct) if cp_struct is not None else None, 1 if self._causal else 0)
        rc = ctx.lib.must3r_hip_decode(ctx.handle, C.byref(args), _lib.stream_ptr(dev))
        if cp is not None and rc != 0:
            cp.reraise()
        _lib.check(rc)

        if render:
            out = current_mem
        else:
            owner.valid = Nm + R
            new_vals = owner.views(Nm + R)
            labels = []
            k = 0
            from ..engine import _label_runs, attach_label_runs
            runs = [] if Nm == 0 else _label_runs(mem_labels)
            runs = list(runs) if runs is not None and sum(c for _, c in runs) == Nm else None
            for n, N in zip(nimgs, Ns):
                labels.append((torch.arange(n, dtype=torch.int64, device=device) + (mem_nimgs + k)).repeat_interleave(N).view(1, -1)
                              .expand(B, -1))
                if runs is not None:
                    runs += [(mem_nimgs + k + j, N) for j in range(n)]
                k += n
            mem_labels = torch.cat([mem_labels.to(device)] + labels, dim=1)
            if runs is not None and B == 1:
                attach_label_runs(mem_labels, runs)
            tot = mem_nimgs + sum(nimgs)
            out = self._memory_tail(new_vals, mem_labels, tot, mem_prot_imgs, mem_prot_tok, sum(nimgs), Ns[0])
        feats = None
        if return_feats:
            feats, r0 = [], 0
            for xi, n, N in zip(xs, nimgs, Ns):
                feats.append([xi] + [feats_buf[l, :, r0:r0 + n * N].reshape(B, n, N, D) for l in range(self.depth)])
                r0 += n * N
        return out, outs, feats

    def forward_list(self, x, pos, true_shape, current_mem=None, render=False, return_feats=False):
        return self._forward(list(x), list(pos), list(true_shape), current_mem, render, return_feats)

    _causal = False

    def _memory_tail(self, vals, labels, n_imgs, prot_imgs, prot_tok, n_new, N):
        return (vals, labels, n_imgs, n_imgs, labels.shape[1])


class CausalMUSt3R(MUSt3R):

    _causal = True

    def __init__(self, protected_imgs=1, mem_dropout=0.0, dropout_mode="temporary", use_xformers_mask=False, use_mem_mask=False, **kv):
        if dropout_mode not in ("temporary", "permanent"):
            raise ValueError(f"Invalid dropout mode = {dropout_mode}")
        if float(mem_dropout) > 0.0:
            raise NotImplementedError("CausalMUSt3R(mem_dropout > 0) is the training-time random token dropout (decoder.py:470-485): not part of the forward path")
        super().__init__(**kv)
        self.protected_imgs = int(protected_imgs)
        self.dropout_mode = dropout_mode
        self.use_xformers_mask, self.use_mem_mask = bool(use_xformers_mask), bool(use_mem_mask)

    @torch.no_grad()
    def forward(self, x, pos, true_shape, current_mem=None, render=False, return_feats=False, pointmaps_out=None):
        if isinstance(x, (list, tuple)):
            raise TypeError("CausalMUSt3R.forward takes tensors [B, nimgs, N, C] (the reference's class has no list dispatch, decoder.py:435-439)")
        return self._forward(x, pos, true_shape, current_mem, render, return_feats, pointmaps_out)

    def forward_list(self, *a, **k):
        raise TypeError("CausalMUSt3R has no forward_list (decoder.py:352-553)")

    def _memory_tail(self, vals, labels, n_imgs, prot_imgs, prot_tok, n_new, N):
        prot = min(self.protected_imgs, int(prot_imgs) + int(n_new))
        return (vals, labels, n_imgs, prot, int(prot_tok) + (prot - int(prot_imgs)) * int(N))
```

Measured before the change: 537.0 views/s.

## Compute decoder block-0 prefix once per view and reuse across update and render

Adds a prefix pass that runs the decoder embedding plus block 0's self-attention and cross-attention query projection once per distinct view slot, storing x0, x1, q16 and positions. The memory-update and render decode calls then gather these rows through a chunk-gather kernel instead of recomputing embedding, self-attention and the query GEMM for block 0. This removes duplicated block-0 work, since each view is otherwise decoded twice (once for the update, once for the render). In exchange it adds buffers, gather copies and extra constraints: no LN fold, no fp8 attention, a single group, and no feats output.

After: 540.0 views/s (median of 6 runs). About the same (+0.6%).

```diff
diff --git a/include/must3r_hip.h b/include/must3r_hip.h
--- a/include/must3r_hip.h
+++ b/include/must3r_hip.h
@@ -76,7 +76,32 @@
     int64_t mem_scene_stride;
     const must3r_hip_cp* cp;
     int32_t causal;
+    const struct must3r_hip_prefix* prefix;
 } must3r_hip_decode_args;
+
+typedef struct must3r_hip_prefix_args {
+    int32_t dtype;
+    const float* tokens;
+    const int64_t* pos;
+    int32_t n_scenes, n_views, n_tokens;
+    int32_t n_slots;
+    const int32_t* slot_view;
+    const int32_t* slot_embed;
+    float* x0;
+    float* x1;
+    void* q16;
+    int64_t* pos_out;
+    void* stream;
+} must3r_hip_prefix_args;
+int must3r_hip_decode_prefix(must3r_hip_ctx* ctx, const must3r_hip_prefix_args* args);
+
+typedef struct must3r_hip_prefix {
+    const float* x0; const float* x1; const void* q16; const int64_t* pos;
+    int32_t n_slots, n_scenes, n_tokens;
+    const int32_t* view_slot;
+} must3r_hip_prefix;
+
+int must3r_hip_prefix_once(void);
 
 size_t must3r_hip_cp_slot_bytes(const must3r_hip_ctx* ctx, int rows);
 size_t must3r_hip_cp_slot_bytes16(const must3r_hip_ctx* ctx, int rows);
diff --git a/must3r_amd/_lib.py b/must3r_amd/_lib.py
--- a/must3r_amd/_lib.py
+++ b/must3r_amd/_lib.py
@@ -46,7 +46,19 @@
                 ("n_groups", C.c_int32), ("groups", C.POINTER(Group)), ("n_mem", C.c_int32),
                 ("mem", C.POINTER(C.c_void_p)), ("feats", C.c_void_p),
                 ("mem_capacity", C.c_int32), ("n_scenes", C.c_int32), ("mem_scene_stride", C.c_int64),
-                ("cp", C.POINTER(Cp)), ("causal", C.c_int32)]
+                ("cp", C.POINTER(Cp)), ("causal", C.c_int32), ("prefix", C.c_void_p)]
+
+
+class PrefixArgs(C.Structure):
+    _fields_ = [("dtype", C.c_int32), ("tokens", C.c_void_p), ("pos", C.c_void_p),
+                ("n_scenes", C.c_int32), ("n_views", C.c_int32), ("n_tokens", C.c_int32), ("n_slots", C.c_int32),
+                ("slot_view", C.POINTER(C.c_int32)), ("slot_embed", C.POINTER(C.c_int32)),
+                ("x0", C.c_void_p), ("x1", C.c_void_p), ("q16", C.c_void_p), ("pos_out", C.c_void_p), ("stream", C.c_void_p)]
+
+
+class Prefix(C.Structure):
+    _fields_ = [("x0", C.c_void_p), ("x1", C.c_void_p), ("q16", C.c_void_p), ("pos", C.c_void_p),
+                ("n_slots", C.c_int32), ("n_scenes", C.c_int32), ("n_tokens", C.c_int32), ("view_slot", C.POINTER(C.c_int32))]
 
 
 class ImageDesc(C.Structure):
@@ -261,6 +273,8 @@
     "must3r_hip_load_weight": (i32, [vp, cstr, vp, i32, i32, P(i64)]),
     "must3r_hip_finalize_weights": (i32, [vp, i32]),
     "must3r_hip_encode": (i32, [vp, i32, vp, i32, i32, i32, vp, vp, vp]),
+    "must3r_hip_decode_prefix": (i32, [vp, P(PrefixArgs)]),
+    "must3r_hip_prefix_once": (i32, []),
     "must3r_hip_cp_slot_bytes": (sz, [vp, i32]),
     "must3r_hip_cp_slot_bytes16": (sz, [vp, i32]),
     "must3r_hip_decode": (i32, [vp, P(DecodeArgs), vp]),
diff --git a/must3r_amd/csrc/kernels.hpp b/must3r_amd/csrc/kernels.hpp
--- a/must3r_amd/csrc/kernels.hpp
+++ b/must3r_amd/csrc/kernels.hpp
@@ -134,6 +134,13 @@
 
 int launch_im2col(DType dt, const float* img, void* out16, int V, int H, int W, hipStream_t s, const char** err);
 int launch_cast(DType dt, const float* in, void* out16, void* out16_lo, size_t n, hipStream_t s, const char** err);
+struct ChunkGatherArgs {
+    const int* table;
+    int nchunks;
+    const void* src[4]; void* dst[4]; unsigned units[4];
+    const float* cast_in; void* cast_out; unsigned cast_n4;
+};
+int launch_chunk_gather(DType dt, const ChunkGatherArgs& a, hipStream_t s, const char** err);
 int launch_quant8(DType dt, const void* in16, int ld_in, void* out8, int ld_out, void* const* out_table, int rows_per_group,
                   size_t rows, int cols, int tail_cols, hipStream_t s, const char** err);
 int launch_fill_pos(int64_t* pos, int V, int gh, int gw, hipStream_t s, const char** err);
diff --git a/must3r_amd/csrc/misc.hip b/must3r_amd/csrc/misc.hip
--- a/must3r_amd/csrc/misc.hip
+++ b/must3r_amd/csrc/misc.hip
@@ -13,6 +13,7 @@
     {"PERSIST", 0, 0, 1}, {"GEMM256", 1, 0, 2}, {"G256K", 1, 0, 2}, {"G256P", 1, 0, 1}, {"G256P_SPLIT", 1, 0, 2}, {"SPARSE_256", 1, 0, 1},
     {"SPARSE_LO", 1, 0, 1}, {"BK128", 1, 0, 1}, {"LN_ROWS", 1, 0, 1}, {"LNFOLD", 1, 0, 2}, {"ENC_CHUNK_ROWS", 32768, 256, 1 << 22}, {"ATTN_LZ", 1, 0, 2},
     {"LNFOLD256", 0, 0, 1}, {"G256_GM", 4, 1, 64}, {"NN_LEAF_LOG2", 5, 4, 6}, {"NN_QUERY_LANES_LOG2", 3, 0, 4},
+    {"PREFIX_ONCE", 1, 0, 1},
 };
 long long g_opt_val[OPT_COUNT];
 bool g_opt_init[OPT_COUNT];
@@ -300,6 +301,40 @@
     return launch_split16(dt, in, out16, out16_lo, n, s, err);
 }
 
+template <class T>
+__global__ void __launch_bounds__(256) chunk_gather_kernel(const ChunkGatherArgs p) {
+    typedef typename Vec<T>::v4 v4;
+    const size_t i = blockIdx.y, c = (size_t)p.table[i];
+    const unsigned t0 = blockIdx.x * blockDim.x + threadIdx.x, step = gridDim.x * blockDim.x;
+#pragma unroll
+    for (int k = 0; k < 4; ++k) {
+        if (!p.dst[k]) continue;
+        const uint4* src = reinterpret_cast<const uint4*>(p.src[k]) + c * p.units[k];
+        uint4* dst = reinterpret_cast<uint4*>(p.dst[k]) + i * p.units[k];
+        for (unsigned u = t0; u < p.units[k]; u += step) dst[u] = src[u];
+    }
+    if (p.cast_out) {
+        const f32x4* src = reinterpret_cast<const f32x4*>(p.cast_in) + c * p.cast_n4;
+        v4* dst = reinterpret_cast<v4*>(p.cast_out) + i * p.cast_n4;
+        for (unsigned u = t0; u < p.cast_n4; u += step) dst[u] = cvt4<T>(src[u]);
+    }
+}
+
+int launch_chunk_gather(DType dt, const ChunkGatherArgs& a, hipStream_t s, const char** err) {
+    if (a.nchunks <= 0) return 0;
+    if (a.nchunks > 65535) { *err = "chunk gather: more than 65535 chunks"; return 1; }
+    unsigned most = a.cast_out ? a.cast_n4 : 0;
+    for (int k = 0; k < 4; ++k)
+        if (a.dst[k] && a.units[k] > most) most = a.units[k];
+    if (!most) return 0;
+    unsigned bx = (most + 1023) / 1024;
+    if (bx > 64) bx = 64;
+    if (dt == DT_BF16) hipLaunchKernelGGL(chunk_gather_kernel<bf16_t>, dim3(bx, a.nchunks), dim3(256), 0, s, a);
+    else hipLaunchKernelGGL(chunk_gather_kernel<f16_t>, dim3(bx, a.nchunks), dim3(256), 0, s, a);
+    if (hipGetLastError() != hipSuccess) { *err = "chunk gather: launch failed"; return 1; }
+    return 0;
+}
+
 __global__ void sparse24_pack_kernel(const float* __restrict__ w, int rows, int K, f16_t* __restrict__ vals, unsigned short* __restrict__ idx) {
     const size_t total = (size_t)(K / 64) * rows * 4;
     for (size_t u = (size_t)blockIdx.x * blockDim.x + threadIdx.x; u < total; u += (size_t)gridDim.x * blockDim.x) {
diff --git a/must3r_amd/csrc/model.hip b/must3r_amd/csrc/model.hip
--- a/must3r_amd/csrc/model.hip
+++ b/must3r_amd/csrc/model.hip
@@ -799,6 +799,7 @@
 
 struct Decode {
     must3r_hip_ctx* c; const must3r_hip_decode_args* A; void* stream; hipStream_t s; DType dt; bool a8;
+    const must3r_hip_prefix* px;
     int C, D, Hh, F, L, Nm, mode;
     int S, Rs, R, total_views, max_n; long long mem_stride; std::vector<int> grow0; bool one_block;
     bool update, use_mask, lone_view, need_pre_kv, lnf, lnf_all, f256;
@@ -813,6 +814,7 @@
     must3r_hip_ctx* c = d.c; const must3r_hip_decode_args* A = d.A;
     const must3r_hip_config& g = c->cfg;
     d.dt = c->dt;
+    d.px = A->prefix;
     d.a8 = kAttnFp8Built && c->attn8 != 0;
     d.C = g.enc_dim; d.D = g.dec_dim; d.Hh = g.dec_heads; d.F = g.mlp_ratio * g.dec_dim; d.L = g.dec_depth; d.Nm = A->n_mem; d.mode = A->mem_mode;
     const int D = d.D, F = d.F, Nm = d.Nm;
@@ -969,6 +971,31 @@
     return 0;
 }
 
+static int decode_prefix_rows(Decode& d) {
+    must3r_hip_ctx* c = d.c; const must3r_hip_prefix& X = *d.px;
+    const int S = d.S, nv = d.A->groups[0].n_views, N = d.A->groups[0].n_tokens;
+    std::vector<int> chunk((size_t)S * nv);
+    for (int b = 0; b < S; ++b)
+        for (int j = 0; j < nv; ++j) chunk[(size_t)b * nv + j] = X.view_slot[j] * S + b;
+    void* tab = nullptr;
+    M3R_OK(upload_table(c, chunk.data(), sizeof(int) * chunk.size(), &tab, d.s));
+    int64_t* pos_ws = reinterpret_cast<int64_t*>(d.t16);
+    ChunkGatherArgs g;
+    memset(&g, 0, sizeof(g));
+    g.table = reinterpret_cast<const int*>(tab); g.nchunks = S * nv;
+    const unsigned row4 = (unsigned)((size_t)N * d.D / 4);
+    g.src[0] = X.x1; g.dst[0] = d.b.x; g.units[0] = row4;
+    g.src[1] = X.q16; g.dst[1] = d.q16; g.units[1] = row4 / 2;
+    g.src[2] = X.pos; g.dst[2] = pos_ws; g.units[2] = (unsigned)N;
+    if (d.update) { g.src[3] = X.x0; g.dst[3] = d.newmem; g.units[3] = row4; }
+    d.b.pos = pos_ws;
+    const char* err = "";
+    ProfScope ps(c, d.s, PC_MISC, 0.0);
+    if (launch_chunk_gather(d.dt, g, d.s, &err)) return fail("%s", err);
+    ps.kernel("prefix_gather");
+    return 0;
+}
+
 static int kv_project(Decode& d, int l, const float* src, const float* add, float* copy) {
     must3r_hip_ctx* c = d.c; const must3r_hip_decode_args* A = d.A; hipStream_t s = d.s;
     const int S = d.S, Rs = d.Rs, R = d.R, D = d.D, Nm = d.Nm;
@@ -1046,19 +1073,26 @@
     return 0;
 }
 
-static int cross_attention_sublayer(Decode& d, int l) {
+static int cross_attention_query(must3r_hip_ctx* c, DType dt, const std::vector<Param*>& LP, const BlockRows& b, Fold& fold, uint16_t* q16, hipStream_t s) {
+    const int R = b.R, D = b.C;
+    const bool folded = fold.on();
+    const void* w;
+    if (!folded) M3R_OK(layernorm_a(c, dt, lnargs(b.x, nullptr, LP[LF_N2W]->d, LP[LF_N2B]->d, b.h16, nullptr, nullptr, nullptr, R, D, 1e-6f), s));
+    M3R_OK(w16p(c, *LP[folded ? LF_PQLN_W : LF_PQW], dt, &w, s));
+    GemmArgs gq = gargs(b.h16, w, LP[LF_PQB]->d, q16, R, D, D, D, D);
+    if (folded) fold.in(gq, LP[LF_PQLN_S], LP[LF_PQLN_C]);
+    gq.out_scale = kQScale; gq.scale_cols = D;
+    return gemm(c, dt, EPI_STORE16, gq, s);
+}
+
+static int cross_attention_sublayer(Decode& d, int l, bool have_q) {
     must3r_hip_ctx* c = d.c; hipStream_t s = d.s; const DType dt = d.dt;
     const BlockRows& b = d.b;
     const std::vector<Param*>& LP = c->dec_tab[l];
     const int R = d.R, D = d.D;
     const bool folded = d.fold.on();
     const void* w;
-    if (!folded) M3R_OK(layernorm_a(c, dt, lnargs(b.x, nullptr, LP[LF_N2W]->d, LP[LF_N2B]->d, b.h16, nullptr, nullptr, nullptr, R, D, 1e-6f), s));
-    M3R_OK(w16p(c, *LP[folded ? LF_PQLN_W : LF_PQW], dt, &w, s));
-    GemmArgs gq = gargs(b.h16, w, LP[LF_PQB]->d, d.q16, R, D, D, D, D);
-    if (folded) d.fold.in(gq, LP[LF_PQLN_S], LP[LF_PQLN_C]);
-    gq.out_scale = kQScale; gq.scale_cols = D;
-    M3R_OK(gemm(c, dt, EPI_STORE16, gq, s));
+    if (!have_q) M3R_OK(cross_attention_query(c, dt, LP, b, d.fold, d.q16, s));
     const void* mk = nullptr;
     M3R_OK(kv_source(d, l, &mk));
     AttnArgs aa;
@@ -1154,16 +1188,19 @@
     if (c->dec_tab.empty()) build_layer_tables(c, true);
     Decode d; d.c = c; d.A = A; d.stream = stream; d.s = reinterpret_cast<hipStream_t>(stream);
     decode_plan(d);
+    if (d.px && (d.lnf || d.f256)) return fail("decode: a prefix cannot feed a call that takes the LN fold (its chain starts at block 0's norm1)");
     M3R_OK(decode_workspace(d));
     M3R_OK(decode_tables(d));
-    M3R_OK(decode_embed(d));
+    if (d.px) M3R_OK(decode_prefix_rows(d));
+    else M3R_OK(decode_embed(d));
     const size_t RD = (size_t)d.R * d.D;
     for (int l = 0; l < d.L; ++l) {
         const std::vector<Param*>& LP = c->dec_tab[l];
-        if (d.need_pre_kv) M3R_OK(kv_project(d, l, d.b.x, nullptr, nullptr));
+        const bool pre = d.px && l == 0;
+        if (d.need_pre_kv) M3R_OK(kv_project(d, l, pre ? d.newmem : d.b.x, nullptr, nullptr));
         const bool fq = d.lnf_all || (d.fold.on() && l > 0);
-        M3R_OK(self_attention_sublayer(c, d.dt, LP, d.b, d.sv, d.fold, fq, d.update ? d.newmem + l * RD : nullptr, d.lnf ? d.fold.shift : nullptr, d.s));
-        M3R_OK(cross_attention_sublayer(d, l));
+        if (!pre) M3R_OK(self_attention_sublayer(c, d.dt, LP, d.b, d.sv, d.fold, fq, d.update ? d.newmem + l * RD : nullptr, d.lnf ? d.fold.shift : nullptr, d.s));
+        M3R_OK(cross_attention_sublayer(d, l, pre));
         M3R_OK(mlp_sublayer(c, d.dt, LP, LF_N3W, d.b, d.fold, d.fold.on() && l + 1 < d.L, d.update ? d.newmem + (l + 1) * RD : nullptr, d.s));
         if (A->feats && l < d.L - 1)
             HIP_OK(hipMemcpyAsync(A->feats + l * RD, d.b.x, RD * sizeof(float), hipMemcpyDeviceToDevice, d.s));
@@ -1217,7 +1254,7 @@
     long long Rs = 0, views_s = 0;
     for (int gi = 0; gi < A->n_groups; ++gi) {
         const must3r_hip_group& G = A->groups[gi];
-        if (!G.tokens || !G.pos || !G.pointmaps) return fail("decode: null buffer in group %d", gi);
+        if (((!G.tokens || !G.pos) && !A->prefix) || !G.pointmaps) return fail("decode: null buffer in group %d", gi);
         if (G.n_views <= 0 || G.n_tokens <= 0) return fail("decode: empty group %d", gi);
         if (G.pointmaps_scene_stride != 0 && G.pointmaps_scene_stride < (long long)G.n_views * G.H * G.W * 7)
             return fail("decode: group %d: pointmaps_scene_stride %lld is smaller than one scene's pointmaps", gi, (long long)G.pointmaps_scene_stride);
@@ -1228,6 +1265,20 @@
         if (G.H / 16 > c->rope_npos || G.W / 16 > c->rope_npos) return fail("decode: group %d: image too large for the RoPE table", gi);
         Rs += (long long)G.n_views * G.n_tokens;
         views_s += G.n_views;
+    }
+    if (A->prefix) {
+        const must3r_hip_prefix& X = *A->prefix;
+        if (A->n_groups != 1) return fail("decode: a prefix feeds ONE group of views (no forward_list)");
+        if (A->cp) return fail("decode: a prefix cannot feed a context-parallel call");
+        if (A->feats) return fail("decode: a prefix cannot feed a return_feats call (the encoder-side rows of block 0 are not recomputed)");
+        if (A->dtype & MUST3R_ATTN_FP8) return fail("decode: a prefix holds 16-bit queries, not MUST3R_ATTN_FP8 ones");
+        if (!X.x0 || !X.x1 || !X.q16 || !X.pos || !X.view_slot) return fail("decode: prefix: null buffer");
+        if ((reinterpret_cast<uintptr_t>(X.x0) | reinterpret_cast<uintptr_t>(X.x1) | reinterpret_cast<uintptr_t>(X.q16) | reinterpret_cast<uintptr_t>(X.pos)) & 15)
+            return fail("decode: prefix: x0, x1, q16 and pos must be 16-byte aligned");
+        if (X.n_slots <= 0 || X.n_scenes != S || X.n_tokens != A->groups[0].n_tokens || (long long)X.n_slots * S > 65535)
+            return fail("decode: prefix of %d slots x %d scenes x %d tokens for a call of %d scenes x %d tokens", X.n_slots, X.n_scenes, X.n_tokens, S, A->groups[0].n_tokens);
+        for (int j = 0; j < A->groups[0].n_views; ++j)
+            if (X.view_slot[j] < 0 || X.view_slot[j] >= X.n_slots) return fail("decode: prefix: view %d names slot %d of %d", j, X.view_slot[j], X.n_slots);
     }
     for (int l = 0; l < c->cfg.dec_depth; ++l)
         if (!A->mem[l]) return fail("decode: null memory buffer for layer %d", l);
@@ -1251,6 +1302,7 @@
                     must3r_hip_ctx::kSlotBytes / (2 * sizeof(void*) * c->cfg.dec_depth), c->cfg.dec_depth);
     if (S * views_s <= max_views) return decode_impl(c, A, stream);
     if (!A->render) return fail("decode: %lld views in one memory update (limit %lld)", S * views_s, max_views);
+    if (A->prefix) return fail("decode: a prefix cannot feed a render of %lld views, which is cut into several calls (limit %lld)", S * views_s, max_views);
     if (A->feats) return fail("decode: return_feats with %lld rendered views in one call (limit %lld)", S * views_s, max_views);
     must3r_hip_decode_args sub = *A;
     if (S > 1) {
@@ -1291,6 +1343,88 @@
     return 0;
 }
 
+static int prefix_slots(must3r_hip_ctx* c, const must3r_hip_prefix_args* P, int k0, int nk, int n0, hipStream_t s) {
+    const must3r_hip_config& g = c->cfg;
+    const DType dt = c->dt;
+    const int C = g.enc_dim, D = g.dec_dim, S = P->n_scenes, V = P->n_views, N = P->n_tokens, nviews = nk * S, R = nviews * N;
+    const size_t row0 = (size_t)k0 * S * N;
+    uint16_t* t16;
+    BlockRows b{R, D, g.dec_heads, g.mlp_ratio * D, P->x1 + row0 * D, nullptr, nullptr, nullptr, nullptr, nullptr, P->pos_out + row0 * 2};
+    Workspace ws;
+    ws.want(t16, (size_t)R * C);
+    ws.want(b.h16, (size_t)R * D);
+    ws.want(b.qkv, (size_t)R * 3 * D);
+    ws.want(b.a16, (size_t)R * D);
+    M3R_OK(ws.commit(c, s));
+    std::vector<int> chunk((size_t)nviews);
+    std::vector<AttnView> views((size_t)nviews);
+    double sa_flops = 0;
+    for (int k = 0; k < nk; ++k)
+        for (int sc = 0; sc < S; ++sc) {
+            const int i = k * S + sc;
+            chunk[i] = sc * V + P->slot_view[k0 + k];
+            views[i] = AttnView{i * N, N, i * N, N, 0, 0};
+            sa_flops += 4.0 * N * (double)N * D;
+        }
+    void *chunk_dev = nullptr, *views_dev = nullptr;
+    M3R_OK(upload_table(c, chunk.data(), sizeof(int) * chunk.size(), &chunk_dev, s));
+    M3R_OK(upload_table(c, views.data(), sizeof(AttnView) * views.size(), &views_dev, s));
+    {
+        ChunkGatherArgs ga;
+        memset(&ga, 0, sizeof(ga));
+        ga.table = reinterpret_cast<const int*>(chunk_dev); ga.nchunks = nviews;
+        ga.src[0] = P->pos; ga.dst[0] = P->pos_out + row0 * 2; ga.units[0] = (unsigned)N;
+        ga.cast_in = P->tokens; ga.cast_out = t16; ga.cast_n4 = (unsigned)((size_t)N * C / 4);
+        const char* err = "";
+        ProfScope ps(c, s, PC_MISC, 0.0);
+        if (launch_chunk_gather(dt, ga, s, &err)) return fail("%s", err);
+        ps.kernel("prefix_cast");
+    }
+    const void* w;
+    M3R_OK(w16(c, "decoder.feat_embed_enc_to_dec.weight", dt, &w, s));
+    GemmArgs ge = gargs(t16, w, p32(c, "decoder.feat_embed_enc_to_dec.bias"), b.x, R, D, C, C, D);
+    const long long plain_rows = (long long)(n0 > k0 ? n0 - k0 : 0) * S * N;
+    if (plain_rows < R) { ge.bias2 = p32(c, "decoder.image2_embed"); ge.row_start2 = (int)plain_rows; }
+    M3R_OK(gemm(c, dt, EPI_F32, ge, s));
+    const std::vector<Param*>& LP = c->dec_tab[0];
+    Fold fold;
+    const SelfViews sv{reinterpret_cast<const AttnView*>(views_dev), nviews, N, sa_flops, nviews == 1 ? &views[0] : nullptr};
+    M3R_OK(self_attention_sublayer(c, dt, LP, b, sv, fold, false, P->x0 + row0 * D, nullptr, s));
+    return cross_attention_query(c, dt, LP, b, fold, reinterpret_cast<uint16_t*>(P->q16) + row0 * D, s);
+}
+
+extern "C" int must3r_hip_prefix_once(void) { return opt(OPT_PREFIX_ONCE) != 0 && opt(OPT_LNFOLD256) == 0 ? 1 : 0; }
+
+extern "C" int must3r_hip_decode_prefix(must3r_hip_ctx* c, const must3r_hip_prefix_args* P) {
+    if (!c || !P) return fail("decode_prefix: null argument");
+    if (!c->fin_dec) return fail("decode_prefix: decoder weights not finalized");
+    if (P->dtype & MUST3R_ATTN_FP8) return fail("decode_prefix: the pass leaves 16-bit queries, not MUST3R_ATTN_FP8 ones");
+    if (!set_mode(c, P->dtype)) return fail("decode_prefix: bad dtype %d", P->dtype);
+    if (!P->tokens || !P->pos || !P->slot_view || !P->slot_embed || !P->x0 || !P->x1 || !P->q16 || !P->pos_out) return fail("decode_prefix: null buffer");
+    if ((reinterpret_cast<uintptr_t>(P->tokens) | reinterpret_cast<uintptr_t>(P->pos) | reinterpret_cast<uintptr_t>(P->x0) | reinterpret_cast<uintptr_t>(P->x1) |
+         reinterpret_cast<uintptr_t>(P->q16) | reinterpret_cast<uintptr_t>(P->pos_out)) & 15)
+        return fail("decode_prefix: tokens, pos, x0, x1, q16 and pos_out must be 16-byte aligned");
+    const int S = P->n_scenes, V = P->n_views, N = P->n_tokens, K = P->n_slots;
+    if (S <= 0 || V <= 0 || N <= 0 || K <= 0) return fail("decode_prefix: %d scenes x %d views x %d tokens, %d slots", S, V, N, K);
+    int n0 = 0;
+    for (int k = 0; k < K; ++k) {
+        if (P->slot_view[k] < 0 || P->slot_view[k] >= V) return fail("decode_prefix: slot %d names view %d of %d", k, P->slot_view[k], V);
+        if (!P->slot_embed[k]) {
+            if (n0 != k) return fail("decode_prefix: the slots without image2_embed must come first (slot %d)", k);
+            ++n0;
+        }
+    }
+    const long long max_views = (long long)(must3r_hip_ctx::kSlotBytes / (2 * sizeof(AttnView)));
+    long long per = max_views / S;
+    if ((1LL << 24) / ((long long)S * N) < per) per = (1LL << 24) / ((long long)S * N);
+    if (per < 1) return fail("decode_prefix: %d scenes x %d tokens do not fit one launch sequence (limit %lld views, 2^24 rows)", S, N, max_views);
+    DeviceGuard dev_guard(c->device);
+    if (c->dec_tab.empty()) build_layer_tables(c, true);
+    for (int k0 = 0; k0 < K; k0 += (int)per)
+        M3R_OK(prefix_slots(c, P, k0, K - k0 < per ? K - k0 : (int)per, n0, reinterpret_cast<hipStream_t>(P->stream)));
+    return 0;
+}
+
 extern "C" int must3r_hip_op_gemm(int dtype, int epi, const void* A, const void* W, const float* bias, void* out, int M, int N,
                                   int K, int lda, int ldc, const int64_t* pos, const float* rope_tab, int rope_cols,
                                   int rope_npos, const float* bias2, int row_start2, int accumulate, int ntok, int gw, int H,
diff --git a/must3r_amd/csrc/options.hpp b/must3r_amd/csrc/options.hpp
--- a/must3r_amd/csrc/options.hpp
+++ b/must3r_amd/csrc/options.hpp
@@ -19,6 +19,7 @@
     OPT_G256_GM,
     OPT_NN_LEAF_LOG2,
     OPT_NN_QUERY_LANES_LOG2,
+    OPT_PREFIX_ONCE,
     OPT_COUNT
 };
 
diff --git a/must3r_amd/engine.py b/must3r_amd/engine.py
--- a/must3r_amd/engine.py
+++ b/must3r_amd/engine.py
@@ -102,15 +102,20 @@
     strided = bool(getattr(decoder, "_ctx", "x") != "x") and imgs.is_cuda
     H, W = int(imgs.shape[-2]), int(imgs.shape[-1])
     upd_all = torch.empty((S, sum(mem_batches), H, W, 7), dtype=torch.float32, device=imgs.device) if strided else None
+    Vm = sum(mem_batches)
+    once = (strided and S > 1 and Vm == V and bool(_lib.load().must3r_hip_prefix_once()) and not getattr(decoder, "attention_fp8", False)
+            and getattr(decoder, "prefix_pass", None) is not None)
+    rows = decoder.prefix_pass(x, pos, list(range(V)) + [0], [0] + [1] * V) if once else None
     mem, upd, i = None, [], 0
     for nb in mem_batches:
         if strided:
-            mem, pm = decoder(x[:, i:i + nb], pos[:, i:i + nb], ts[:, i:i + nb], mem, pointmaps_out=upd_all[:, i:i + nb])
+            mem, pm = decoder(x[:, i:i + nb], pos[:, i:i + nb], ts[:, i:i + nb], mem, pointmaps_out=upd_all[:, i:i + nb],
+                              **({"prefix": (rows, list(range(i, i + nb)))} if once else {}))
         else:
             mem, pm = decoder(x[:, i:i + nb], pos[:, i:i + nb], ts[:, i:i + nb], mem)
             upd.append(pm)
         i += nb
-    _, ren = decoder(x, pos, ts, mem, render=True)
+    _, ren = decoder(x, pos, ts, mem, render=True, **({"prefix": (rows, [V] + list(range(1, V)))} if once else {}))
     out = {"update": upd_all if strided else torch.cat(upd, dim=1), "render": ren, "mem": mem, "x": x, "pos": pos}
     if activate:
         out.update(postprocess(out["render"]))
diff --git a/must3r_amd/model/decoder.py b/must3r_amd/model/decoder.py
--- a/must3r_amd/model/decoder.py
+++ b/must3r_amd/model/decoder.py
@@ -28,6 +28,10 @@
             v._m3r_owner = self
             out.append(v)
         return out
+
+
+class _PrefixRows:
+    """Result of ``MUSt3R.prefix_pass``: ``x0`` / ``x1`` fp32 and ``q16`` [n_slots, B, N, D], ``pos`` int64 [n_slots, B, N, 2] (slot-major)."""
 
 
 class MUSt3R(HipModule):
@@ -150,13 +154,37 @@
                                  "and cannot be read with it off; re-run the update in this mode)")
 
     @torch.no_grad()
-    def forward(self, x, pos, true_shape, current_mem=None, render=False, return_feats=False, pointmaps_out=None, cp=None):
+    def forward(self, x, pos, true_shape, current_mem=None, render=False, return_feats=False, pointmaps_out=None, cp=None, prefix=None):
         is_list = isinstance(x, (list, tuple))
         if is_list:
             return_feats = False
-        return self._forward(x, pos, true_shape, current_mem, render, return_feats, pointmaps_out, cp)
-
-    def _forward(self, x, pos, true_shape, current_mem, render, return_feats, pointmaps_out=None, cp=None):
+        return self._forward(x, pos, true_shape, current_mem, render, return_feats, pointmaps_out, cp, prefix)
+
+    @torch.no_grad()
+    def prefix_pass(self, x, pos, slot_view, slot_embed):
+        ctx = self._context()
+        dev = self._ctx_dev
+        device = torch.device("cuda", dev)
+        if self.attention_fp8:
+            raise ValueError("prefix_pass leaves 16-bit queries: not with attention_fp8")
+        B, V, N, _ = x.shape
+        x = self._check_input(x, "x", torch.float32)
+        pos = self._check_input(pos, "pos", torch.int64)
+        odt = self._operand()
+        K, D = len(slot_view), self.embed_dim
+        rows = _PrefixRows()
+        rows.n_slots, rows.B, rows.N = K, int(B), int(N)
+        rows.x0 = torch.empty((K, B, N, D), dtype=torch.float32, device=device)
+        rows.x1 = torch.empty((K, B, N, D), dtype=torch.float32, device=device)
+        rows.q16 = torch.empty((K, B, N, D), dtype=_TORCH_DT[odt], device=device)
+        rows.pos = torch.empty((K, B, N, 2), dtype=torch.int64, device=device)
+        args = _lib.PrefixArgs(odt, x.data_ptr(), pos.data_ptr(), B, V, N, K, (C.c_int32 * K)(*[int(v) for v in slot_view]),
+                               (C.c_int32 * K)(*[1 if e else 0 for e in slot_embed]), rows.x0.data_ptr(), rows.x1.data_ptr(), rows.q16.data_ptr(),
+                               rows.pos.data_ptr(), _lib.stream_ptr(dev))
+        _lib.check(ctx.lib.must3r_hip_decode_prefix(ctx.handle, C.byref(args)))
+        return rows
+
+    def _forward(self, x, pos, true_shape, current_mem, render, return_feats, pointmaps_out=None, cp=None, prefix=None):
         is_list = isinstance(x, (list, tuple))
         xs = list(x) if is_list else [x]
         poss = list(pos) if is_list else [pos]
@@ -164,12 +192,12 @@
         B = int(xs[0].shape[0])
         assert all(int(t.shape[0]) == B for t in xs + poss), "all groups must share the batch size"
         pouts = None if pointmaps_out is None else (list(pointmaps_out) if isinstance(pointmaps_out, (list, tuple)) else [pointmaps_out])
-        out, outs, feats = self._forward_scene(xs, poss, shapes, current_mem, render, return_feats, pouts, cp)
+        out, outs, feats = self._forward_scene(xs, poss, shapes, current_mem, render, return_feats, pouts, cp, prefix)
         if return_feats:
             return out, (outs if is_list else outs[0]), (feats if is_list else feats[0])
         return out, (outs if is_list else outs[0])
 
-    def _forward_scene(self, xs, poss, shapes, current_mem, render, return_feats, pouts=None, cp=None):
+    def _forward_scene(self, xs, poss, shapes, current_mem, render, return_feats, pouts=None, cp=None, prefix=None):
         MAXV = 1024
         B = int(xs[0].shape[0])
         if render and return_feats and B == 1 and sum(int(x.shape[1]) for x in xs) > MAXV:
@@ -203,8 +231,9 @@
         nimgs, Ns = [], []
         for i, (xi, pi, ti) in enumerate(zip(xs, poss, shapes)):
             _, n, N, Cenc = xi.shape
-            xi = self._check_input(xi, "x", torch.float32)
-            pi = self._check_input(pi, "pos", torch.int64)
+            if prefix is None:
+                xi = self._check_input(xi, "x", torch.float32)
+                pi = self._check_input(pi, "pos", torch.int64)
             ts = ti.reshape(-1, 2)
             if ts.is_cuda:
                 ts = ts.cpu()
@@ -225,7 +254,7 @@
                 pm = torch.empty((B, n, H, W, 7), dtype=torch.float32, device=device)
             keep += [xi, pi]
             outs.append(pm)
-            groups[i] = _lib.Group(xi.data_ptr(), pi.data_ptr(), n, N, H, W, pm.data_ptr(), sstride)
+            groups[i] = _lib.Group(xi.data_ptr() if prefix is None else None, pi.data_ptr() if prefix is None else None, n, N, H, W, pm.data_ptr(), sstride)
             R += n * N
             nimgs.append(n)
             Ns.append(N)
@@ -268,10 +297,20 @@
                 raise ValueError("context-parallel cross attention is for one-view memory updates of one scene against an existing memory, memory_mode 'kv', "
                                  "16-bit attention operands")
             cp_struct = cp.native_args(ctx, R, device)
+        px_struct = None
+        if prefix is not None:
+            rows, slots = prefix
+            if rows.q16.dtype != _TORCH_DT[odt] or rows.q16.device != device:
+                raise ValueError("prefix: the rows were computed in another precision mode or on another device")
+            px_struct = _lib.Prefix(rows.x0.data_ptr(), rows.x1.data_ptr(), rows.q16.data_ptr(), rows.pos.data_ptr(), rows.n_slots, rows.B, rows.N,
+                                    (C.c_int32 * len(slots))(*[int(k) for k in slots]))
+            if len(slots) != sum(nimgs):
+                raise ValueError(f"prefix: {len(slots)} slots for {sum(nimgs)} views")
         args = _lib.DecodeArgs(odt | (_lib.ATTN_FP8 if self.attention_fp8 else 0), _MEM_MODE[self.memory_mode],
                                1 if render else 0, 1 if current_mem is None else 0,
                                len(xs), groups, Nm, ptrs, feats_buf.data_ptr() if return_feats else None,
-                               cap, B, stride, C.pointer(cp_struct) if cp_struct is not None else None, 1 if self._causal else 0)
+                               cap, B, stride, C.pointer(cp_struct) if cp_struct is not None else None, 1 if self._causal else 0,
+                               C.addressof(px_struct) if px_struct is not None else None)
         rc = ctx.lib.must3r_hip_decode(ctx.handle, C.byref(args), _lib.stream_ptr(dev))
         if cp is not None and rc != 0:
             cp.reraise()
@@ -330,10 +369,10 @@
         self.use_xformers_mask, self.use_mem_mask = bool(use_xformers_mask), bool(use_mem_mask)
 
     @torch.no_grad()
-    def forward(self, x, pos, true_shape, current_mem=None, render=False, return_feats=False, pointmaps_out=None):
+    def forward(self, x, pos, true_shape, current_mem=None, render=False, return_feats=False, pointmaps_out=None, prefix=None):
         if isinstance(x, (list, tuple)):
             raise TypeError("CausalMUSt3R.forward takes tensors [B, nimgs, N, C] (the reference's class has no list dispatch, decoder.py:435-439)")
-        return self._forward(x, pos, true_shape, current_mem, render, return_feats, pointmaps_out)
+        return self._forward(x, pos, true_shape, current_mem, render, return_feats, pointmaps_out, None, prefix)
 
     def forward_list(self, *a, **k):
         raise TypeError("CausalMUSt3R has no forward_list (decoder.py:352-553)")
```
